# Beryl2000/SE-UNet-AirSeg

Hardware: AMD Instinct MI355X
Metric: voxels/sec SE-UNet fwd+bwd, 128^3 patch (higher is better)
Workload: dtype bf16

## Files before the change

### se-unet-airseg_amd/SE_UNet.py

```python
from __future__ import annotations

import ctypes as C
import os
from typing import List, Optional, Tuple

import torch
import torch.nn as nn

from . import _lib

config = {}

_DEBUG_FILL: Optional[int] = None


def _fresh(shape, dtype, device):
    t = torch.empty(shape, dtype=dtype, device=device)
    if _DEBUG_FILL is not None:
        t.view(torch.uint8).fill_(_DEBUG_FILL)
    return t


def _default_dtype() -> str:
    return os.environ.get("SEUNET_DTYPE", "bf16")
# ... 86 lines not shown
    while lib.seunet_net_conv_info(C.byref(desc), len(out), C.byref(info)) == 0:
        k = lambda code: _lib.KERNEL_NAMES[code]
        x_name = info.x_name.decode() or None
        out.append({
            "name": info.name.decode(), "taps": info.taps, "dilation": info.dilation, "level": info.level,
            "dims": (info.dims.n, info.dims.d, info.dims.h, info.dims.w),
            "src_c": [info.src_c[i] for i in range(info.nsrc)],
            "src_is_input": [bool(info.src_is_input[i]) for i in range(info.nsrc)],
            "cin": info.cin, "cout": info.cout, "need_dgrad": bool(info.need_dgrad),
            "fwd": k(info.fwd), "dgrad": k(info.dgrad) if info.need_dgrad else None, "wgrad": k(info.wgrad),
            "x_name": x_name, "x_materialised": bool(info.x_materialised),
            "x_fwd": k(info.x_fwd) if x_name and info.x_materialised else None,
            "x_wgrad": k(info.x_wgrad) if x_name and info.x_materialised else None,
            "src_dist": info.src_dist,
        })
    return out


def _is_decoder(name: str) -> bool:
    return name.startswith("dc") and not name.startswith("dc0_")


def alloc_flat_grads(params, dead, device, names=None):
    idx = list(range(len(params)))
    if names is not None:
        idx = [i for i in idx if not _is_decoder(names[i])] + [i for i in idx if _is_decoder(names[i])]
    sizes = {i: (0 if dead[i] else params[i].numel()) for i in idx}
    flat = _fresh(sum(sizes.values()), torch.float32, device)
    grads, off, split = [None] * len(params), 0, None
    for i in idx:
        if names is not None and split is None and _is_decoder(names[i]):
            split = off
        if not dead[i]:
            grads[i] = flat[off:off + sizes[i]].view(params[i].shape)
        off += sizes[i]
    return flat, grads, (off if split is None else split)


class _SEUNetFunction(torch.autograd.Function):
    @staticmethod
    def forward(ctx, x, drop1, drop2, meta, *params):
        lib = _lib.load()
        b, _, d, h, w = x.shape
        desc = make_desc(b, meta["in_channel"], meta["n_classes"], d, h, w, meta["width_mult"],
                         meta["dtype"], meta["conv_impl"], meta["negative_slope"])
        with torch.cuda.device(x.device):
            ws_bytes = lib.seunet_net_workspace_bytes(C.byref(desc))
            if ws_bytes == 0:
                raise RuntimeError("libseunet_hip net_workspace_bytes: " + _lib.last_error())
            ws = _fresh(ws_bytes, torch.uint8, x.device)
            pred0 = _fresh((b, meta["n_classes"], d, h, w), torch.float32, x.device)
            pred1 = _fresh((b, meta["n_classes"], d, h, w), torch.float32, x.device)
            plist = [p.detach().contiguous() for p in params]
            for p in plist:
                if p.device != x.device:
                    raise RuntimeError(f"SE_UNet parameters are on {p.device} but the input is on {x.device}")
            parr = _lib.ptr_array(plist)
            _lib.check(lib.seunet_net_forward(C.byref(desc), parr, x.data_ptr(), _lib.ptr(drop1), _lib.ptr(drop2),
                                              pred0.data_ptr(), pred1.data_ptr(), ws.data_ptr(), ws_bytes,
                                              _lib.stream_ptr()), "net_forward")
        ctx.desc, ctx.ws, ctx.ws_bytes = desc, ws, ws_bytes
        ctx.plist, ctx.drop = plist, (drop1, drop2)
        ctx.dead = meta["dead"]
        ctx.loss_scale = float(meta.get("loss_scale", 1.0))
        ctx.overflow, ctx.pending = meta.get("overflow"), meta.get("pending")
        ctx.names, ctx.grad_sync = meta.get("names"), meta.get("grad_sync")
        ctx.input_grad = bool(meta.get("input_grad", False))
        return pred0, pred1

    @staticmethod
    def backward(ctx, g0, g1):
        if ctx.ws is None:
            raise RuntimeError("SE_UNet (HIP path): the backward pass of this forward call has already run; it consumes "
                               "the saved workspace, so a second backward (retain_graph=True, or two losses "
                               "back-propagated separately) is not supported -- sum the losses and call backward once")
        lib = _lib.load()
        dev = ctx.ws.device
        shape = (ctx.desc.batch, ctx.desc.n_classes, ctx.desc.d, ctx.desc.h, ctx.desc.w)
        with torch.cuda.device(dev):
            g0 = torch.zeros(shape, dtype=torch.float32, device=dev) if g0 is None else g0.contiguous().float()
            g1 = torch.zeros(shape, dtype=torch.float32, device=dev) if g1 is None else g1.contiguous().float()
            if ctx.loss_scale != 1.0:
                g0, g1 = g0 * ctx.loss_scale, g1 * ctx.loss_scale
            flat, grads, split = alloc_flat_grads(ctx.plist, ctx.dead, dev, ctx.names)
            garr = _lib.ptr_array(grads)
            parr = _lib.ptr_array(ctx.plist)
            sync = ctx.grad_sync
            ev = sync.decoder_event() if sync is not None else None
            grad_x = None
            if ctx.input_grad and ctx.needs_input_grad[0]:
                d = ctx.desc
                grad_x = _fresh((d.batch, d.in_channel, d.d, d.h, d.w), torch.float32, dev)
                sbytes = lib.seunet_net_input_grad_bytes(C.byref(d))
                if sbytes == 0:
                    raise RuntimeError("libseunet_hip net_input_grad_bytes: " + _lib.last_error())
                scratch = _fresh(sbytes, torch.uint8, dev)
                _lib.check(lib.seunet_net_backward_input(C.byref(d), parr, g0.data_ptr(), g1.data_ptr(), _lib.ptr(ctx.drop[0]),
                                                         _lib.ptr(ctx.drop[1]), garr, grad_x.data_ptr(), scratch.data_ptr(), sbytes,
                                                         ctx.ws.data_ptr(), ctx.ws_bytes, _lib.stream_ptr(),
                                                         None if ev is None else ev.cuda_event), "net_backward_input")
            else:
                _lib.check(lib.seunet_net_backward_ev(C.byref(ctx.desc), parr, g0.data_ptr(), g1.data_ptr(),
                                                      _lib.ptr(ctx.drop[0]), _lib.ptr(ctx.drop[1]), garr,
                                                      ctx.ws.data_ptr(), ctx.ws_bytes, _lib.stream_ptr(),
                                                      None if ev is None else ev.cuda_event), "net_backward")
            if sync is not None:
                sync.exchange(flat, split, ev)
            if ctx.loss_scale != 1.0:
                ok = torch.isfinite(flat).all()
                if grad_x is not None:
                    ok = ok & torch.isfinite(grad_x).all()
                    grad_x.copy_(torch.where(ok, grad_x * (1.0 / ctx.loss_scale), torch.zeros((), dtype=grad_x.dtype, device=dev)))
                flat.copy_(torch.where(ok, flat * (1.0 / ctx.loss_scale), torch.zeros((), dtype=flat.dtype, device=dev)))
                if ctx.overflow is not None:
                    ctx.overflow.add_((~ok).to(ctx.overflow.dtype))
                if ctx.pending is not None:
                    ctx.pending.bitwise_or_((~ok).to(ctx.pending.dtype))
        ctx.ws = None
        return (grad_x, None, None, None) + tuple(grads)


class SE_UNet(nn.Module):

    def __init__(self, in_channel=1, n_classes=1, width_mult=1, negative_slope=0.01,
                 act_dtype: Optional[str] = None, conv_impl: Optional[int] = None, input_grad: bool = False):
        super().__init__()
        self.input_grad = bool(input_grad)
        self.in_channel, self.n_classes = in_channel, n_classes
        self.width_mult, self.negative_slope = width_mult, negative_slope
        self.act_dtype = act_dtype or _default_dtype()
        self.conv_impl = _default_conv_impl() if conv_impl is None else conv_impl
        self.loss_scale = 65536.0 if _lib.dtype_code(self.act_dtype) == _lib.F16 else 1.0
        self.overflow_steps = None
        self.overflow_pending = None
        self.batchnorm, self.bias, self.out_channel2, self.sigmoid_output = False, True, 2, 0
        m = width_mult
        self.ec1 = SSEConv(in_channel, 8 * m)
        self.ec2 = SSEConv(8 * m, 16 * m)
        self.ec3 = SSEConv(16 * m, 32 * m, dilation=2)
        self.ec33 = CATConv(56 * m, 32 * m)
        self.x33 = CATConv(in_channel, 32 * m)
        self.ec4 = SSEConv2(32 * m, 32 * m, down_sample=2)
        self.ec5 = SSEConv2(32 * m, 32 * m, dilation=2, down_sample=2)
        self.ec6 = SSEConv2(32 * m, 64 * m, dilation=2, down_sample=2)
        self.ec63 = CATConv(128 * m, 64 * m)
        self.x63 = CATConv(in_channel, 64 * m)
        self.ec7 = SSEConv2(64 * m, 64 * m, down_sample=4)
        self.ec8 = SSEConv2(64 * m, 64 * m, dilation=2, down_sample=4)
        self.ec9 = SSEConv2(64 * m, 64 * m, dilation=2, down_sample=4)
        self.ec93 = CATConv(192 * m, 64 * m)
        self.x93 = CATConv(in_channel, 64 * m)
        self.ec10 = SSEConv2(64 * m, 64 * m, down_sample=8)
        self.ec11 = SSEConv2(64 * m, 64 * m, down_sample=8)
        self.ec12 = SSEConv2(64 * m, 64 * m, down_sample=8)
        self.ec123 = CATConv(192 * m, 64 * m)
        self.dc1 = SSEConv2(128 * m, 64 * m, down_sample=4)
        self.dc2 = SSEConv2(64 * m, 64 * m, down_sample=4)
        self.dc22 = CATConv(128 * m, 64 * m)
        self.dc3 = SSEConv2(128 * m, 64 * m, down_sample=2)
        self.dc4 = SSEConv2(64 * m, 32 * m, down_sample=2)
        self.dc42 = CATConv(96 * m, 32 * m)
        self.dc5 = SSEConv(64 * m, 32 * m, down_sample=1)
        self.dc6 = SSEConv(32 * m, 16 * m, down_sample=1)
        self.dc62 = CATConv(48 * m, 16 * m)
        self.dc0_0 = nn.Conv3d(24, n_classes, 1, bias=True)
        self.dc0_1 = nn.Conv3d(12, n_classes, 1, bias=True)
        self.dropout1 = DropLayer(channel_num=24, thr=0.3)
# ... 222 lines not shown
```

### se-unet-airseg_amd/csrc/cat.hip

```cpp
#include "epilogue.h"
#include <type_traits>

namespace seunet {

template <bool XR>
__device__ __forceinline__ void second_branch(const float (&in8)[8], const float (&wa)[8], const float (&wb)[8], float (&x2)[8]) {
#pragma unroll
  for (int j = 0; j < 8; ++j) x2[j] = XR ? wa[j] * in8[0] + wb[j] * in8[1] : in8[j];
}

template <typename T, int LPV, bool TWO, bool XR>
__global__ void __launch_bounds__(EPI_THREADS)
cat_fwd_kernel(const T* __restrict__ raw, const float* __restrict__ mean, const float* __restrict__ rstd,
               const T* __restrict__ raw2, const float* __restrict__ mean2, const float* __restrict__ rstd2, int C, float slope,
               T* __restrict__ out, long long V, const float* __restrict__ w2x, int xic) {
  SEUNET_EPI_THREAD(LPV);
  float mu[8], rs[8], mu2[8], rs2[8], wa[8], wb[8];
#pragma unroll
  for (int j = 0; j < 8; ++j) {
    mu[j] = mean[n * C + c0 + j]; rs[j] = rstd[n * C + c0 + j];
    mu2[j] = TWO ? mean2[n * C + c0 + j] : 0.f;
    rs2[j] = TWO ? rstd2[n * C + c0 + j] : 0.f;
    wa[j] = XR ? w2x[(c0 + j) * xic] : 0.f;
    wb[j] = (XR && xic > 1) ? w2x[(c0 + j) * xic + 1] : 0.f;
  }
  const long long stride = (long long)P * VPB;
  long long v = (long long)blockIdx.x * VPB + vb;
  Pack8<T> nx, nx2;
  zero8p(nx); zero8p(nx2);
  if (v < V) {
    const long long o = ((long long)n * V + v) * C + c0;
    load8p(raw + o, nx);
    if (TWO) load8p(XR ? raw2 + ((long long)n * V + v) * 8 : raw2 + o, nx2);
  }
  for (; v < V; v += stride) {
    const long long o = ((long long)n * V + v) * C + c0;
    float x[8], in2[8], x2[8], y[8];
    unpack8(nx, x);
    if (TWO) { unpack8(nx2, in2); second_branch<XR>(in2, wa, wb, x2); }
    if (v + stride < V) {
      load8p(raw + o + stride * C, nx);
      if (TWO) load8p(XR ? raw2 + ((long long)n * V + v + stride) * 8 : raw2 + o + stride * C, nx2);
    }
#pragma unroll
    for (int j = 0; j < 8; ++j) y[j] = norm_lrelu(x[j], mu[j], rs[j], slope);
    if (TWO) {
#pragma unroll
      for (int j = 0; j < 8; ++j) y[j] += norm_lrelu(x2[j], mu2[j], rs2[j], slope);
    }
    store8(out + o, y);
  }
}

template <typename T, int LPV>
__global__ void __launch_bounds__(EPI_THREADS)
cat_fwd_pool_kernel(const T* __restrict__ raw, const float* __restrict__ mean, const float* __restrict__ rstd,
                    const T* __restrict__ xin, const float* __restrict__ mean2, const float* __restrict__ rstd2, int C, float slope,
                    T* __restrict__ out, T* __restrict__ pooled, int D, int H, int W, const float* __restrict__ w2x, int xic,
                    unsigned* __restrict__ argmax) {
  SEUNET_EPI_THREAD(LPV);
  float mu[8], rs[8], mu2[8], rs2[8], wa[8], wb[8];
#pragma unroll
  for (int j = 0; j < 8; ++j) {
    mu[j] = mean[n * C + c0 + j]; rs[j] = rstd[n * C + c0 + j];
    mu2[j] = mean2[n * C + c0 + j]; rs2[j] = rstd2[n * C + c0 + j];
    wa[j] = w2x[(c0 + j) * xic];
    wb[j] = xic > 1 ? w2x[(c0 + j) * xic + 1] : 0.f;
  }
  const int Do = D / 2, Ho = H / 2, Wo = W / 2;
  const long long V = (long long)D * H * W, Vo = (long long)Do * Ho * Wo;
  const long long stride = (long long)P * VPB;
  for (long long cv = (long long)blockIdx.x * VPB + vb; cv < Vo; cv += stride) {
    const int xo = (int)(cv % Wo);
    const int yo = (int)((cv / Wo) % Ho);
    const int zo = (int)(cv / ((long long)Wo * Ho));
    const long long v0 = ((long long)(2 * zo) * H + 2 * yo) * W + 2 * xo;
    Pack8<T> px[8], pi[8];
#pragma unroll
    for (int k = 0; k < 8; ++k) {
      const long long v = v0 + ((long long)(k >> 2) * H + ((k >> 1) & 1)) * W + (k & 1);
      load8p(raw + ((long long)n * V + v) * C + c0, px[k]);
      load8p(xin + ((long long)n * V + v) * 8, pi[k]);
    }
// ... 153 lines not shown
      }
    }
    if (APPLY) store8(dxhat_out + o, d);
  }
  if (APPLY) return;
  const int wave = threadIdx.x >> 6, lane = threadIdx.x & 63;
  if (XW) {
    __shared__ double redx[4][16][16];
#pragma unroll
    for (int j = 0; j < 8; ++j)
#pragma unroll
      for (int i = 0; i < 2; ++i) {
        const double r = stride_sum_d<LPV>((double)xw[j][i]);
        if (lane < LPV) redx[wave][lane][j * 2 + i] = r;
      }
    __syncthreads();
    double* rec = xw_partial + ((long long)n * P + blockIdx.x) * (C * 2);
    for (int e = threadIdx.x; e < LPV * 16; e += EPI_THREADS) {
      const int gq = e / 16, k = e % 16;
      rec[(gq * 8 + (k >> 1)) * 2 + (k & 1)] = ((redx[0][gq][k] + redx[1][gq][k]) + redx[2][gq][k]) + redx[3][gq][k];
    }
  }
  __shared__ double red[4][16][32];
#pragma unroll
  for (int q = 0; q < 4; ++q)
#pragma unroll
    for (int j = 0; j < 8; ++j) {
      const double r = stride_sum_d<LPV>((double)s[q][j]);
      if (lane < LPV) red[wave][lane][q * 8 + j] = r;
    }
  __syncthreads();
  const long long rec = (long long)n * P + blockIdx.x;
  for (int i = threadIdx.x; i < LPV * 32; i += EPI_THREADS) {
    const int gq = i / 32, k = i % 32, q = k >> 3;
    const double tot = ((red[0][gq][k] + red[1][gq][k]) + red[2][gq][k]) + red[3][gq][k];
    const int c = gq * 8 + (k & 7);
    if (q < 2) stat_partial[(rec * C + c) * 2 + q] = tot;
    else if (TWO) stat_partial2[(rec * C + c) * 2 + (q - 2)] = tot;
  }
}

template <typename T>
__global__ void __launch_bounds__(EPI_THREADS)
input_moments_kernel(const T* __restrict__ xin, double* __restrict__ partial, long long V) {
  const int n = blockIdx.y, P = gridDim.x;
  double s[5] = {0.0, 0.0, 0.0, 0.0, 0.0};
  for (long long v = (long long)blockIdx.x * EPI_THREADS + threadIdx.x; v < V; v += (long long)P * EPI_THREADS) {
    float x[8];
    load8(xin + ((long long)n * V + v) * 8, x);
    const double a = (double)x[0], b = (double)x[1];
    s[0] += a; s[1] += b; s[2] += a * a; s[3] += a * b; s[4] += b * b;
  }
  __shared__ double red[4][5];
  block_sum(s, red);
  if (const int k = threadIdx.x; k < 5) partial[((long long)n * P + blockIdx.x) * 5 + k] = wave4_sum(red, k);
}

__global__ void __launch_bounds__(256)
xbranch_stats_kernel(const double* __restrict__ partial, int slots, const float* __restrict__ w2, int C, int ic,
                     double inv_count, float eps, float* __restrict__ mean2, float* __restrict__ rstd2,
                     double* __restrict__ moments_out) {
  const int n = blockIdx.x;
  __shared__ double red[4][5], tot[5];
  double s[5] = {0.0, 0.0, 0.0, 0.0, 0.0};
  for (int b = threadIdx.x; b < slots; b += 256)
#pragma unroll
    for (int k = 0; k < 5; ++k) s[k] += partial[((long long)n * slots + b) * 5 + k];
  block_sum(s, red);
  if (threadIdx.x < 5) tot[threadIdx.x] = wave4_sum(red, threadIdx.x) * inv_count;
  __syncthreads();
  if (moments_out != nullptr && threadIdx.x < 5) moments_out[n * 5 + threadIdx.x] = tot[threadIdx.x];
  const double m0 = tot[0], m1 = tot[1];
  const double c00 = tot[2] - m0 * m0, c01 = tot[3] - m0 * m1, c11 = tot[4] - m1 * m1;
  for (int c = threadIdx.x; c < C; c += 256) {
    const double a = (double)w2[c * ic], b = ic > 1 ? (double)w2[c * ic + 1] : 0.0;
    const double mu = a * m0 + b * m1;
    double var = a * a * c00 + 2.0 * a * b * c01 + b * b * c11;
    if (var < 0.0) var = 0.0;
    mean2[n * C + c] = (float)mu;
    rstd2[n * C + c] = (float)(1.0 / sqrt(var + (double)eps));
  }
}

__global__ void __launch_bounds__(256)
xw_finalize_kernel(const double* __restrict__ xw_partial, const double* __restrict__ stat_partial2, int slots, int C, int N,
                   const double* __restrict__ moments, const float* __restrict__ w2, int ic, double eps, float* __restrict__ dw) {
  const int wave = threadIdx.x >> 6, lane = threadIdx.x & 63;
  const int c = blockIdx.x;
  __shared__ double red[4][3];
  const double wa = (double)w2[c * ic], wb = ic > 1 ? (double)w2[c * ic + 1] : 0.0;
  double g0 = 0.0, g1 = 0.0;
  for (int n = 0; n < N; ++n) {
    double s[3] = {0.0, 0.0, 0.0};
    for (int r = threadIdx.x; r < slots; r += 256) {
      const long long rec = (long long)n * slots + r;
      s[0] += xw_partial[(rec * C + c) * 2 + 0];
      s[1] += xw_partial[(rec * C + c) * 2 + 1];
      s[2] += stat_partial2[(rec * C + c) * 2 + 0];
    }
#pragma unroll
    for (int k = 0; k < 3; ++k) {
      double r = s[k];
#pragma unroll
      for (int off = 32; off >= 1; off >>= 1) r += shfl_xor_settled(r, off);
      if (lane == 0) red[wave][k] = r;
    }
    __syncthreads();
    if (threadIdx.x == 0) {
      const double S0 = wave4_sum(red, 0), S1 = wave4_sum(red, 1), Sd = wave4_sum(red, 2);
      const double* m = moments + n * 5;
      const double c00 = m[2] - m[0] * m[0], c01 = m[3] - m[0] * m[1], c11 = m[4] - m[1] * m[1];
      const double A0 = S0 - m[0] * Sd, A1 = S1 - m[1] * Sd;
      double var = wa * wa * c00 + 2.0 * wa * wb * c01 + wb * wb * c11;
      if (var < 0.0) var = 0.0;
      const double rs2 = 1.0 / (var + eps), rs = sqrt(rs2);
      const double proj = wa * A0 + wb * A1;
      g0 += rs * (A0 - rs2 * proj * (wa * c00 + wb * c01));
      g1 += rs * (A1 - rs2 * proj * (wa * c01 + wb * c11));
    }
    __syncthreads();
  }
  if (threadIdx.x == 0) {
    dw[c * ic] = (float)g0;
    if (ic > 1) dw[c * ic + 1] = (float)g1;
  }
}

template <typename T>
__global__ void __launch_bounds__(256)
xbranch_values_kernel(const T* __restrict__ x_in, const float* __restrict__ w2x, int C, int xic, float* __restrict__ out, long long V,
                      long long total) {
  for (long long i = blockIdx.x * (long long)blockDim.x + threadIdx.x; i < total; i += (long long)gridDim.x * blockDim.x) {
    const int cg = (int)(i % (C / 8));
    const long long nv = i / (C / 8);
    const long long n = nv / V, v = nv % V;
    float wa[8], wb[8], in2[8], x2[8];
#pragma unroll
    for (int j = 0; j < 8; ++j) {
      wa[j] = w2x[(cg * 8 + j) * xic];
      wb[j] = xic > 1 ? w2x[(cg * 8 + j) * xic + 1] : 0.f;
    }
    Pack8<T> px;
    load8p(x_in + nv * 8, px);
    unpack8(px, in2);
    second_branch<true>(in2, wa, wb, x2);
#pragma unroll
    for (int j = 0; j < 8; ++j) out[(n * C + cg * 8 + j) * V + v] = x2[j];
  }
}

static int cat_branch(const char* who, const CatBlock& b, Branch2& x, bool& two, bool& xr) {
  if (int e = check_c(b.C)) return e;
  x = b.b.kind == Branch2::None ? Branch2{} : b.b;
  two = x.kind != Branch2::None;
  xr = x.kind == Branch2::Recomputed;
  SEUNET_CHECK(!xr || (x.in_channel >= 1 && x.in_channel <= 2), "%s: in_channel %d (1 or 2)", who, x.in_channel);
  return 0;
}

int launch_cat_fwd(int dtype, const CatBlock& b, void* out, const PoolOut& pool, Dims d, hipStream_t s) {
  Branch2 x;
  bool two, xr;
  if (int e = cat_branch("cat_epilogue_fwd", b, x, two, xr)) return e;
  SEUNET_CHECK(!pool.pooled || (xr && d.D % 2 == 0 && d.H % 2 == 0 && d.W % 2 == 0),
               "cat_epilogue_fwd: the fused max-pool needs a recomputed second branch and even extents");
  dim3 grid(epi_partials(d) * 4, d.N);
#define SEUNET_CAT_FWD(...) <<<grid, EPI_THREADS, 0, s>>>((const T*)b.a.raw, b.a.mean, b.a.rstd, (const T*)x.src, x.mean2, x.rstd2, b.C, b.slope, (T*)out, __VA_ARGS__)
  SEUNET_LPV_SWITCH(b.C / 8, {
    SEUNET_DTYPE_SWITCH(dtype, {
      if (pool.pooled) cat_fwd_pool_kernel<T, LPV> SEUNET_CAT_FWD((T*)pool.pooled, d.D, d.H, d.W, x.w2, x.in_channel, pool.argmax);
      else if (xr) cat_fwd_kernel<T, LPV, true, true> SEUNET_CAT_FWD(d.vox(), x.w2, x.in_channel);
      else if (two) cat_fwd_kernel<T, LPV, true, false> SEUNET_CAT_FWD(d.vox(), nullptr, 0);
      else cat_fwd_kernel<T, LPV, false, false> SEUNET_CAT_FWD(d.vox(), nullptr, 0);
    });
  });
#undef SEUNET_CAT_FWD
  SEUNET_LAUNCH_CHECK();
  return 0;
}

static int cat_bwd_pool(const char* who, bool xr, const PoolGrad& pool, Dims d, PoolRef& pr) {
  pr = PoolRef{};
  if (pool.argmax == nullptr) return 0;
  SEUNET_CHECK(xr && pool.g_pool != nullptr && d.D % 2 == 0 && d.H % 2 == 0 && d.W % 2 == 0 && d.vox() < (1ll << 31),
               "%s: pooled gradient needs a recomputed second branch and even extents below 2^31 voxels", who);
  pr.argmax = pool.argmax; pr.g_pool = pool.g_pool;
  pr.W = (unsigned)d.W; pr.H = (unsigned)d.H; pr.Wo = (unsigned)d.W / 2; pr.Ho = (unsigned)d.H / 2;
  pr.mW = (unsigned)((1ull << 32) / (unsigned)d.W); pr.mH = (unsigned)((1ull << 32) / (unsigned)d.H);
  pr.Vo = d.vox() / 8;
  return 0;
}

#define SEUNET_CAT_BWD(TWO, APPLY, XW, XR, XG)                                                                                   \
  cat_bwd_kernel<T, LPV, TWO, APPLY, XW, XR, XG><<<grid, EPI_THREADS, 0, s>>>(                                                    \
      (const T*)g_out, (const T*)b.a.raw, b.a.mean, b.a.rstd, (const T*)x.src, x.mean2, x.rstd2, b.C, b.slope, a.m1, a.m2, a.m1b, \
      a.m2b, (T*)a.dx, (T*)a.dx2, o.stat_partial, o.stat_partial2, d.vox(), o.xw_partial, x.w2, x.in_channel, pr, a.gx_out,     \
      a.gx_acc)

int launch_cat_bwd_sums(int dtype, const CatBlock& b, const void* g_out, const PoolGrad& pool, const CatSums& out, Dims d,
                        hipStream_t s) {
  Branch2 x;
  bool two, xr;
  PoolRef pr;
  if (int e = cat_branch("cat_epilogue_bwd_sums", b, x, two, xr)) return e;
  if (int e = cat_bwd_pool("cat_epilogue_bwd_sums", xr, pool, d, pr)) return e;
  SEUNET_CHECK(out.stat_partial && (!two || out.stat_partial2), "cat_epilogue_bwd_sums needs the partial buffers");
  SEUNET_CHECK(!out.xw_partial || xr, "cat_epilogue_bwd_sums: the weight-gradient sums belong to a recomputed second branch");
  const CatSums o{out.stat_partial, two ? out.stat_partial2 : nullptr, out.xw_partial};
  const CatApply a{};
  dim3 grid(epi_partials(d), d.N);
  SEUNET_LPV_SWITCH(b.C / 8, {
    SEUNET_DTYPE_SWITCH(dtype, {
      if (xr && o.xw_partial) SEUNET_CAT_BWD(true, false, true, true, false);
      else if (xr) SEUNET_CAT_BWD(true, false, false, true, false);
      else if (two) SEUNET_CAT_BWD(true, false, false, false, false);
      else SEUNET_CAT_BWD(false, false, false, false, false);
    });
  });
  SEUNET_LAUNCH_CHECK();
  return 0;
}

int launch_cat_bwd_apply(int dtype, const CatBlock& b, const void* g_out, const PoolGrad& pool, const CatApply& io, Dims d,
                         hipStream_t s) {
  Branch2 x;
  bool two, xr;
  PoolRef pr;
  if (int e = cat_branch("cat_epilogue_bwd_apply", b, x, two, xr)) return e;
  if (int e = cat_bwd_pool("cat_epilogue_bwd_apply", xr, pool, d, pr)) return e;
  SEUNET_CHECK(io.m1 && io.m2 && io.dx && (!two || (io.m1b && io.m2b)) && (!two || xr || io.dx2),
               "cat_epilogue_bwd_apply: missing argument");
  SEUNET_CHECK(!io.gx_out || xr, "cat_epilogue_bwd_apply: the input-gradient term belongs to a recomputed second branch");
  const CatApply a{io.m1, io.m2, two ? io.m1b : nullptr, two ? io.m2b : nullptr, io.dx, two && !xr ? io.dx2 : nullptr,
                   io.gx_out, io.gx_out ? io.gx_acc : 0};
  const CatSums o{};
  dim3 grid(epi_partials(d) * 4, d.N);
  SEUNET_LPV_SWITCH(b.C / 8, {
    SEUNET_DTYPE_SWITCH(dtype, {
      if (xr && a.gx_out) SEUNET_CAT_BWD(true, true, false, true, true);
      else if (xr) SEUNET_CAT_BWD(true, true, false, true, false);
      else if (two) SEUNET_CAT_BWD(true, true, false, false, false);
      else SEUNET_CAT_BWD(false, true, false, false, false);
    });
  });
  SEUNET_LAUNCH_CHECK();
  return 0;
}
#undef SEUNET_CAT_BWD

int xbranch_moment_slots(Dims d) { return epi_partials(d); }

int launch_xbranch_moments(int dtype, const void* x_in, double* partial, Dims d, hipStream_t s) {
  dim3 grid(xbranch_moment_slots(d), d.N);
  SEUNET_DTYPE_SWITCH(dtype, input_moments_kernel<T><<<grid, EPI_THREADS, 0, s>>>((const T*)x_in, partial, d.vox()));
  SEUNET_LAUNCH_CHECK();
  return 0;
}

int launch_xbranch_stats(const double* partial, int slots, const float* w2, int C, int in_channel, int N, long long count,
                         float eps, float* mean2, float* rstd2, double* moments_out, hipStream_t s) {
  SEUNET_CHECK(in_channel >= 1 && in_channel <= 2, "xbranch_stats: in_channel %d (1 or 2)", in_channel);
  xbranch_stats_kernel<<<N, 256, 0, s>>>(partial, slots, w2, C, in_channel, 1.0 / (double)count, eps, mean2, rstd2, moments_out);
  SEUNET_LAUNCH_CHECK();
  return 0;
}

int launch_cat_xgrad_finalize(const double* xw_partial, const double* stat_partial2, int slots, const double* moments, const float* w2,
                              int C, int in_channel, int N, float eps, float* dw, hipStream_t s) {
  SEUNET_CHECK(in_channel >= 1 && in_channel <= 2, "cat_xgrad_finalize: in_channel %d (1 or 2)", in_channel);
  xw_finalize_kernel<<<C, 256, 0, s>>>(xw_partial, stat_partial2, slots, C, N, moments, w2, in_channel, (double)eps, dw);
  SEUNET_LAUNCH_CHECK();
  return 0;
}

int launch_xbranch_values(int dtype, const void* x_in, const float* w2, int C, int in_channel, float* out, Dims d, hipStream_t s) {
  SEUNET_CHECK(in_channel >= 1 && in_channel <= 2 && C % 8 == 0, "xbranch_values: bad argument");
  const long long total = (long long)d.N * d.vox() * (C / 8);
  const int grid = (int)((total + 255) / 256 > 8192 ? 8192 : (total + 255) / 256);
  SEUNET_DTYPE_SWITCH(dtype, xbranch_values_kernel<T><<<grid, 256, 0, s>>>((const T*)x_in, w2, C, in_channel, out, d.vox(), total));
  SEUNET_LAUNCH_CHECK();
  return 0;
}

}
```

### se-unet-airseg_amd/csrc/epilogue.h

```cpp
#pragma once
#include "seunet_common.h"

namespace seunet {

int epi_partials(Dims d);
int launch_channel_stats(int dtype, const void* t, int C, double* partial, Dims d, hipStream_t s);
int launch_stats_finalize(const double* partial, int slots, int C, int N, long long count,
                          float eps, int mode, float* out_a, float* out_b, hipStream_t s);
struct NormIn { const void* raw; const float* mean; const float* rstd; };
struct SseParams {
  const float* w_se;
  const float* w_se2;
  const float* w_side;
  const float* b_side;
  float slope;
};
struct GateBlock { NormIn a; int C; SseParams p; };
struct SseHead {
  float* side_out;
  float* level_map;
  int level_accumulate;
  const float* head_w;
  const float* drop;
  int drop_stride;
};
struct SseBwdIn {
  const void* g_e;
  const float* g_side;
  const float* g_level;
};
struct SseSums { double* stat_partial; float* pgrad_partial; };
struct SseApply { const float* m1; const float* m2; void* draw_out; };
int launch_sse_fwd(int dtype, const GateBlock& b, void* e_out, const SseHead& head, Dims d, hipStream_t s);
int launch_sse_bwd_sums(int dtype, const GateBlock& b, const SseBwdIn& g, const SseHead& head, const SseSums& out, Dims d,
                        hipStream_t s);
int launch_sse_bwd_apply(int dtype, const GateBlock& b, const SseBwdIn& g, const SseHead& head, const SseApply& io, Dims d,
                         hipStream_t s);
int launch_gate_bwd_finalize(const double* stat_partial, int slots, int C, int N, long long count, float* m1, float* m2,
                             const float* pgrad_partial, int records, float* dw_se, float* dw_se2, float* dw_side,
                             float* db_side, float* dhead_w, hipStream_t s);
int launch_pgrad_reduce(const float* pgrad_partial, int records, int C, float* dw_se,
                        float* dw_se2, float* dw_side, float* db_side, float* dhead_w,
                        hipStream_t s);
struct Branch2 {
  enum Kind { None, Stored, Recomputed } kind;
  const void* src;
  const float* mean2;
  const float* rstd2;
  const float* w2;
  int in_channel;
};
struct CatBlock { NormIn a; Branch2 b; int C; float slope; };
struct PoolOut { void* pooled; unsigned* argmax; };
struct PoolGrad { const unsigned* argmax; const void* g_pool; };
struct CatSums {
  double* stat_partial;
  double* stat_partial2;
  double* xw_partial;
};
struct CatApply {
  const float *m1, *m2, *m1b, *m2b;
  void* dx;
  void* dx2;
  float* gx_out;
  int gx_acc;
};
int launch_cat_fwd(int dtype, const CatBlock& b, void* out, const PoolOut& pool, Dims d, hipStream_t s);
int launch_cat_bwd_sums(int dtype, const CatBlock& b, const void* g_out, const PoolGrad& pool, const CatSums& out, Dims d,
                        hipStream_t s);
int launch_cat_bwd_apply(int dtype, const CatBlock& b, const void* g_out, const PoolGrad& pool, const CatApply& io, Dims d,
                         hipStream_t s);
int xbranch_moment_slots(Dims d);
int launch_xbranch_moments(int dtype, const void* x_in, double* partial, Dims d, hipStream_t s);
int launch_xbranch_stats(const double* partial, int slots, const float* w2, int C, int in_channel, int N, long long count,
                         float eps, float* mean2, float* rstd2, double* moments_out, hipStream_t s);
int launch_cat_xgrad_finalize(const double* xw_partial, const double* stat_partial2, int slots, const double* moments, const float* w2,
                              int C, int in_channel, int N, float eps, float* dw, hipStream_t s);
int launch_xbranch_values(int dtype, const void* x_in, const float* w2, int C, int in_channel, float* out_ncdhw, Dims d, hipStream_t s);

#ifdef __HIPCC__
static constexpr int EPI_THREADS = 256;

template <typename T> __device__ __forceinline__ float round_to(float v) {
  if constexpr (sizeof(T) == 4) return v;
  else return unpack_lo<T>(pack2<T>(v, 0.f));
}

template <typename T> __device__ __forceinline__ float gate_sigmoid(float z) {
  if constexpr (sizeof(T) == 4) return 1.f / (1.f + expf(-z));
  else return __builtin_amdgcn_rcpf(1.f + __builtin_amdgcn_exp2f(-1.44269504088896341f * z));
}

#define SEUNET_EPI_THREAD(LPV)                                \
  const int n = blockIdx.y, P = gridDim.x;                    \
  const int cg = threadIdx.x % LPV, vb = threadIdx.x / LPV;   \
  constexpr int VPB = EPI_THREADS / LPV;                      \
  const int c0 = cg * 8

__device__ __forceinline__ float lrelu(float xh, float slope) { return xh > 0.f ? xh : xh * slope; }
__device__ __forceinline__ float norm_lrelu(float x, float mu, float rs, float slope) { return lrelu((x - mu) * rs, slope); }
__device__ __forceinline__ float lrelu_slope(float xh, float slope) { return xh > 0.f ? 1.f : slope; }

template <typename E, int K> __device__ __forceinline__ E wave4_sum(const E (&red)[4][16][K], int g, int k) {
  return ((red[0][g][k] + red[1][g][k]) + red[2][g][k]) + red[3][g][k];
}
template <typename E, int K> __device__ __forceinline__ E wave4_sum(const E (&red)[4][K], int k) {
  return ((red[0][k] + red[1][k]) + red[2][k]) + red[3][k];
}
template <typename E> __device__ __forceinline__ E wave4_sum(const E (&w)[4]) { return ((w[0] + w[1]) + w[2]) + w[3]; }

template <int K> __device__ __forceinline__ void block_sum(const double (&s)[K], double (&red)[4][K]) {
  const int wave = threadIdx.x >> 6, lane = threadIdx.x & 63;
#pragma unroll
  for (int k = 0; k < K; ++k) {
    double r = s[k];
#pragma unroll
    for (int off = 32; off >= 1; off >>= 1) r += shfl_xor_settled(r, off);
    if (lane == 0) red[wave][k] = r;
  }
  __syncthreads();
}

__device__ __forceinline__ void stats_finalize_body(int idx, const double* __restrict__ partial, int slots, int C, double inv_count,
                                                    float eps, int mode, float* __restrict__ out_a, float* __restrict__ out_b) {
  const int n = idx / C, c = idx % C;
  double s1 = 0.0, s2 = 0.0;
  for (int p = threadIdx.x; p < slots; p += 256) {
    const double* q = partial + (((long long)n * slots + p) * C + c) * 2;
    s1 += q[0];
    s2 += q[1];
  }
#pragma unroll
  for (int off = 32; off >= 1; off >>= 1) {
    s1 += shfl_xor_settled(s1, off);
    s2 += shfl_xor_settled(s2, off);
  }
  __shared__ double w1[4], w2[4];
  if ((threadIdx.x & 63) == 0) { w1[threadIdx.x >> 6] = s1; w2[threadIdx.x >> 6] = s2; }
  __syncthreads();
  if (threadIdx.x == 0) {
    s1 = wave4_sum(w1);
    s2 = wave4_sum(w2);
    if (mode == 0) {
      const double mean = s1 * inv_count;
      double var = s2 * inv_count - mean * mean;
      if (var < 0.0) var = 0.0;
      out_a[idx] = (float)mean;
      out_b[idx] = (float)(1.0 / sqrt(var + (double)eps));
    } else {
      out_a[idx] = (float)(s1 * inv_count);
      out_b[idx] = (float)(s2 * inv_count);
    }
  }
}

#define SEUNET_LPV_SWITCH(LPVVAL, ...)                                                  \
  switch (LPVVAL) {                                                                       \
    case 1: { constexpr int LPV = 1; __VA_ARGS__; } break;                                       \
    case 2: { constexpr int LPV = 2; __VA_ARGS__; } break;                                       \
    case 4: { constexpr int LPV = 4; __VA_ARGS__; } break;                                       \
// ... 13 lines not shown
```

### se-unet-airseg_amd/csrc/gate.hip

```cpp
#include "epilogue.h"

namespace seunet {

template <typename T, int LPV, bool G2>
__global__ void __launch_bounds__(EPI_THREADS)
sse_fwd_kernel(const T* __restrict__ raw, const float* __restrict__ mean, const float* __restrict__ rstd, int C, SseParams p,
               T* __restrict__ e_out, SseHead head, long long V) {
  SEUNET_EPI_THREAD(LPV);
  float mu[8], rs[8], wse[8], wse2[8], w20[8], w21[8];
#pragma unroll
  for (int j = 0; j < 8; ++j) {
    mu[j] = mean[n * C + c0 + j];
    rs[j] = rstd[n * C + c0 + j];
    wse[j] = p.w_se[c0 + j];
    wse2[j] = G2 ? p.w_se2[c0 + j] : 0.f;
    w20[j] = p.w_side[c0 + j];
    w21[j] = p.w_side[C + c0 + j];
  }
  const float b20 = p.b_side[0], b21 = p.b_side[1], slope = p.slope;
  const bool want_side = head.side_out != nullptr || head.level_map != nullptr;
  float hw0 = 0.f, hw1 = 0.f;
  if (head.level_map) {
    hw0 = head.head_w[0] * (head.drop ? head.drop[n * head.drop_stride + 0] : 1.f);
    hw1 = head.head_w[1] * (head.drop ? head.drop[n * head.drop_stride + 1] : 1.f);
  }
  const long long stride = (long long)P * VPB;
  long long v = (long long)blockIdx.x * VPB + vb;
  Pack8<T> nx;
  zero8p(nx);
  if (v < V) load8p(raw + ((long long)n * V + v) * C + c0, nx);
  for (; v < V; v += stride) {
    const long long vi = (long long)n * V + v;
    float x[8], a[8], e[8];
    unpack8(nx, x);
    if (v + stride < V) load8p(raw + (vi + stride) * C + c0, nx);
    float d1 = 0.f;
#pragma unroll
    for (int j = 0; j < 8; ++j) {
      a[j] = norm_lrelu(x[j], mu[j], rs[j], slope);
      d1 += wse[j] * a[j];
    }
    const float g1 = gate_sigmoid<T>(group_sum<LPV>(d1));
    float d2 = 0.f;
#pragma unroll
    for (int j = 0; j < 8; ++j) {
      e[j] = a[j] * g1;
      d2 += wse2[j] * e[j];
    }
    if (G2) {
      const float g2 = gate_sigmoid<T>(group_sum<LPV>(d2));
#pragma unroll
      for (int j = 0; j < 8; ++j) e[j] *= g2;
    }
    store8(e_out + vi * C + c0, e);
    if (want_side) {
      float s0 = 0.f, s1 = 0.f;
#pragma unroll
      for (int j = 0; j < 8; ++j) { s0 += w20[j] * e[j]; s1 += w21[j] * e[j]; }
      s0 = group_sum<LPV>(s0) + b20;
      s1 = group_sum<LPV>(s1) + b21;
      if (cg == 0) {
        if (head.side_out) { head.side_out[vi * 2] = s0; head.side_out[vi * 2 + 1] = s1; }
        if (head.level_map) {
          const float t = hw0 * s0 + hw1 * s1;
          head.level_map[vi] = head.level_accumulate ? head.level_map[vi] + t : t;
        }
      }
    }
  }
}

template <typename T, int LPV, bool G2, bool APPLY, bool LEVEL>
__global__ void __launch_bounds__(EPI_THREADS, (APPLY || G2) ? 1 : 3)
sse_bwd_kernel(const T* __restrict__ raw, const float* __restrict__ mean, const float* __restrict__ rstd, int C, SseParams p,
               SseBwdIn g, SseHead head, const float* __restrict__ m1p, const float* __restrict__ m2p, T* dxhat_out,
               double* __restrict__ stat_partial, float* __restrict__ pgrad_partial, long long V) {
  SEUNET_EPI_THREAD(LPV);
  float mu[8], rs[8], wse[8], wse2[8], w20[8], w21[8];
#pragma unroll
  for (int j = 0; j < 8; ++j) {
    mu[j] = mean[n * C + c0 + j];
    rs[j] = rstd[n * C + c0 + j];
    wse[j] = p.w_se[c0 + j];
// ... 137 lines not shown
  if (LEVEL) {
    float h0 = cg == 0 ? b20 * sgl : 0.f, h1 = cg == 0 ? b21 * sgl : 0.f;
#pragma unroll
    for (int j = 0; j < 8; ++j) {
      const float G = aw20[j];
      h0 += w20[j] * G;
      h1 += w21[j] * G;
      aw20[j] = hw0 * G;
      aw21[j] = hw1 * G;
    }
    adh0 = dr0 * h0;
    adh1 = dr1 * h1;
    adb0 = cg == 0 ? hw0 * sgl : 0.f;
    adb1 = cg == 0 ? hw1 * sgl : 0.f;
  }
  double sdx[8], sdxx[8];
#pragma unroll
  for (int j = 0; j < 8; ++j) {
    sdx[j] = (F64ACC ? acc64[j][threadIdx.x] : 0.0) + (double)fdx[j];
    sdxx[j] = (F64ACC ? acc64[8 + j][threadIdx.x] : 0.0) + (double)fdxx[j];
  }

  __shared__ double redd[4][16][16];
  __shared__ float red[4][16][32];
  __shared__ float reds[4][4];
  const int wave = threadIdx.x >> 6, lane = threadIdx.x & 63;
#pragma unroll
  for (int j = 0; j < 8; ++j) {
    const double r0 = stride_sum_d<LPV>(sdx[j]), r1 = stride_sum_d<LPV>(sdxx[j]);
    const float r2 = stride_sum<LPV>(awse[j]), r3 = stride_sum<LPV>(awse2[j]);
    const float r4 = stride_sum<LPV>(aw20[j]), r5 = stride_sum<LPV>(aw21[j]);
    if (lane < LPV) {
      redd[wave][lane][j] = r0;     redd[wave][lane][8 + j] = r1;
      red[wave][lane][j] = r2;      red[wave][lane][8 + j] = r3;
      red[wave][lane][16 + j] = r4; red[wave][lane][24 + j] = r5;
    }
  }
  {
    const float q0 = stride_sum<1>(adb0), q1 = stride_sum<1>(adb1);
    const float q2 = stride_sum<1>(adh0), q3 = stride_sum<1>(adh1);
    if (lane == 0) { reds[wave][0] = q0; reds[wave][1] = q1; reds[wave][2] = q2; reds[wave][3] = q3; }
  }
  __syncthreads();
  const long long rec = (long long)n * P + blockIdx.x;
  float* pg = pgrad_partial + rec * (4 * C + 4);
  for (int i = threadIdx.x; i < LPV * 16; i += EPI_THREADS) {
    const int gq = i / 16, k = i % 16;
    const double tot = wave4_sum(redd, gq, k);
    stat_partial[(rec * C + gq * 8 + (k & 7)) * 2 + (k >> 3)] = tot;
  }
  for (int i = threadIdx.x; i < LPV * 32; i += EPI_THREADS) {
    const int gq = i / 32, k = i % 32;
    const float tot = wave4_sum(red, gq, k);
    pg[(k >> 3) * C + gq * 8 + (k & 7)] = tot;
  }
  if (const int k = threadIdx.x; k < 4) pg[4 * C + k] = wave4_sum(reds, k);
}

__device__ __forceinline__ void pgrad_reduce_body(int blk, const float* __restrict__ pg, int records, int C, float* dw_se,
                                                  float* dw_se2, float* dw_side, float* db_side, float* dhead_w) {
  const int wave = threadIdx.x >> 6, lane = threadIdx.x & 63;
  const int k = blk * 4 + wave, K = 4 * C + 4;
  if (k >= K) return;
  double s = 0.0;
  for (int r = lane; r < records; r += 64) s += (double)pg[(long long)r * K + k];
#pragma unroll
  for (int off = 32; off >= 1; off >>= 1) s += shfl_xor_settled(s, off);
  if (lane != 0) return;
  const float v = (float)s;
  if (k < C) { if (dw_se) dw_se[k] = v; }
  else if (k < 2 * C) { if (dw_se2) dw_se2[k - C] = v; }
  else if (k < 4 * C) { if (dw_side) dw_side[k - 2 * C] = v; }
  else if (k < 4 * C + 2) { if (db_side) db_side[k - 4 * C] = v; }
  else { if (dhead_w) dhead_w[k - 4 * C - 2] = v; }
}
__global__ void __launch_bounds__(256)
pgrad_reduce_kernel(const float* __restrict__ pg, int records, int C, float* dw_se, float* dw_se2,
                    float* dw_side, float* db_side, float* dhead_w) {
  pgrad_reduce_body(blockIdx.x, pg, records, C, dw_se, dw_se2, dw_side, db_side, dhead_w);
}
__global__ void __launch_bounds__(256)
gate_bwd_finalize_kernel(const double* __restrict__ partial, int slots, int C, int N, double inv_count, float* __restrict__ m1,
                         float* __restrict__ m2, const float* __restrict__ pg, int records, float* dw_se, float* dw_se2,
                         float* dw_side, float* db_side, float* dhead_w) {
  if ((int)blockIdx.x < N * C) stats_finalize_body(blockIdx.x, partial, slots, C, inv_count, 0.f, 1, m1, m2);
  else pgrad_reduce_body((int)blockIdx.x - N * C, pg, records, C, dw_se, dw_se2, dw_side, db_side, dhead_w);
}

int launch_sse_fwd(int dtype, const GateBlock& b, void* e_out, const SseHead& head, Dims d, hipStream_t s) {
  if (int e = check_c(b.C)) return e;
  dim3 grid(epi_partials(d) * 4, d.N);
  const bool g2 = b.p.w_se2 != nullptr;
  SEUNET_LPV_SWITCH(b.C / 8, {
    SEUNET_DTYPE_SWITCH(dtype, {
      if (g2) sse_fwd_kernel<T, LPV, true><<<grid, EPI_THREADS, 0, s>>>((const T*)b.a.raw, b.a.mean, b.a.rstd, b.C, b.p, (T*)e_out, head, d.vox());
      else sse_fwd_kernel<T, LPV, false><<<grid, EPI_THREADS, 0, s>>>((const T*)b.a.raw, b.a.mean, b.a.rstd, b.C, b.p, (T*)e_out, head, d.vox());
    });
  });
  SEUNET_LAUNCH_CHECK();
  return 0;
}

template <typename T, bool APPLY>
static int sse_bwd_t(const GateBlock& b, const SseBwdIn& g, const SseHead& head, const SseSums& o, const SseApply& a, Dims d,
                     hipStream_t s) {
  dim3 grid(epi_partials(d) * (APPLY ? 4 : 1), d.N);
  const bool g2 = b.p.w_se2 != nullptr;
  const bool level = g.g_level != nullptr;
#define SEUNET_SSE_BWD(G2V, LV) sse_bwd_kernel<T, LPV, G2V, APPLY, LV><<<grid, EPI_THREADS, 0, s>>>((const T*)b.a.raw, b.a.mean, b.a.rstd, b.C, b.p, g, head, a.m1, a.m2, (T*)a.draw_out, o.stat_partial, o.pgrad_partial, d.vox())
  SEUNET_LPV_SWITCH(b.C / 8, {
    if (g2) { if (level) SEUNET_SSE_BWD(true, true); else SEUNET_SSE_BWD(true, false); }
    else { if (level) SEUNET_SSE_BWD(false, true); else SEUNET_SSE_BWD(false, false); }
  });
#undef SEUNET_SSE_BWD
  SEUNET_LAUNCH_CHECK();
  return 0;
}

int launch_sse_bwd_sums(int dtype, const GateBlock& b, const SseBwdIn& g, const SseHead& head, const SseSums& out, Dims d,
                        hipStream_t s) {
  if (int e = check_c(b.C)) return e;
  SEUNET_CHECK(out.stat_partial && out.pgrad_partial, "gate_epilogue_bwd_sums needs the partial buffers");
  SEUNET_DTYPE_SWITCH(dtype, return (sse_bwd_t<T, false>(b, g, head, out, SseApply{}, d, s)));
  return 1;
}

int launch_sse_bwd_apply(int dtype, const GateBlock& b, const SseBwdIn& g, const SseHead& head, const SseApply& io, Dims d,
                         hipStream_t s) {
  if (int e = check_c(b.C)) return e;
  SEUNET_CHECK(io.m1 && io.m2 && io.draw_out, "gate_epilogue_bwd_apply needs m1, m2 and the output tensor");
  SEUNET_DTYPE_SWITCH(dtype, return (sse_bwd_t<T, true>(b, g, head, SseSums{}, io, d, s)));
  return 1;
}

int launch_gate_bwd_finalize(const double* stat_partial, int slots, int C, int N, long long count, float* m1, float* m2,
                             const float* pgrad_partial, int records, float* dw_se, float* dw_se2, float* dw_side,
                             float* db_side, float* dhead_w, hipStream_t s) {
  gate_bwd_finalize_kernel<<<N * C + cdiv(4 * C + 4, 4), 256, 0, s>>>(stat_partial, slots, C, N, 1.0 / (double)count, m1, m2,
                                                                     pgrad_partial, records, dw_se, dw_se2, dw_side, db_side, dhead_w);
  SEUNET_LAUNCH_CHECK();
  return 0;
}

int launch_pgrad_reduce(const float* pgrad_partial, int records, int C, float* dw_se, float* dw_se2, float* dw_side, float* db_side,
                        float* dhead_w, hipStream_t s) {
  pgrad_reduce_kernel<<<cdiv(4 * C + 4, 4), 256, 0, s>>>(pgrad_partial, records, C, dw_se, dw_se2, dw_side, db_side, dhead_w);
  SEUNET_LAUNCH_CHECK();
  return 0;
}

}
```

### se-unet-airseg_amd/csrc/heads.hip

```cpp
#include "seunet_common.h"
#include "trilinear.h"

namespace seunet {

__global__ void side_upsample_kernel(const float* __restrict__ side, int C, int scale,
                                     float* __restrict__ out, int c_total, int c_off, int D, int H, int W,
                                     long long total) {
  const int Do = D * scale, Ho = H * scale, Wo = W * scale;
  const float rz = ac_scale(D, Do), ry = ac_scale(H, Ho), rx = ac_scale(W, Wo);
  const long long Vo = (long long)Do * Ho * Wo;
  for (long long i = blockIdx.x * (long long)blockDim.x + threadIdx.x; i < total;
       i += (long long)gridDim.x * blockDim.x) {
    long long r = i;
    const int xo = (int)(r % Wo); r /= Wo;
    const int yo = (int)(r % Ho); r /= Ho;
    const int zo = (int)(r % Do);
    const long long n = r / Do;
    int z0, z1, y0, y1, x0, x1; float lz, ly, lx;
    ac_src(zo, rz, D, z0, z1, lz);
    ac_src(yo, ry, H, y0, y1, ly);
    ac_src(xo, rx, W, x0, x1, lx);
    for (int c = 0; c < C; ++c) {
      float acc = 0.f;
#pragma unroll
// ... 197 lines not shown
  ka = (ca + 3) & ~3; kb = (cb + 3) & ~3;
  const int la = e0 < ebase[2] ? 1 : (e0 < ebase[3] ? 2 : 3), lb = e1 < ebase[2] ? 1 : (e1 < ebase[3] ? 2 : 3);
  float* const outa = e0 < nent ? (la == 1 ? t1a : (la == 2 ? t1b : t1c)) : nullptr;
  float* const outb = e1 < nent ? (lb == 1 ? t1a : (lb == 2 ? t1b : t1c)) : nullptr;
  const int cola = e0 - ebase[la], colb = e1 - ebase[lb], wla = W >> la, wlb = W >> lb;
  double sum = 0.0;
#pragma unroll
  for (int j = 0; j < RPW; ++j) {
    const int rr = wv + 4 * j;
    const long long row = row0 + rr;
    if (row >= rows) break;
    float* rb = hsm + wv * RW;
    if (pf) {
#pragma unroll
      for (int k = 0; k < 4; ++k) {
        const int x = lane + 64 * k;
        if (x < W) { rb[x] = pre[j][k]; sum += (double)pre[j][k]; }
      }
    } else {
      for (int x = lane; x < W; x += 64) { const float v = g[row * W + x]; rb[x] = v; sum += (double)v; }
    }
    __builtin_amdgcn_wave_barrier();
    if (fast) {
      float a0 = 0.f, a1 = 0.f;
#pragma unroll
      for (int k = 0; k < HB_KA; ++k)
        if (k < ka) a0 += wa[k] * rb[fa + k];
#pragma unroll
      for (int k = 0; k < HB_K; ++k)
        if (k < kb) a1 += wb[k] * rb[fb + k];
      if (outa) outa[row * wla + cola] = a0;
      if (outb) outb[row * wlb + colb] = a1;
      __builtin_amdgcn_wave_barrier();
      continue;
    }
    for (int e = lane; e < nent; e += 64) {
      const int l = e < ebase[2] ? 1 : (e < ebase[3] ? 2 : 3);
      float* out = outs[l - 1];
      if (out == nullptr) continue;
      const float* t = tab + e * (HB_K + 2);
      const int first = __float_as_int(t[0]), cnt = __float_as_int(t[1]);
      float acc = 0.f;
      for (int k = 0; k < cnt; k += 4) {
        float w[4], v[4];
#pragma unroll
        for (int j = 0; j < 4; ++j) {
          const bool in = k + j < cnt;
          w[j] = in ? t[2 + k + j] : 0.f;
          v[j] = in ? rb[first + k + j] : 0.f;
        }
#pragma unroll
        for (int j = 0; j < 4; ++j)
          if (w[j] != 0.f) acc += w[j] * v[j];
      }
      out[row * (W >> l) + (e - ebase[l])] = acc;
    }
    __builtin_amdgcn_wave_barrier();
  }
  if (bias_part != nullptr) {
#pragma unroll
    for (int off = 32; off >= 1; off >>= 1) sum += shfl_xor_settled(sum, off);
    __shared__ double wsum[4];
    if (lane == 0) wsum[wv] = sum;
    __syncthreads();
    if (threadIdx.x == 0) bias_part[blockIdx.x] = ((wsum[0] + wsum[1]) + wsum[2]) + wsum[3];
  }
}

__global__ void __launch_bounds__(1024) sum_stage2_wide_kernel(const double* __restrict__ partial, int n, float* __restrict__ out) {
  double s = 0.0;
  for (int i = threadIdx.x; i < n; i += 1024) s += partial[i];
#pragma unroll
  for (int off = 32; off >= 1; off >>= 1) s += shfl_xor_settled(s, off);
  __shared__ double w[16];
  if ((threadIdx.x & 63) == 0) w[threadIdx.x >> 6] = s;
  __syncthreads();
  if (threadIdx.x == 0) {
    double t = 0.0;
    for (int k = 0; k < 16; ++k) t += w[k];
    out[0] = (float)t;
  }
}

int launch_side_upsample(const float* side, int C, int scale, float* out, int c_total, int c_off, Dims dl,
                         hipStream_t s) {
  const long long total = (long long)dl.N * dl.vox() * scale * scale * scale;
  side_upsample_kernel<<<grid_for(total), 256, 0, s>>>(side, C, scale, out, c_total, c_off, dl.D, dl.H, dl.W, total);
  SEUNET_LAUNCH_CHECK();
  return 0;
}

int launch_head_fwd(const float* const* level_maps, int nlevels, const float* bias, float* pred, Dims d0,
                    hipStream_t s) {
  SEUNET_CHECK(nlevels >= 1 && nlevels <= 4, "head: nlevels=%d out of range", nlevels);
  HeadLevels lv;
  for (int l = 0; l < 4; ++l) lv.map[l] = l < nlevels ? level_maps[l] : nullptr;
  for (int l = 1; l < nlevels; ++l)
    SEUNET_CHECK((d0.D >> l) >= 1 && (d0.H >> l) >= 1 && (d0.W >> l) >= 1, "head: volume too small for level %d", l);
  SEUNET_CHECK(d0.W % 4 == 0, "head: W=%d must be a multiple of 4", d0.W);
  if (d0.W % 8 == 0 && d0.W <= 2048 && (long long)d0.D * d0.H * d0.W < (1ll << 31)) {
    const size_t lds = (size_t)4 * HF_RPW * ((d0.W >> 1) + (d0.W >> 2) + (d0.W >> 3)) * sizeof(float);
    const int ybl = (d0.H + 4 * HF_RPW - 1) / (4 * HF_RPW);
    head_fwd_rows_kernel<<<d0.N * d0.D * ybl, 256, lds, s>>>(lv, bias, pred, d0.D, d0.H, d0.W);
  } else {
    const long long total4 = (long long)d0.N * d0.vox() / 4;
    head_fwd_kernel<<<grid_for(total4), 256, 0, s>>>(lv, bias, pred, d0.D, d0.H, d0.W, total4);
  }
  SEUNET_LAUNCH_CHECK();
  return 0;
}

struct AxisJob { const float* in; float* out; int I, O; long long inner, total; };
struct AxisJobs { AxisJob j[3]; };
__global__ void __launch_bounds__(256) up_transpose_axis_multi_kernel(AxisJobs jobs) {
  const AxisJob jb = jobs.j[blockIdx.y];
  if (jb.total == 0) return;
  const float rs = ac_scale(jb.I, jb.O);
  const unsigned inner = (unsigned)jb.inner, I = (unsigned)jb.I, total = (unsigned)jb.total;
  for (unsigned idx = blockIdx.x * blockDim.x + threadIdx.x; idx < total; idx += gridDim.x * blockDim.x) {
    const unsigned q = idx / inner;
    const unsigned in_i = idx - q * inner;
    const unsigned outer = q / I;
    const int i = (int)(q - outer * I);
    int lo, hi;
    ac_range(i, rs, jb.O, lo, hi);
    float acc = 0.f;
    for (int o = lo; o <= hi; o += 4) {
      float w[4], v[4];
#pragma unroll
      for (int k = 0; k < 4; ++k) {
        w[k] = o + k <= hi ? ac_weight(o + k, i, rs, jb.I) : 0.f;
        v[k] = w[k] != 0.f ? jb.in[(outer * (unsigned)jb.O + (unsigned)(o + k)) * inner + in_i] : 0.f;
      }
#pragma unroll
      for (int k = 0; k < 4; ++k)
        if (w[k] != 0.f) acc += w[k] * v[k];
    }
    jb.out[idx] = acc;
  }
}

struct HeadBwdLayout { long long t1[4], t2[4], part, total; };
static HeadBwdLayout head_bwd_layout(Dims d0, int nlevels) {
  HeadBwdLayout m{};
  const long long rows = (long long)d0.N * d0.D * d0.H, V = rows * d0.W;
  long long off = 0, off2 = V - V / 8;
  for (int l = 1; l < nlevels; ++l) {
    m.t1[l] = off;
    off += rows * (d0.W >> l);
    m.t2[l] = off2;
    off2 += (long long)d0.N * d0.D * (d0.H >> l) * (d0.W >> l);
  }
  m.part = (V + V / 2 + 64 + 1) & ~1ll;
  m.total = V + V / 2 + 64 + 2 * ((rows + HB_ROWS - 1) / HB_ROWS + 64);
  return m;
}
size_t head_bwd_tmp_floats(Dims d0) { return (size_t)head_bwd_layout(d0, 4).total; }
int launch_head_bwd(const float* g_pred, float* const* g_levels, int nlevels, float* tmp, float* g_bias,
                    Dims d0, hipStream_t s) {
  SEUNET_CHECK(nlevels >= 1 && nlevels <= 4, "head: nlevels=%d out of range", nlevels);
  const long long rows = (long long)d0.N * d0.D * d0.H;
  const long long V = rows * d0.W;
  const HeadBwdLayout m = head_bwd_layout(d0, nlevels);
  float* t1[4] = {nullptr, nullptr, nullptr, nullptr};
  float* t2[4] = {nullptr, nullptr, nullptr, nullptr};
  for (int l = 1; l < nlevels; ++l) {
    if (g_levels[l]) t1[l] = tmp + m.t1[l];
    t2[l] = tmp + m.t2[l];
  }
  double* part = reinterpret_cast<double*>(tmp + m.part);
  const int nblk = (int)((rows + HB_ROWS - 1) / HB_ROWS);
  SEUNET_CHECK(d0.W <= 1024, "head_bwd: W=%d too large", d0.W);
  SEUNET_CHECK(V / 2 < (1ll << 31), "head_bwd: %lld voxels per call exceed the 32-bit index range of the axis passes", V);
  const size_t lds = ((size_t)4 * (d0.W + HB_PAD) + (size_t)(d0.W - (d0.W >> 3)) * (HB_K + 2)) * sizeof(float);
  head_bwd_x_multi_kernel<<<nblk, 256, lds, s>>>(g_pred, t1[1], t1[2], t1[3], nlevels, d0.W, rows, g_bias ? part : nullptr);
  AxisJobs jy{}, jz{};
  long long max_y = 0, max_z = 0;
  int njobs = 0;
  for (int l = 1; l < nlevels; ++l) {
    if (!g_levels[l]) continue;
    const int Dl = d0.D >> l, Hl = d0.H >> l, Wl = d0.W >> l;
    const long long ty = (long long)d0.N * d0.D * Hl * Wl, tz = (long long)d0.N * Dl * Hl * Wl;
    jy.j[njobs] = AxisJob{t1[l], t2[l], Hl, d0.H, (long long)Wl, ty};
    jz.j[njobs] = AxisJob{t2[l], g_levels[l], Dl, d0.D, (long long)Hl * Wl, tz};
    max_y = ty > max_y ? ty : max_y;
    max_z = tz > max_z ? tz : max_z;
    ++njobs;
  }
  if (njobs) {
    up_transpose_axis_multi_kernel<<<dim3((unsigned)grid_for(max_y), (unsigned)njobs), 256, 0, s>>>(jy);
    up_transpose_axis_multi_kernel<<<dim3((unsigned)grid_for(max_z), (unsigned)njobs), 256, 0, s>>>(jz);
  }
  if (g_bias) sum_stage2_wide_kernel<<<1, 1024, 0, s>>>(part, nblk, g_bias);
  SEUNET_LAUNCH_CHECK();
  return 0;
}

}
```

### se-unet-airseg_amd/csrc/layout.hip

```cpp
#include "seunet_common.h"

namespace seunet {

template <typename T>
__global__ void pack_cl_kernel(const float* __restrict__ in, int C, T* __restrict__ out, int Cpad,
                               long long V, long long total) {
  const int G = Cpad / 8;
  for (long long i = blockIdx.x * (long long)blockDim.x + threadIdx.x; i < total;
       i += (long long)gridDim.x * blockDim.x) {
    const long long v = i % V;
    const int g = (int)((i / V) % G);
    const long long n = i / (V * G);
    float x[8];
#pragma unroll
    for (int j = 0; j < 8; ++j) {
      const int c = g * 8 + j;
      x[j] = c < C ? in[(n * C + c) * V + v] : 0.f;
    }
    store8(out + (n * V + v) * Cpad + g * 8, x);
  }
}

template <typename T>
__global__ void unpack_cl_kernel(const T* __restrict__ in, int C, float* __restrict__ out, long long V,
                                 long long total) {
  const int G = C / 8;
  for (long long i = blockIdx.x * (long long)blockDim.x + threadIdx.x; i < total;
       i += (long long)gridDim.x * blockDim.x) {
    const long long v = i % V;
    const int g = (int)((i / V) % G);
    const long long n = i / (V * G);
    float x[8];
    load8(in + (n * V + v) * C + g * 8, x);
#pragma unroll
    for (int j = 0; j < 8; ++j) out[(n * C + g * 8 + j) * V + v] = x[j];
  }
}

template <typename T>
__global__ void maxpool_fwd_kernel(const T* __restrict__ in, int C, T* __restrict__ out, int D, int H,
                                   int W, long long total) {
  const int G = C / 8, Do = D / 2, Ho = H / 2, Wo = W / 2;
  for (long long i = blockIdx.x * (long long)blockDim.x + threadIdx.x; i < total;
       i += (long long)gridDim.x * blockDim.x) {
    const int g = (int)(i % G);
    long long r = i / G;
    const int xo = (int)(r % Wo); r /= Wo;
    const int yo = (int)(r % Ho); r /= Ho;
    const int zo = (int)(r % Do);
    const long long n = r / Do;
    float m[8];
#pragma unroll
    for (int j = 0; j < 8; ++j) m[j] = -INFINITY;
#pragma unroll
    for (int k = 0; k < 8; ++k) {
      const int z = 2 * zo + (k >> 2), y = 2 * yo + ((k >> 1) & 1), x = 2 * xo + (k & 1);
      float v[8];
      load8(in + ((((n * D + z) * H + y) * W + x) * (long long)C) + g * 8, v);
#pragma unroll
      for (int j = 0; j < 8; ++j) m[j] = v[j] > m[j] ? v[j] : m[j];
    }
    store8(out + ((((n * Do + zo) * Ho + yo) * Wo + xo) * (long long)C) + g * 8, m);
  }
}

template <typename T>
__global__ void maxpool_bwd_kernel(const T* __restrict__ in, const T* __restrict__ g_out, int C,
                                   T* g_in, int accumulate, int D, int H, int W, long long total) {
  const int G = C / 8, Do = D / 2, Ho = H / 2, Wo = W / 2;
  for (long long i = blockIdx.x * (long long)blockDim.x + threadIdx.x; i < total;
       i += (long long)gridDim.x * blockDim.x) {
    const int g = (int)(i % G);
    long long r = i / G;
    const int xo = (int)(r % Wo); r /= Wo;
    const int yo = (int)(r % Ho); r /= Ho;
    const int zo = (int)(r % Do);
    const long long n = r / Do;
    float m[8], gy[8];
    int am[8];
#pragma unroll
    for (int j = 0; j < 8; ++j) { m[j] = -INFINITY; am[j] = 0; }
#pragma unroll
    for (int k = 0; k < 8; ++k) {
      const int z = 2 * zo + (k >> 2), y = 2 * yo + ((k >> 1) & 1), x = 2 * xo + (k & 1);
      float v[8];
      load8(in + ((((n * D + z) * H + y) * W + x) * (long long)C) + g * 8, v);
#pragma unroll
      for (int j = 0; j < 8; ++j)
        if (v[j] > m[j]) { m[j] = v[j]; am[j] = k; }
    }
    load8(g_out + ((((n * Do + zo) * Ho + yo) * Wo + xo) * (long long)C) + g * 8, gy);
#pragma unroll
    for (int k = 0; k < 8; ++k) {
      const int z = 2 * zo + (k >> 2), y = 2 * yo + ((k >> 1) & 1), x = 2 * xo + (k & 1);
      T* p = g_in + ((((n * D + z) * H + y) * W + x) * (long long)C) + g * 8;
      float v[8];
      if (accumulate) load8(p, v);
#pragma unroll
      for (int j = 0; j < 8; ++j) v[j] = (accumulate ? v[j] : 0.f) + (am[j] == k ? gy[j] : 0.f);
      store8(p, v);
    }
  }
}

int launch_pack_cl(int dtype, const float* in, int C, void* out, int Cpad, Dims d, hipStream_t s) {
  SEUNET_CHECK(Cpad % 8 == 0 && Cpad >= C, "pack_cl: padded channel count %d invalid for C=%d", Cpad, C);
  const long long V = d.vox(), total = (long long)d.N * V * (Cpad / 8);
  SEUNET_DTYPE_SWITCH(dtype, pack_cl_kernel<T><<<grid_for(total), 256, 0, s>>>(in, C, (T*)out, Cpad, V, total));
  SEUNET_LAUNCH_CHECK();
  return 0;
}
int launch_pack_input(int dtype, const float* x, int in_channel, void* out, Dims d, hipStream_t s) {
  SEUNET_CHECK(in_channel >= 1 && in_channel <= 8, "in_channel %d unsupported (1..8)", in_channel);
  return launch_pack_cl(dtype, x, in_channel, out, 8, d, s);
}
int launch_unpack_cl(int dtype, const void* in, int C, float* out, Dims d, hipStream_t s) {
  SEUNET_CHECK(C % 8 == 0, "unpack_cl: C=%d must be a multiple of 8", C);
  const long long V = d.vox(), total = (long long)d.N * V * (C / 8);
  SEUNET_DTYPE_SWITCH(dtype, unpack_cl_kernel<T><<<grid_for(total), 256, 0, s>>>((const T*)in, C, out, V, total));
  SEUNET_LAUNCH_CHECK();
  return 0;
}

int launch_maxpool_fwd(int dtype, const void* in, int C, void* out, Dims d, hipStream_t s) {
  SEUNET_CHECK(C % 8 == 0 && d.D % 2 == 0 && d.H % 2 == 0 && d.W % 2 == 0, "maxpool: bad shape");
  const long long total = (long long)d.N * (d.D / 2) * (d.H / 2) * (d.W / 2) * (C / 8);
  SEUNET_DTYPE_SWITCH(dtype, maxpool_fwd_kernel<T><<<grid_for(total), 256, 0, s>>>((const T*)in, C, (T*)out, d.D, d.H, d.W, total));
  SEUNET_LAUNCH_CHECK();
  return 0;
}
int launch_maxpool_bwd(int dtype, const void* in, const void* g_out, int C, void* g_in, int accumulate,
                       Dims d, hipStream_t s) {
  SEUNET_CHECK(C % 8 == 0 && d.D % 2 == 0 && d.H % 2 == 0 && d.W % 2 == 0, "maxpool: bad shape");
  const long long total = (long long)d.N * (d.D / 2) * (d.H / 2) * (d.W / 2) * (C / 8);
  SEUNET_DTYPE_SWITCH(dtype, maxpool_bwd_kernel<T><<<grid_for(total), 256, 0, s>>>((const T*)in, (const T*)g_out, C, (T*)g_in, accumulate, d.D, d.H, d.W, total));
  SEUNET_LAUNCH_CHECK();
  return 0;
}

struct ZeroList { float* ptr[48]; int count[48]; int n; };
__global__ void multi_zero_kernel(ZeroList z) {
  float* p = z.ptr[blockIdx.x];
  for (int i = threadIdx.x; i < z.count[blockIdx.x]; i += blockDim.x) p[i] = 0.f;
}
int launch_multi_zero(float* const* ptrs, const int* counts, int n, hipStream_t s) {
  for (int base = 0; base < n; base += 48) {
    ZeroList z{};
    z.n = n - base < 48 ? n - base : 48;
    for (int i = 0; i < z.n; ++i) { z.ptr[i] = ptrs[base + i]; z.count[i] = counts[base + i]; }
    multi_zero_kernel<<<z.n, 256, 0, s>>>(z);
  }
  SEUNET_LAUNCH_CHECK();
  return 0;
}

}
```

### se-unet-airseg_amd/csrc/net.cpp

```cpp
#include "seunet_common.h"
#include "epilogue.h"
#include "wgrad.h"
#include "../../include/seunet_hip.h"

#include <algorithm>
#include <cstdio>
#include <cstring>
#include <string>
#include <vector>

namespace seunet {

ConvKernel wgrad_kernel(int dtype, int taps, int dil, const SrcList& x, int cin_logical, int cout, Dims d, long long src_dist) {
  if (taps == 1) {
    const int combos = cdiv(cin_logical, 32) * cdiv(cout, 32);
    const long long nv = (long long)d.N * d.vox();
    const bool pays = combos >= 16 || (combos >= 8 && nv >= 500000);
    return pays && wgrad_1x1_supported(dtype, x, cin_logical, cout) ? ConvKernel::Wgrad1x1 : ConvKernel::Tiled;
  }
  const bool fine = d.W >= 32 && (long long)d.D * d.H * d.W >= 48LL * 48 * 48;
  const bool pays = fine || dil == 2 || cin_logical >= 256;
  return pays && wgrad_march_supported(dtype, taps, dil, x, cin_logical, cout, d, src_dist) ? ConvKernel::March : ConvKernel::Tiled;
}

namespace {

enum TId {
  T_NONE,
  T_X0, T_X1, T_X2,
  T_E0, T_E1A, T_E1_1, T_E1, T_E2IN, T_E2, T_E3A, T_E3_1, T_E3, T_E4IN, T_E4, T_E5A, T_E5_1, T_E5,
  T_E6IN, T_E6, T_E7A, T_E7_1, T_E7, T_E8, T_D0A, T_D0_1, T_D0, T_D1U, T_D1A, T_D1_1, T_D1, T_D2U, T_D2A, T_D2_1,
  T_COUNT
};
enum OpKind { OP_GATED, OP_CAT, OP_POOL, OP_UP };
struct OpDesc {
  OpKind kind; const char* name;
  int src[3]; int dst;
  int cout;
  int dil; int gates;
  const char* xname; int xsrc;
};
constexpr OpDesc kOps[] = {
    {.kind = OP_GATED, .name = "ec1", .src = {T_X0}, .dst = T_E0, .cout = 8, .dil = 1, .gates = 1},
    {.kind = OP_GATED, .name = "ec2", .src = {T_E0}, .dst = T_E1A, .cout = 16, .dil = 1, .gates = 1},
    {.kind = OP_GATED, .name = "ec3", .src = {T_E1A}, .dst = T_E1_1, .cout = 32, .dil = 2, .gates = 1},
    {.kind = OP_CAT, .name = "ec33", .src = {T_E1_1, T_E0, T_E1A}, .dst = T_E1, .cout = 32, .xname = "x33", .xsrc = T_X0},
    {.kind = OP_POOL, .name = "pool0", .src = {T_E1}, .dst = T_E2IN},
    {.kind = OP_POOL, .name = "pool0x", .src = {T_X0}, .dst = T_X1},
    {.kind = OP_GATED, .name = "ec4", .src = {T_E2IN}, .dst = T_E2, .cout = 32, .dil = 1, .gates = 2},
    {.kind = OP_GATED, .name = "ec5", .src = {T_E2}, .dst = T_E3A, .cout = 32, .dil = 2, .gates = 2},
    {.kind = OP_GATED, .name = "ec6", .src = {T_E3A}, .dst = T_E3_1, .cout = 64, .dil = 2, .gates = 2},
    {.kind = OP_CAT, .name = "ec63", .src = {T_E3_1, T_E2, T_E3A}, .dst = T_E3, .cout = 64, .xname = "x63", .xsrc = T_X1},
    {.kind = OP_POOL, .name = "pool1", .src = {T_E3}, .dst = T_E4IN},
    {.kind = OP_POOL, .name = "pool1x", .src = {T_X1}, .dst = T_X2},
    {.kind = OP_GATED, .name = "ec7", .src = {T_E4IN}, .dst = T_E4, .cout = 64, .dil = 1, .gates = 2},
    {.kind = OP_GATED, .name = "ec8", .src = {T_E4}, .dst = T_E5A, .cout = 64, .dil = 2, .gates = 2},
    {.kind = OP_GATED, .name = "ec9", .src = {T_E5A}, .dst = T_E5_1, .cout = 64, .dil = 2, .gates = 2},
    {.kind = OP_CAT, .name = "ec93", .src = {T_E5_1, T_E4, T_E5A}, .dst = T_E5, .cout = 64, .xname = "x93", .xsrc = T_X2},
    {.kind = OP_POOL, .name = "pool2", .src = {T_E5}, .dst = T_E6IN},
    {.kind = OP_GATED, .name = "ec10", .src = {T_E6IN}, .dst = T_E6, .cout = 64, .dil = 1, .gates = 2},
    {.kind = OP_GATED, .name = "ec11", .src = {T_E6}, .dst = T_E7A, .cout = 64, .dil = 1, .gates = 2},
    {.kind = OP_GATED, .name = "ec12", .src = {T_E7A}, .dst = T_E7_1, .cout = 64, .dil = 1, .gates = 2},
    {.kind = OP_CAT, .name = "ec123", .src = {T_E7_1, T_E6, T_E7A}, .dst = T_E7, .cout = 64},
    {.kind = OP_UP, .name = "up0", .src = {T_E7}, .dst = T_E8},
    {.kind = OP_GATED, .name = "dc1", .src = {T_E8, T_E5}, .dst = T_D0A, .cout = 64, .dil = 1, .gates = 2},
    {.kind = OP_GATED, .name = "dc2", .src = {T_D0A}, .dst = T_D0_1, .cout = 64, .dil = 1, .gates = 2},
    {.kind = OP_CAT, .name = "dc22", .src = {T_D0_1, T_D0A}, .dst = T_D0, .cout = 64},
    {.kind = OP_UP, .name = "up1", .src = {T_D0}, .dst = T_D1U},
    {.kind = OP_GATED, .name = "dc3", .src = {T_D1U, T_E3}, .dst = T_D1A, .cout = 64, .dil = 1, .gates = 2},
    {.kind = OP_GATED, .name = "dc4", .src = {T_D1A}, .dst = T_D1_1, .cout = 32, .dil = 1, .gates = 2},
    {.kind = OP_CAT, .name = "dc42", .src = {T_D1_1, T_D1A}, .dst = T_D1, .cout = 32},
    {.kind = OP_UP, .name = "up2", .src = {T_D1}, .dst = T_D2U},
    {.kind = OP_GATED, .name = "dc5", .src = {T_D2U, T_E1}, .dst = T_D2A, .cout = 32, .dil = 1, .gates = 1},
    {.kind = OP_GATED, .name = "dc6", .src = {T_D2A}, .dst = T_D2_1, .cout = 16, .dil = 1, .gates = 1},
};
constexpr int kNumOps = sizeof(kOps) / sizeof(kOps[0]);
constexpr bool is_conv(const OpDesc& o) { return o.kind == OP_GATED || o.kind == OP_CAT; }

enum PField { P_CONV1_W, P_CONV1_B, P_CONV2_W, P_CONV2_B, P_SE, P_SE2, P_HEAD_W, P_HEAD_B };
constexpr const char* kFieldName[] = {"conv1.weight", "conv1.bias", "conv2.weight", "conv2.bias", "conv_se.weight", "conv_se2.weight",
                                      "weight", "bias"};
struct BlockParams { int at[6] = {-1, -1, -1, -1, -1, -1}, xw = -1; };
struct ParamDesc { const char* block; PField f; int cin, cout, k; };
constexpr int kNumParams = 117;

struct Graph {
  int level[T_COUNT] = {}, cbase[T_COUNT] = {};
  const char* tname[T_COUNT] = {};
  int nsrc[kNumOps] = {}, cin[kNumOps] = {};
  int head[kNumOps] = {}, slot[kNumOps] = {};
  int sides[2] = {};
  int first_up = -1, nconv = 0;
  BlockParams prm[kNumOps] = {};
  ParamDesc param[kNumParams] = {};
  int nparams = 0, dead = -1, head_w[2] = {}, head_b[2] = {};

  constexpr int add(const char* block, PField f, int ci, int co, int k) { param[nparams] = {block, f, ci, co, k}; return nparams++; }
  constexpr BlockParams add_block(const char* name, int gates, int ci, int co) {
    BlockParams b;
    const int fields = gates ? 4 + gates : 1;
    for (int f = 0; f < fields; ++f) b.at[f] = add(name, (PField)f, ci, co, gates ? 3 : 1);
    return b;
  }
};
constexpr Graph derive() {
  Graph g;
  g.tname[T_X0] = "x";
  for (int i = 0; i < kNumOps; ++i) {
// ... 386 lines not shown
    mark("epi_fwd:", c.o.name);
    if (int e = launch_sse_fwd(p.d.dtype, gate_block(c), at(p.feat[c.o.dst]), hd, c.dm, s)) return e;
    return hd.side_out ? side_to_level(c, hd.level_accumulate) : 0;
  }

  int cat_forward(const Op& c) {
    const OpRes& r = c.r;
    const CatBlock blk = cat_block(c);
    if (int e = conv_and_stats(c.o.name, r.fwd, 1, 1, srcs(c.i), r.cin, par(c.i, P_CONV1_W), nullptr, r.wp_f, r.raw, r.cout, r.mean,
                               r.rstd, c.dm)) return e;
    PoolOut pool_out{};
    if (blk.b.kind == Branch2::Recomputed) {
      mark("stats");
      if (int e = launch_xbranch_moments(p.d.dtype, blk.b.src, dat(p.xmom), c.dm, s)) return e;
      if (int e = launch_xbranch_stats(dat(p.xmom), xbranch_moment_slots(c.dm), blk.b.w2, r.cout, p.d.in_channel, c.dm.N, c.dm.vox(),
                                       p.d.eps, fat(r.mean2), fat(r.rstd2), dat(r.xtot), s)) return e;
      SEUNET_CHECK(r.fused >= 0, "net: internal: %s has no max-pool to write", c.o.name);
      pool_out = PoolOut{at(p.feat[kOps[r.fused].dst]), reinterpret_cast<unsigned*>(at(p.op[r.fused].pool_idx))};
    } else if (blk.b.kind == Branch2::Stored) {
      if (int e = conv_and_stats(c.o.xname, r.x_fwd, 1, 1, xbranch_src(c.o), p.d.in_channel, par(kG.prm[c.i].xw), nullptr, r.wp_x, r.raw2,
                                 r.cout, r.mean2, r.rstd2, c.dm)) return e;
    }
    mark("cat_fwd:", c.o.name);
    return launch_cat_fwd(p.d.dtype, blk, at(p.feat[c.o.dst]), pool_out, c.dm, s);
  }

  int pool_forward(const Op& c) {
    if (c.r.fused >= 0) return 0;
    const int t = c.o.src[0];
    mark("pool_fwd:", c.o.name);
    return launch_maxpool_fwd(p.d.dtype, at(p.feat[t]), p.C[t], at(p.feat[c.o.dst]), p.dims_of(t), s);
  }

  int up_forward(const Op& c) {
    const int t = c.o.src[0];
    mark("up_fwd:", c.o.name);
    return launch_upsample2_fwd(p.d.dtype, at(p.feat[t]), p.C[t], at(p.feat[c.o.dst]), p.dims_of(t), s);
  }

  int heads_forward(float* pred0, float* pred1) {
    float* const pred[2] = {pred0, pred1};
    const Dims d1{1, p.dims[0].D, p.dims[0].H, p.dims[0].W};
    mark("head_fwd");
    for (int h = 0; h < 2; ++h) {
      if (pred[h] == nullptr) continue;
      const int nl = 4 - h;
      if (p.d.n_classes > 1) {
        if (int e = per_sample_class(p.lvl[h], 0, nl, [&](float* const* lm, size_t nc) {
              return launch_head_fwd(lm, nl, par(kG.head_b[h]) + nc % p.d.n_classes, pred[h] + nc * d1.vox(), d1, s);
            })) return e;
      } else {
        const float* lm[4] = {fat(p.lvl[h][0]), fat(p.lvl[h][1]), fat(p.lvl[h][2]), fat(p.lvl[h][3])};
        if (int e = launch_head_fwd(lm, nl, par(kG.head_b[h]), pred[h], p.dims[0], s)) return e;
      }
    }
    mark("outside");
    return 0;
  }

  int forward(const float* x, const float* drop1, const float* drop2, float* pred0, float* pred1) {
    skip_enc_head = pred0 == nullptr;
    drops[0] = drop1; drops[1] = drop2;
    if (int e = pack_all_weights(false)) return e;
    mark("pack_input");
    if (int e = launch_pack_input(p.d.dtype, x, p.d.in_channel, at(p.feat[T_X0]), p.dims[0], s)) return e;
    for (int i = 0; i < kNumOps; ++i) {
      const Op c = op(i);
      const OpKind k = c.o.kind;
      if (int e = k == OP_GATED ? gated_forward(c) : k == OP_CAT ? cat_forward(c) : k == OP_POOL ? pool_forward(c) : up_forward(c))
        return e;
    }
    return heads_forward(pred0, pred1);
  }

  const float* g_pred[2] = {nullptr, nullptr};
  float* const* grads = nullptr;
  bool written[T_COUNT] = {};
  std::vector<float*> zero_ptrs;
  std::vector<int> zero_counts;
  hipEvent_t decoder_done = nullptr;

  float* gpar(int op, PField f) const { const int k = kG.prm[op].at[f]; return k < 0 ? nullptr : grads[k]; }

  int conv_backward(const Op& c) {
    const OpDesc& o = c.o;
    const OpRes& r = c.r;
    const SrcList x = srcs(c.i);
    if (float* gw = gpar(c.i, P_CONV1_W)) {
      mark("wgrad:", o.name);
      if (int e = run_wgrad(r.wgrad, p.d.dtype, r.taps, o.dil, x, r.cin, at(p.grad[o.dst]), r.cout, gw, at(p.wgrad_ws),
                            p.wgrad_ws_bytes, c.dm, s)) return e;
    }
    if (!r.need_dgrad) return 0;
    const SrcList gsrc{{at(p.grad[o.dst])}, {r.cout}, 1};
    DstList gd{};
    gd.n = x.n;
    for (int k = 0; k < x.n; ++k) {
      const int t = o.src[k];
      gd.C[k] = p.C[t];
      gd.ptr[k] = is_input(t) ? nullptr : at(p.grad[t]);
      gd.acc[k] = (!is_input(t) && written[t]) ? 1 : 0;
      if (!is_input(t)) written[t] = true;
    }
    mark("dgrad:", o.name);
    return run_conv(r.dgrad, r.taps, o.dil, gsrc, r.cout, par(c.i, P_CONV1_W), 1, at(r.wp_d), nullptr, gd, nullptr, c.dm);
  }

  int heads_backward() {
    const Dims d1{1, p.dims[0].D, p.dims[0].H, p.dims[0].W};
    mark("head_bwd");
    for (int h = 0; h < 2; ++h) {
      const int nl = 4 - h;
      float* gb = grads[kG.head_b[h]];
      if (p.d.n_classes > 1) {
        if (int e = per_sample_class(p.glvl[h], 1, nl, [&](float* const* gl, size_t nc) {
              return launch_head_bwd(g_pred[h] + nc * d1.vox(), gl, nl, fat(p.head_tmp), fat(p.cls_bias) + nc, d1, s);
            })) return e;
        if (gb)
          if (int e = launch_class_bias_grad(fat(p.cls_bias), p.d.batch, p.d.n_classes, gb, s)) return e;
      } else {
        float* gl[4] = {nullptr, fat(p.glvl[h][1]), fat(p.glvl[h][2]), nl == 4 ? fat(p.glvl[h][3]) : nullptr};
        if (int e = launch_head_bwd(g_pred[h], gl, nl, fat(p.head_tmp), gb, p.dims[0], s)) return e;
      }
    }
    return 0;
  }

  int gated_backward(const Op& c) {
    const OpDesc& o = c.o;
    const int h = kG.head[c.i], P_slots = epi_partials(c.dm);
    const GateBlock blk = gate_block(c);
    SseBwdIn g{written[o.dst] ? at(p.grad[o.dst]) : nullptr, nullptr, c.lv == 0 ? g_pred[h] : fat(p.glvl[h][c.lv])};
    SseHead hd = sse_head(c.i, false);
    float* g_head = head_slice(c.i, grads).gw;
    if (p.d.n_classes > 1) {
      if (int e = level_to_side_grad(c, g.g_level)) return e;
      g.g_level = nullptr;
      g.g_side = fat(p.gside);
      hd.side_out = nullptr;
      g_head = nullptr;
    }
    mark("epi_bwd:", o.name);
    if (int e = launch_sse_bwd_sums(p.d.dtype, blk, g, hd, SseSums{dat(p.stats), fat(p.pgrad)}, c.dm, s)) return e;
    mark("stats");
    if (int e = launch_gate_bwd_finalize(dat(p.stats), P_slots, c.r.cout, c.dm.N, c.dm.vox(), fat(p.m1), fat(p.m2), fat(p.pgrad),
                                         c.dm.N * P_slots, gpar(c.i, P_SE), gpar(c.i, P_SE2), gpar(c.i, P_CONV2_W),
                                         gpar(c.i, P_CONV2_B), g_head, s)) return e;
    mark("in_bwd:", o.name);
    if (int e = launch_sse_bwd_apply(p.d.dtype, blk, g, hd, SseApply{fat(p.m1), fat(p.m2), at(p.grad[o.dst])}, c.dm, s)) return e;
    written[o.dst] = true;
    if (float* gb = gpar(c.i, P_CONV1_B)) { zero_ptrs.push_back(gb); zero_counts.push_back(c.r.cout); }
    return conv_backward(c);
  }

  int cat_backward(const Op& c) {
    const OpDesc& o = c.o;
    const OpRes& r = c.r;
    const int P_slots = epi_partials(c.dm);
    SEUNET_CHECK(written[o.dst], "net: internal: gradient of %s output missing", o.name);
    const CatBlock blk = cat_block(c);
    const bool two = blk.b.kind != Branch2::None, recomputed = blk.b.kind == Branch2::Recomputed;
    float* gxw = two ? grads[kG.prm[c.i].xw] : nullptr;
    const void* g_out = at(p.grad[o.dst]);
    PoolGrad pool{};
    if (r.fused >= 0) pool = PoolGrad{reinterpret_cast<const unsigned*>(at(p.op[r.fused].pool_idx)), at(p.grad[kOps[r.fused].dst])};
    mark("cat_bwd:", o.name);
    const CatSums sums{dat(p.stats), dat(p.stats2), recomputed && gxw ? dat(p.xwp) : nullptr};
    if (int e = launch_cat_bwd_sums(p.d.dtype, blk, g_out, pool, sums, c.dm, s)) return e;
    mark("stats");
    if (recomputed && gxw)
      if (int e = launch_cat_xgrad_finalize(dat(p.xwp), dat(p.stats2), P_slots, dat(r.xtot), blk.b.w2, r.cout, p.d.in_channel, c.dm.N,
                                            p.d.eps, gxw, s)) return e;
    if (int e = launch_stats_finalize(dat(p.stats), P_slots, r.cout, c.dm.N, c.dm.vox(), 0.f, 1, fat(p.m1), fat(p.m2), s)) return e;
    if (two)
      if (int e = launch_stats_finalize(dat(p.stats2), P_slots, r.cout, c.dm.N, c.dm.vox(), 0.f, 1, fat(p.m1b), fat(p.m2b), s)) return e;
    mark("in_bwd:", o.name);
    CatApply ap{fat(p.m1), fat(p.m2), fat(p.m1b), fat(p.m2b), at(p.grad[o.dst]), two && !recomputed ? at(p.gx) : nullptr, nullptr, 0};
    if (recomputed && grad_x) { ap.gx_out = gxl(c.lv); ap.gx_acc = c.lv == 1 ? 1 : 0; }
    if (int e = launch_cat_bwd_apply(p.d.dtype, blk, g_out, pool, ap, c.dm, s)) return e;
    if (two && !recomputed) {
      if (grad_x) {
        mark("input_grad:", o.xname);
        if (int e = launch_xgrad_contract(p.d.dtype, at(p.gx), r.cout, par(kG.prm[c.i].xw), p.d.in_channel, gxl(c.lv), c.lv == 1 ? 1 : 0, c.dm, s)) return e;
      }
      if (gxw) {
        mark("wgrad:", o.xname);
        if (int e = run_wgrad(r.x_wgrad, p.d.dtype, 1, 1, xbranch_src(o), p.d.in_channel, at(p.gx), r.cout, gxw, at(p.wgrad_ws),
                              p.wgrad_ws_bytes, c.dm, s)) return e;
      }
    }
    return conv_backward(c);
  }

  int pool_backward(const Op& c) {
    const OpDesc& o = c.o;
    const int t = o.src[0];
    if (grad_x && o.dst == T_X2) {
      mark("input_grad:unpool1");
      if (int e = launch_xgrad_unpool(p.d.dtype, at(p.feat[T_X1]), p.d.in_channel, gxl(2), gxl(1), p.dims[1], s)) return e;
    }
    if (is_input(t)) return 0;
    SEUNET_CHECK(written[o.dst], "net: internal: gradient of %s output missing", o.name);
    mark("pool_bwd:", o.name);
    if (c.r.fused >= 0) {
      SEUNET_CHECK(written[t], "net: internal: gradient of %s input missing before its deferred pool gradient", o.name);
      return 0;
    }
    if (int e = launch_maxpool_bwd(p.d.dtype, at(p.feat[t]), at(p.grad[o.dst]), p.C[t], at(p.grad[t]), written[t] ? 1 : 0,
                                   p.dims_of(t), s)) return e;
    written[t] = true;
    return 0;
  }

  int up_backward(const Op& c) {
    const int t = c.o.src[0];
    SEUNET_CHECK(written[c.o.dst], "net: internal: gradient of %s output missing", c.o.name);
    mark("up_bwd:", c.o.name);
    if (int e = launch_upsample2_bwd(p.d.dtype, at(p.grad[c.o.dst]), p.C[t], at(p.grad[t]), written[t] ? 1 : 0, p.dims_of(t), s)) return e;
    written[t] = true;
    return 0;
  }

  int backward(const float* g_pred0, const float* g_pred1, const float* drop1, const float* drop2, float* const* grads_) {
    drops[0] = drop1; drops[1] = drop2;
    g_pred[0] = g_pred0; g_pred[1] = g_pred1;
    grads = grads_;
    if (int e = pack_all_weights(true)) return e;
    if (int e = heads_backward()) return e;
    for (int i = kNumOps - 1; i >= 0; --i) {
      if (decoder_done && i == kG.first_up) {
        SEUNET_HIP(hipEventRecord(decoder_done, s));
      }
      const Op c = op(i);
      const OpKind k = c.o.kind;
      if (int e = k == OP_GATED ? gated_backward(c) : k == OP_CAT ? cat_backward(c) : k == OP_POOL ? pool_backward(c) : up_backward(c))
        return e;
    }
    if (!zero_ptrs.empty()) {
      mark("stats");
      if (int e = launch_multi_zero(zero_ptrs.data(), zero_counts.data(), (int)zero_ptrs.size(), s)) return e;
    }
    if (grad_x) {
      mark("input_grad:ec1");
      if (int e = launch_input_grad(p.d.dtype, at(p.grad[T_E0]), p.C[T_E0], par(0, P_CONV1_W), at(p.feat[T_X0]), p.d.in_channel,
                                    gxl(0), gxl(1), grad_x, p.dims[0], s)) return e;
    }
    mark("outside");
    return 0;
  }
};

}
}

using namespace seunet;

extern "C" {

int seunet_net_param_count(const seunet_net_desc* desc) {
  return desc ? kNumParams : -1;
}

int seunet_net_param_info(const seunet_net_desc* desc, int index, char* name, int name_cap, int* shape5, int* ndim) {
  SEUNET_CHECK(desc && name && shape5 && ndim, "param_info: null argument");
  SEUNET_CHECK(index >= 0 && index < kNumParams, "param_info: index %d out of range", index);
  const seunet_net_desc& d = *desc;
  const ParamDesc& q = kG.param[index];
  snprintf(name, (size_t)name_cap, "%s.%s", q.block, kFieldName[q.f]);
  const int ci = q.cin ? q.cin * d.width_mult : d.in_channel, co = q.cout * d.width_mult;
  const int shapes[][5] = {{co, ci, q.k, q.k, q.k}, {co}, {2, co, 1, 1, 1}, {2}, {1, co, 1, 1, 1}, {1, co, 1, 1, 1},
                           {d.n_classes, q.cin, 1, 1, 1}, {d.n_classes}};
  for (int k = 0; k < 5; ++k) shape5[k] = shapes[q.f][k];
  *ndim = shapes[q.f][1] ? 5 : 1;
  return 0;
}

size_t seunet_net_workspace_bytes(const seunet_net_desc* desc) {
  Plan p;
  return desc && p.init(*desc) == 0 ? p.total : 0;
}

int seunet_debug_net_layout(const seunet_net_desc* desc, int index, char* name, int cap, size_t* offset, size_t* bytes) {
  SEUNET_CHECK(desc && name && offset && bytes, "debug_net_layout: null argument");
  Plan p;
  if (int e = p.init(*desc)) return e;
  if (index < 0 || index >= (int)p.log.size()) return 1;
  const Take& t = p.log[index];
  snprintf(name, (size_t)cap, "%s%s%s", t.what, t.of[0] ? ":" : "", t.of);
  *offset = t.off;
  *bytes = t.bytes;
  return 0;
}

int seunet_net_forward(const seunet_net_desc* desc, const float* const* params, const float* x, const float* drop1,
                       const float* drop2, float* pred0, float* pred1, void* workspace, size_t workspace_bytes,
                       seunet_stream_t s) {
  SEUNET_CHECK(x && pred1, "net_forward: null tensor");
  Exec ex;
  if (int e = ex.setup(desc, params, workspace, workspace_bytes, (hipStream_t)s)) return e;
  return ex.forward(x, drop1, drop2, pred0, pred1);
}

struct NetGraph {
  hipGraph_t graph = nullptr;
  hipGraphExec_t exec = nullptr;
};

int seunet_net_forward_capture(const seunet_net_desc* desc, const float* const* params, const float* x, const float* drop1,
                               const float* drop2, float* pred0, float* pred1, void* workspace, size_t workspace_bytes,
                               seunet_stream_t s, void** graph_out) {
  SEUNET_CHECK(x && pred1 && graph_out, "net_forward_capture: null argument");
  SEUNET_CHECK(s != nullptr, "net_forward_capture: stream capture needs a stream other than the null stream");
  SEUNET_CHECK(!prof_on(), "net_forward_capture: switch the launch-group timer off before capturing");
  *graph_out = nullptr;
  Exec ex;
  if (int e = ex.setup(desc, params, workspace, workspace_bytes, (hipStream_t)s)) return e;
  SEUNET_CHECK(device_zero_page() != nullptr, "net_forward_capture: zero page allocation failed");
  SEUNET_HIP(hipStreamBeginCapture((hipStream_t)s, hipStreamCaptureModeThreadLocal));
  const int rc = ex.forward(x, drop1, drop2, pred0, pred1);
  NetGraph* g = new NetGraph;
  const hipError_t e_end = hipStreamEndCapture((hipStream_t)s, &g->graph);
  if (rc != 0 || e_end != hipSuccess) {
    if (g->graph) (void)hipGraphDestroy(g->graph);
    delete g;
    if (rc != 0) return rc;
    return fail("net_forward_capture: hipStreamEndCapture failed: %s", hipGetErrorString(e_end));
  }
  const hipError_t e_inst = hipGraphInstantiate(&g->exec, g->graph, nullptr, nullptr, 0);
  if (e_inst != hipSuccess) {
    (void)hipGraphDestroy(g->graph);
    delete g;
    return fail("net_forward_capture: hipGraphInstantiate failed: %s", hipGetErrorString(e_inst));
  }
  *graph_out = g;
  return 0;
}

int seunet_graph_launch(void* graph, seunet_stream_t s) {
  SEUNET_CHECK(graph != nullptr, "graph_launch: null graph");
  SEUNET_HIP(hipGraphLaunch(static_cast<NetGraph*>(graph)->exec, (hipStream_t)s));
  return 0;
}

int seunet_graph_destroy(void* graph) {
  if (!graph) return 0;
  NetGraph* g = static_cast<NetGraph*>(graph);
  if (g->exec) (void)hipGraphExecDestroy(g->exec);
  if (g->graph) (void)hipGraphDestroy(g->graph);
  delete g;
  return 0;
}

int seunet_net_read_tensor(const seunet_net_desc* desc, const float* const* params, const void* workspace, size_t workspace_bytes,
                           const char* name, int which, float* out, int* channels, seunet_stream_t s) {
  SEUNET_CHECK(desc && workspace && name && out, "net_read_tensor: null argument");
  Plan p;
  int i;
  bool xbranch;
  if (int e = plan_and_find(*desc, -1, name, &p, &i, &xbranch)) return e;
  SEUNET_CHECK(workspace_bytes >= p.total, "net_read_tensor: workspace too small");
  SEUNET_CHECK(i >= 0, "net_read_tensor: no block named %s", name);
  const unsigned char* ws = reinterpret_cast<const unsigned char*>(workspace);
  const OpDesc& o = kOps[i];
  const OpRes& r = p.op[i];
  const Dims& dm = p.dims_of(o.dst);
  const size_t raw = xbranch ? r.raw2 : r.raw, mean = xbranch ? r.mean2 : r.mean, rstd = xbranch ? r.rstd2 : r.rstd;
  SEUNET_CHECK(!xbranch || (which >= 0 && which <= 2), "net_read_tensor: which=%d is not stored for an x-branch", which);
  if (channels) *channels = which == 3 ? p.C[o.dst] : r.cout;
  if (xbranch && which == 0 && p.fuse_x) {
    SEUNET_CHECK(params != nullptr, "net_read_tensor: the recomputed x-branch %s needs the parameter list", name);
    const float* w = params[kG.prm[i].xw];
    SEUNET_CHECK(w, "net_read_tensor: no weight for %s", name);
    return launch_xbranch_values(p.d.dtype, ws + p.feat[o.xsrc], w, r.cout, p.d.in_channel, out, dm, (hipStream_t)s);
  }
// ... 85 lines not shown
```

### se-unet-airseg_amd/csrc/seunet_common.h

```cpp
#pragma once
#include <hip/hip_runtime.h>
#include <stdint.h>
#include <string>

#define SEUNET_F32 0
#define SEUNET_BF16 1
#define SEUNET_F16 2

typedef __bf16 bf16_t;
typedef _Float16 f16_t;

namespace seunet {

void set_error(const std::string& msg);
const char* get_error();
int fail(const char* fmt, ...);
bool prof_on();
void prof_mark(const char* tag, hipStream_t s);

#define SEUNET_CHECK(cond, ...)                       \
  do {                                                \
    if (!(cond)) return ::seunet::fail(__VA_ARGS__);  \
  } while (0)

// ... 173 lines not shown
  asm volatile("v_mov_b32 %0, %0\n\tv_mov_b32 %1, %1" : "+v"(lo), "+v"(hi));
  return ((unsigned long long)hi << 32) | lo;
}
__device__ __forceinline__ double dpp_settle(double v) {
  return __builtin_bit_cast(double, dpp_settle(__builtin_bit_cast(unsigned long long, v)));
}
template <typename V> __device__ __forceinline__ V shfl_xor_settled(V v, int off) { return dpp_settle(__shfl_xor(v, off, 64)); }
template <int CTRL> __device__ __forceinline__ int dpp_fetch_bits(int v) {
  return __builtin_amdgcn_update_dpp(0, v, CTRL, 0xF, 0xF, true);
}
template <int CTRL> __device__ __forceinline__ float dpp_fetch(float v) {
  return __builtin_bit_cast(float, dpp_fetch_bits<CTRL>(__builtin_bit_cast(int, v)));
}
template <int LPV> __device__ __forceinline__ float group_sum(float v) {
  static_assert(LPV == 1 || LPV == 2 || LPV == 4 || LPV == 8 || LPV == 16, "group_sum: LPV must be 1..16");
  if (LPV >= 2) v += dpp_fetch<0xB1>(v);
  if (LPV >= 4) v += dpp_fetch<0x4E>(v);
  if (LPV >= 8) v += dpp_fetch<0x141>(v);
  if (LPV >= 16) v += dpp_fetch<0x140>(v);
  return LPV >= 2 ? dpp_settle(v) : v;
}
template <int LPV> __device__ __forceinline__ float stride_sum(float v) {
#pragma unroll
  for (int off = 32; off >= LPV; off >>= 1) v += shfl_xor_settled(v, off);
  return v;
}
template <int LPV> __device__ __forceinline__ double stride_sum_d(double v) {
#pragma unroll
  for (int off = 32; off >= LPV; off >>= 1) v += shfl_xor_settled(v, off);
  return v;
}
#endif

int launch_pack_input(int dtype, const float* x_ncdhw, int in_channel, void* out_cl8, Dims d, hipStream_t s);
int launch_unpack_cl(int dtype, const void* in_cl, int C, float* out_ncdhw, Dims d, hipStream_t s);
int launch_pack_cl(int dtype, const float* in_ncdhw, int C, void* out_cl, int Cpad, Dims d, hipStream_t s);

size_t conv_wpack_bytes(int dtype, int taps, int cin, int cout);
int launch_conv_pack_weights(int dtype, const float* w_torch, int taps, int cin_w, int cout_w,
                             int transpose_flip, void* wpack, hipStream_t s);
int conv_stats_tiles(Dims d, int taps, int dil);
struct ConvPackJob { const float* w; void* wpack; int taps, cin_w, cout_w, tflip; };
int launch_conv_pack_weights_multi(int dtype, const ConvPackJob* jobs, int n, hipStream_t s);
int launch_conv_igemm(int dtype, int taps, int dil, const SrcList& src, int cin_logical,
                      const void* wpack, const float* bias, const DstList& dst,
                      double* stats_partial, Dims d, hipStream_t s);
int launch_conv_naive(int dtype, int taps, int dil, const SrcList& src, int cin_logical,
                      const float* w_torch, int transpose_flip, const float* bias,
                      const DstList& dst, Dims d, hipStream_t s);

bool conv_stream_supported(int dtype, int taps, int dil, int src_c, int dst_c);
size_t conv_stream_wpack_bytes(int src_c);
int conv_stream_slots(Dims d, int dil);
int launch_conv_stream_pack(int dtype, const float* w, int cin_w, int cout_w, int tflip, int src_c, int dst_c, void* wpack, hipStream_t s);
struct StreamPackJob { const float* w; void* wpack; int cin_w, cout_w, tflip, src_c, dst_c; };
int launch_conv_stream_pack_multi(int dtype, const StreamPackJob* jobs, int n, hipStream_t s);
int launch_conv_stream(int dtype, int dil, const void* src, int src_c, const void* wpack, const float* bias, void* dst, int dst_c,
                       int dst_accumulate, double* stats, Dims d, hipStream_t s);

bool conv_march_supported(int dtype, int taps, int dil, const SrcList& src, const DstList& dst);
size_t conv_march_wpack_bytes(int cin_e, int cout_e);
int conv_march_slots(Dims d, int dil, int cin_e, int cout_e);
int launch_conv_march_pack(int dtype, const float* w, int cin_w, int cout_w, int tflip, int cin_e, int cout_e, void* wpack, hipStream_t s);
struct MarchPackJob { const float* w; void* wpack; int cin_w, cout_w, tflip, cin_e, cout_e; };
int launch_conv_march_pack_multi(int dtype, const MarchPackJob* jobs, int n, hipStream_t s);
int launch_conv_march(int dtype, int dil, const SrcList& src, const void* wpack, const float* bias, const DstList& dst, double* stats,
                      Dims d, hipStream_t s);

enum class ConvKernel { Naive, Tiled, Stream, March, Wgrad1x1 };


int launch_xgrad_contract(int dtype, const void* d2, int C, const float* w2, int in_channel, float* gx, int accumulate, Dims d,
                          hipStream_t s);
int launch_xgrad_unpool(int dtype, const void* x_fine, int in_channel, const float* gx_coarse, float* gx_fine, Dims fine, hipStream_t s);
int launch_input_grad(int dtype, const void* draw, int ce, const float* w_ec1, const void* x0, int in_channel, const float* gx0,
                      const float* gx1, float* grad_x, Dims d, hipStream_t s);
int launch_maxpool_fwd(int dtype, const void* in, int C, void* out, Dims din, hipStream_t s);
int launch_maxpool_bwd(int dtype, const void* in, const void* g_out, int C, void* g_in,
                       int accumulate, Dims din, hipStream_t s);
int launch_upsample2_fwd(int dtype, const void* in, int C, void* out, Dims din, hipStream_t s);
int launch_upsample2_bwd(int dtype, const void* g_out, int C, void* g_in, int accumulate,
                         Dims din, hipStream_t s);
int upsample2_form(int dtype, int C, Dims din, bool backward);
int launch_multi_zero(float* const* ptrs, const int* counts, int n, hipStream_t s);
int class_max();
int class_grad_records(Dims d);
int launch_side_to_level(const float* side, const float* head_w, int wstride, const float* drop, int drop_stride, int K, float* level,
                         int accumulate, Dims d, hipStream_t s);
int launch_level_to_side_grad(const float* glev, long long cstride, long long nstride, const float* side, const float* head_w, int wstride,
                              const float* drop, int drop_stride, int K, float* g_side, double* partial, float* dhead, Dims d,
                              hipStream_t s);
int launch_class_bias_grad(const float* per_sample, int N, int K, float* out, hipStream_t s);
int launch_crop_batch(const void* img, int img_dtype, const unsigned char* label, const void* weight, int w_dtype,
                      const unsigned char* skel, int D, int H, int W, int cube, int ncrop, const int* starts, const int* aug,
                      double weight_exponent, int f64_math, float* data_out, float* label_out, float* weight_out, float* skel_out,
                      hipStream_t s);
int launch_hu_two_channel(const void* img, int img_dtype, long long nvox, int f64_math, float* out, hipStream_t s);
int launch_window_gather(const float* vol, int C, int X, int Y, int Z, int cube, int nwin, const int* starts, float* out, hipStream_t s);
int launch_window_accumulate(const float* logits, int apply_sigmoid, int nwin, const int* starts, int cube, double* acc, int X, int Y,
                             int Z, hipStream_t s);
int launch_window_finalize(const double* acc, int X, int Y, int Z, int cube, int nx, const int* xs, int ny, const int* ys, int nz,
                           const int* zs, int dup0, double* out, hipStream_t s);
int launch_adamw(float* const* params, const float* const* grads, float* const* exp_avg, float* const* exp_avg_sq,
                 const long long* counts, int n, double lr, double beta1, double beta2, double eps, double weight_decay,
                 int step, int maximize, hipStream_t s);
int launch_adamw_gated(float* const* params, const float* const* grads, float* const* exp_avg, float* const* exp_avg_sq,
                       const long long* counts, const int* steps, float* const* skipped, int n, double lr, double beta1,
                       double beta2, double eps, double weight_decay, int maximize, const int* flag, float* table, hipStream_t s);
int configure_kernel_lds(unsigned long long& mask, const void* fn, int bytes);
const void* device_zero_page();
int launch_side_upsample(const float* side, int C, int scale, float* out_ncdhw, int c_total,
                         int c_off, Dims dlow, hipStream_t s);
int launch_head_fwd(const float* const* level_maps, int nlevels, const float* bias, float* pred,
                    Dims d0, hipStream_t s);
int launch_head_bwd(const float* g_pred, float* const* g_levels, int nlevels, float* tmp,
                    float* g_bias, Dims d0, hipStream_t s);
size_t head_bwd_tmp_floats(Dims d0);

#define SEUNET_LOSS_NSUMS 7
int loss_partials();
int launch_loss_sums(const float* pred, int apply_sigmoid, const float* target,
                     const float* weight, const float* skel, long long n, float* partial,
                     double* sums, hipStream_t s, int terms = 7);
int launch_loss_value(const double* sums0, double c_dice0, double c_gul0, double c_atr0, const double* sums1, double c_dice1,
                      double c_gul1, double c_atr1, float* value, hipStream_t s);
int launch_loss_grad(const float* pred, int apply_sigmoid, const float* target,
                     const float* weight, const float* skel, long long n, const double* sums,
                     float c_dice, float c_gul, float c_atr, float g_scale,
                     const float* g_scale_dev, float* g_pred, hipStream_t s);
int loss_sample_partials(int batch);
int launch_loss_sums_per_sample(const float* pred, int apply_sigmoid, const float* target, const float* weight, const float* skel,
                                int batch, long long n, float* partial, double* sums, int terms, hipStream_t s);
int launch_loss_sample_values(const double* sums, int batch, double c_dice, double c_gul, double c_atr, float* values, hipStream_t s);
#define SEUNET_POOL_MAX_CAPACITY 65535
#define SEUNET_POOL_MAX_BATCH 1024
#define SEUNET_POOL_MAX_GATHER 32
int launch_pool_select(const float* new_keys, int batch, float* keys, long long* seq, long long* state, int capacity, int* slots_out,
                       hipStream_t s);
int launch_pool_scatter(const int* slots_dev, int batch, int capacity, long long voxels, const float* data, const float* label,
                        const float* weight, const float* skel, float* pool_data, unsigned char* pool_label, float* pool_weight,
                        unsigned char* pool_skel, hipStream_t s);
int launch_pool_gather(const int* slots_host, int n, int capacity, long long voxels, const float* pool_data,
                       const unsigned char* pool_label, const float* pool_weight, const unsigned char* pool_skel, float* data_out,
                       float* label_out, float* weight_out, float* skel_out, hipStream_t s);
}
```

### se-unet-airseg_amd/csrc/wgrad.h

```cpp
#pragma once
#include "seunet_common.h"

namespace seunet {

bool wgrad_stream_supported(int dtype, int taps, int dil, int x_c, int dy_c);
size_t wgrad_stream_workspace_bytes(int x_c, int dy_c, int dil, Dims d);
int launch_wgrad_stream(int dtype, int dil, const void* x, int x_c, int cin_w, const void* dy, int dy_c, int cout_w, float* dw,
                        void* workspace, size_t ws_bytes, Dims d, hipStream_t s);

static constexpr int WG_TILED_SLABS = 512;
size_t wgrad_workspace_bytes(int taps, int cin, int cout);
int launch_wgrad(int dtype, int taps, int dil, const SrcList& x, int cin_logical, const void* dy,
                 int cout, float* dw_torch, void* workspace, size_t ws_bytes, Dims d, hipStream_t s);
bool wgrad_march_supported(int dtype, int taps, int dil, const SrcList& x, int cin_logical, int cout, Dims d, long long src_dist);
int launch_wgrad_march(int dtype, int taps, int dil, const SrcList& x, int cin_logical, const void* dy, int cout,
                       float* dw, void* workspace, size_t ws_bytes, Dims d, hipStream_t s);
size_t wgrad_march_workspace_bytes(int taps, int cin, int cout);
bool wgrad_1x1_supported(int dtype, const SrcList& x, int cin_logical, int cout);
int launch_wgrad_1x1(int dtype, const SrcList& x, int cin_logical, const void* dy, int cout, float* dw, void* workspace,
                     size_t ws_bytes, Dims d, hipStream_t s);
size_t wgrad_1x1_workspace_bytes(int cin, int cout);
int launch_wgrad_naive(int dtype, int taps, int dil, const SrcList& x, int cin_logical,
                       const void* dy, int cout, float* dw_torch, Dims d, hipStream_t s);
ConvKernel wgrad_kernel(int dtype, int taps, int dil, const SrcList& x, int cin_logical, int cout, Dims d, long long src_dist);
int run_wgrad(ConvKernel k, int dtype, int taps, int dil, const SrcList& x, int cin_logical, const void* dy, int cout, float* dw,
              void* workspace, size_t ws_bytes, Dims d, hipStream_t s);

static constexpr size_t WG_SLAB_PREFIX = 256;
struct WgSlabs {
  size_t prefix, nslab, per;
  size_t bytes() const { return prefix + nslab * per * sizeof(float); }
  float* base(void* workspace, size_t ws_bytes) const {
    return ws_bytes >= bytes() ? reinterpret_cast<float*>(reinterpret_cast<unsigned char*>(workspace) + prefix) : nullptr;
  }
};

#ifdef __HIPCC__
template <typename Map>
__global__ void __launch_bounds__(256)
wgrad_reduce_kernel(const float* __restrict__ slab, int nslab, int per, Map map, float* __restrict__ dw) {
  const int el = threadIdx.x & 15, part = threadIdx.x >> 4;
  const int e = blockIdx.x * 16 + el;
  const int combo = blockIdx.y;
  double s0 = 0.0, s1 = 0.0;
  if (e < per) {
    const float* p = slab + (size_t)combo * nslab * per + e;
    int k = part;
    for (; k + 16 < nslab; k += 32) {
      s0 += (double)p[(size_t)k * per];
      s1 += (double)p[(size_t)(k + 16) * per];
    }
    if (k < nslab) s0 += (double)p[(size_t)k * per];
  }
  __shared__ double red[16][17];
  red[part][el] = s0 + s1;
  __syncthreads();
  if (part == 0 && e < per) {
    const long long i = map(combo, e);
    if (i >= 0) {
      double t = red[0][el];
#pragma unroll
      for (int q = 1; q < 16; ++q) t += red[q][el];
      dw[i] = (float)t;
    }
  }
}

template <typename Map>
static int launch_wgrad_reduce(const float* slab, int nslab, int per, int combos, Map map, float* dw, hipStream_t s) {
  wgrad_reduce_kernel<Map><<<dim3(cdiv(per, 16), combos), 256, 0, s>>>(slab, nslab, per, map, dw);
  SEUNET_LAUNCH_CHECK();
  return 0;
}
#endif

}
```

### se-unet-airseg_amd/csrc/wgrad.hip

```cpp
#include "seunet_common.h"
#include "mfma.h"
#include "wgrad.h"
#include <climits>
#include <cstdlib>

namespace seunet {

extern unsigned long long* g_conv_debug;

struct WgArgs {
  const void* src0; const void* src1; const void* src2;
  int srcC0, srcC1, srcC2;
  int cum1, cum2;
  int cin;
  const void* dy; int cout;
  float* slab;
  const void* zero;
  int N, D, H, W;
  int tx, ty, tz;
  int co_tiles;
  unsigned long long* debug;
};

template <typename T> struct WgTile;
// ... 211 lines not shown
      load_a(std::integral_constant<int, 1>{});
      static_for<NSTEP>([&](auto st_c) __attribute__((always_inline)) {
        constexpr int ST = decltype(st_c)::value, ti = ST % NT, ri = ST / NT;
        load_a(std::integral_constant<int, ST + 2>{});
        if constexpr (ti == 0) load_b(std::integral_constant<int, ri + 1>{});
        __builtin_amdgcn_sched_barrier(0);
#pragma unroll
        for (int ab = 0; ab < 2; ++ab) {
          const bf16x8 afr = frag_join(abuf[ST % 3][ab][0], abuf[ST % 3][ab][1]);
#pragma unroll
          for (int bb = 0; bb < 2; ++bb) {
            const bf16x8 bfr = frag_join(bbuf[ri % 2][bb][0], bbuf[ri % 2][bb][1]);
            const int q = 4 * (2 * ab + bb);
            f32x4 c = {acc[ti][q], acc[ti][q + 1], acc[ti][q + 2], acc[ti][q + 3]};
            c = mfma_16x16x32<T>(afr, bfr, c);
            acc[ti][q] = c[0]; acc[ti][q + 1] = c[1]; acc[ti][q + 2] = c[2]; acc[ti][q + 3] = c[3];
          }
        }
        __builtin_amdgcn_sched_barrier(0);
      });
    } else {
      for (int row = 0; row < TZ * TY; ++row) {
        if (TAPS == 1 && (row % NW) != wave) continue;
        const int lz = row / TY, ly = row % TY;
        const int xrow = (lz * HY + ly) * HX;
        const int yrow = row * TX;
        const int pl = col >> 2, sub = (col & 3) * 4;
#pragma unroll 4
        for (int kk = 0; kk < 16; ++kk) {
          const int xo = 2 * kk + h;
          const float bfr = *reinterpret_cast<const float*>(ys + pl * YPL + (yrow + xo) * 16 + sub);
#pragma unroll
          for (int ti = 0; ti < NT; ++ti) {
            const float afr = *reinterpret_cast<const float*>(xs + pl * XPL + (xrow + tapoff[ti] + xo) * 16 + sub);
            acc[ti] = __builtin_amdgcn_mfma_f32_32x32x2f32(afr, bfr, acc[ti], 0, 0, 0);
          }
        }
      }
    }
    WSTAMP(4);
  }
  if (TAPS == 27) {
    float* out = a.slab + ((size_t)combo * gridDim.x + blockIdx.x) * (27 * 1024);
#pragma unroll
    for (int ti = 0; ti < NT; ++ti) {
      const int tap = wave + NW * ti;
      if (tap < 27) {
#pragma unroll
        for (int r = 0; r < 16; ++r) {
          const int row = sizeof(T) == 4 ? (r & 3) + 8 * (r >> 2) + 4 * h : 16 * (r >> 3) + 4 * (lane >> 4) + (r & 3);
          const int cc = sizeof(T) == 4 ? col : 16 * ((r >> 2) & 1) + (lane & 15);
          out[(tap * 32 + row) * 32 + cc] = acc[ti][r];
        }
      }
    }
  } else {
    __syncthreads();
    float* part = reinterpret_cast<float*>(smem);
#pragma unroll
    for (int r = 0; r < 16; ++r) {
      const int row = sizeof(T) == 4 ? (r & 3) + 8 * (r >> 2) + 4 * h : 16 * (r >> 3) + 4 * (lane >> 4) + (r & 3);
      const int cc = sizeof(T) == 4 ? col : 16 * ((r >> 2) & 1) + (lane & 15);
      part[wave * 1024 + row * 32 + cc] = acc[0][r];
    }
    __syncthreads();
    float* out = a.slab + ((size_t)combo * gridDim.x + blockIdx.x) * 1024;
    for (int e = tid; e < 1024; e += NW * 64) {
      float t = part[e];
#pragma unroll
      for (int w = 1; w < NW; ++w) t += part[w * 1024 + e];
      out[e] = t;
    }
  }
#ifdef SEUNET_STAMP
  WSTAMP(5);
  if (a.debug != nullptr && lane == 0) {
    const size_t w = ((size_t)blockIdx.y * gridDim.x + blockIdx.x) * NW + wave;
    for (int i = 0; i < 6; ++i) a.debug[w * 12 + i] = ph[i];
    for (int i = 6; i < 12; ++i) a.debug[w * 12 + i] = 0;
  }
#endif
}

struct WgMap {
  int taps, cin_w, cout_w, co_tiles;
  __device__ long long operator()(int combo, int e) const {
    const int tap = e >> 10, ci = (combo / co_tiles) * 32 + ((e >> 5) & 31), co = (combo % co_tiles) * 32 + (e & 31);
    return ci < cin_w && co < cout_w ? (long long)(((size_t)co * cin_w + ci) * taps + tap) : -1;
  }
};

static inline int wgrad_groups(int combos, int total_tiles) {
  int g = WG_TILED_SLABS / combos;
  if (g < 16) g = 16;
  if (g > WG_TILED_SLABS) g = WG_TILED_SLABS;
  if (g > total_tiles) g = total_tiles;
  if (g < 1) g = 1;
  return g;
}
static WgSlabs wgrad_tiled_slabs(int taps, int combos, int groups) {
  return {WG_SLAB_PREFIX, (size_t)combos * groups, (size_t)taps * 1024};
}

size_t wgrad_workspace_bytes(int taps, int cin, int cout) {
  const int combos = cdiv(cin, 32) * cdiv(cout, 32);
  const size_t tiled = wgrad_tiled_slabs(taps, combos, wgrad_groups(combos, INT_MAX)).bytes();
  const size_t other = taps == 1 ? wgrad_1x1_workspace_bytes(cin, cout) : wgrad_march_workspace_bytes(taps, cin, cout);
  return tiled > other ? tiled : other;
}

int run_wgrad(ConvKernel k, int dtype, int taps, int dil, const SrcList& x, int cin_logical, const void* dy, int cout, float* dw,
              void* workspace, size_t ws_bytes, Dims d, hipStream_t s) {
  switch (k) {
    case ConvKernel::Naive: return launch_wgrad_naive(dtype, taps, dil, x, cin_logical, dy, cout, dw, d, s);
    case ConvKernel::Tiled: return launch_wgrad(dtype, taps, dil, x, cin_logical, dy, cout, dw, workspace, ws_bytes, d, s);
    case ConvKernel::Stream:
      return launch_wgrad_stream(dtype, dil, x.ptr[0], x.C[0], cin_logical, dy, cout, cout, dw, workspace, ws_bytes, d, s);
    case ConvKernel::March: return launch_wgrad_march(dtype, taps, dil, x, cin_logical, dy, cout, dw, workspace, ws_bytes, d, s);
    case ConvKernel::Wgrad1x1: return launch_wgrad_1x1(dtype, x, cin_logical, dy, cout, dw, workspace, ws_bytes, d, s);
  }
  return fail("wgrad: unknown kernel %d", (int)k);
}

template <typename T, int TAPS, int DIL, int NW>
static int wgrad_launch_one(const WgArgs& a, dim3 grid, hipStream_t s) {
  constexpr int HALO = (TAPS == 27) ? 1 : 0;
  constexpr int TZ = WgTile<T>::TZ, TY = WgTile<T>::TY;
  constexpr int PPV = 32 / (16 / (int)sizeof(T));
  constexpr int NVH = (TZ + 2 * HALO) * (TY + 2 * HALO) * (32 + 2 * HALO), NVT = TZ * TY * 32;
  constexpr int LDS = PPV * ((((NVH + 63) / 64) * 64 + 4) + (((NVT + 63) / 64) * 64 + 4)) * 16 + NW * 64 * 32;
  static unsigned long long configured = 0;
  if (int e = configure_kernel_lds(configured, reinterpret_cast<const void*>(&wgrad_kernel<T, TAPS, DIL, NW>), LDS)) return e;
  wgrad_kernel<T, TAPS, DIL, NW><<<grid, NW * 64, LDS, s>>>(a);
  SEUNET_LAUNCH_CHECK();
  return 0;
}

static void wg_sources(WgArgs& a, const SrcList& x, int cin_logical) {
  a.src0 = x.ptr[0]; a.srcC0 = x.C[0];
  a.src1 = x.n > 1 ? x.ptr[1] : nullptr; a.srcC1 = x.n > 1 ? x.C[1] : 0;
  a.src2 = x.n > 2 ? x.ptr[2] : nullptr; a.srcC2 = x.n > 2 ? x.C[2] : 0;
  a.cin = cin_logical;
  a.cum1 = x.n > 1 ? x.C[0] : x.total();
  a.cum2 = x.n > 2 ? x.C[0] + x.C[1] : x.total();
}

int launch_wgrad(int dtype, int taps, int dil, const SrcList& x, int cin_logical, const void* dy, int cout,
                 float* dw, void* workspace, size_t ws_bytes, Dims d, hipStream_t s) {
  SEUNET_CHECK(taps == 27 || taps == 1, "wgrad: taps=%d unsupported", taps);
  SEUNET_CHECK(taps == 1 || dil == 1 || dil == 2, "wgrad: dilation %d unsupported", dil);
  SEUNET_CHECK(x.n >= 1 && x.n <= 3, "wgrad: 1..3 sources");
  SEUNET_CHECK(cout % 8 == 0 && cin_logical >= 1 && cin_logical <= x.total(), "wgrad: bad channel counts");
  WgArgs a{};
  wg_sources(a, x, cin_logical);
  a.dy = dy; a.cout = cout;
  a.zero = device_zero_page();
  SEUNET_CHECK(a.zero != nullptr, "wgrad: cannot allocate the device zero page");
  a.N = d.N; a.D = d.D; a.H = d.H; a.W = d.W;
  const int tz = dtype_size(dtype) == 2 ? WgTile<bf16_t>::TZ : WgTile<float>::TZ;
  const int ty = dtype_size(dtype) == 2 ? WgTile<bf16_t>::TY : WgTile<float>::TY;
  const int st = taps == 27 ? dil : 1;
  a.tx = cdiv(cdiv(d.W, st), 32); a.ty = cdiv(cdiv(d.H, st), ty); a.tz = cdiv(cdiv(d.D, st), tz);
  a.co_tiles = cdiv(cout, 32);
  a.debug = g_conv_debug;
  const int combos = cdiv(cin_logical, 32) * a.co_tiles;
  const int G = wgrad_groups(combos, a.tx * a.ty * a.tz * st * st * st * d.N);
  a.slab = wgrad_tiled_slabs(taps, combos, G).base(workspace, ws_bytes);
  SEUNET_CHECK(a.slab != nullptr, "wgrad: workspace too small");
  dim3 grid(G, combos);
  int e;
  SEUNET_DTYPE_SWITCH(dtype, {
    if (taps == 1) e = wgrad_launch_one<T, 1, 1, 4>(a, grid, s);
    else if (dil == 1) e = wgrad_launch_one<T, 27, 1, 4>(a, grid, s);
    else e = wgrad_launch_one<T, 27, 2, 4>(a, grid, s);
  });
  if (e) return e;
  return launch_wgrad_reduce(a.slab, G, taps * 1024, combos, WgMap{taps, cin_logical, cout, a.co_tiles}, dw, s);
}

template <typename T>
__global__ void wgrad_naive_kernel(WgArgs a, int taps, int dil, float* __restrict__ dw, long long total) {
  const long long V = (long long)a.D * a.H * a.W;
  const int t3 = taps == 27 ? 3 : 1, c = taps == 27 ? 1 : 0;
  for (long long i = blockIdx.x * (long long)blockDim.x + threadIdx.x; i < total;
       i += (long long)gridDim.x * blockDim.x) {
    const int tap = (int)(i % taps);
    const int ci = (int)((i / taps) % a.cin);
    const int co = (int)(i / ((long long)taps * a.cin));
    const int dz = (tap / (t3 * t3) - c) * dil, dy = ((tap / t3) % t3 - c) * dil, dx = (tap % t3 - c) * dil;
    const void* sp = a.src0; int sC = a.srcC0, cc = ci;
    if (ci >= a.cum2) { sp = a.src2; sC = a.srcC2; cc = ci - a.cum2; }
    else if (ci >= a.cum1) { sp = a.src1; sC = a.srcC1; cc = ci - a.cum1; }
    double s = 0.0;
    for (int n = 0; n < a.N; ++n)
      for (int z = 0; z < a.D; ++z) {
        const int zz = z + dz;
        if ((unsigned)zz >= (unsigned)a.D) continue;
        for (int y = 0; y < a.H; ++y) {
          const int yy = y + dy;
          if ((unsigned)yy >= (unsigned)a.H) continue;
          for (int x = 0; x < a.W; ++x) {
            const int xx = x + dx;
            if ((unsigned)xx >= (unsigned)a.W) continue;
            const float xv = to_f32(reinterpret_cast<const T*>(sp)[(n * V + ((long long)zz * a.H + yy) * a.W + xx) * sC + cc]);
            const float gv = to_f32(reinterpret_cast<const T*>(a.dy)[(n * V + ((long long)z * a.H + y) * a.W + x) * a.cout + co]);
            s += (double)xv * (double)gv;
          }
        }
      }
    dw[i] = (float)s;
  }
}

int launch_wgrad_naive(int dtype, int taps, int dil, const SrcList& x, int cin_logical, const void* dy, int cout,
                       float* dw, Dims d, hipStream_t s) {
  WgArgs a{};
  wg_sources(a, x, cin_logical);
  a.dy = dy; a.cout = cout;
  a.N = d.N; a.D = d.D; a.H = d.H; a.W = d.W;
  const long long total = (long long)cout * cin_logical * taps;
  const int grid = (int)((total + 63) / 64);
  SEUNET_DTYPE_SWITCH(dtype, wgrad_naive_kernel<T><<<grid, 64, 0, s>>>(a, taps, dil, dw, total));
  SEUNET_LAUNCH_CHECK();
  return 0;
}

}
```

### se-unet-airseg_amd/csrc/wgrad_1x1.hip

```cpp
#include "seunet_common.h"
#include "lds_dma.h"
#include "mfma.h"
#include "wgrad.h"
#include <cstdlib>

namespace seunet {

struct W1Args {
  const void* src[3]; int srcC[3]; int nsrc;
  const void* dy; int cout;
  float* slab; const void* zero;
  long long nvox;
  int nchunk;
  int nst;
};

static constexpr int W1_NW = 4;

template <typename T, int CIBW, int NCOB, int CH>
__global__ void __launch_bounds__(256)
wgrad_1x1_kernel(W1Args a) {
  constexpr int KS = CH / 32;
  extern __shared__ __attribute__((aligned(16))) unsigned char smem[];
  const unsigned lds_base = (unsigned)(size_t)(__attribute__((address_space(3))) unsigned char*)smem;
// ... 43 lines not shown
#pragma unroll
  for (int it = 0; it < MAXI; ++it) {
    const int id = wave + W1_NW * it;
    const int byte = id * 1024 + lane * 16;
    int sel, C, rel;
    if (byte >= yoff0) { sel = 3; C = a.cout; rel = byte - yoff0; }
    else if (a.nsrc > 2 && byte >= roff[2]) { sel = 2; C = a.srcC[2]; rel = byte - roff[2]; }
    else if (a.nsrc > 1 && byte >= roff[1]) { sel = 1; C = a.srcC[1]; rel = byte - roff[1]; }
    else { sel = 0; C = a.srcC[0]; rel = byte; }
    const int sh = 31 - __clz(C * 2);
    const int v = rel >> sh, slot = (rel & (C * 2 - 1)) >> 4;
    const int piece = slot ^ tr16_swz(C / 8, v);
    plan[it] = (it < items && id < ni) ? ((unsigned)sel | ((unsigned)((v << sh) + piece * 16) << 4) | ((unsigned)v << 20)) : 0xFFFFFFFFu;
  }
  const unsigned char* zero_page = reinterpret_cast<const unsigned char*>(a.zero) + lane * 16;
  const unsigned char* tb[4] = {reinterpret_cast<const unsigned char*>(a.src[0]), reinterpret_cast<const unsigned char*>(a.nsrc > 1 ? a.src[1] : a.src[0]),
                                reinterpret_cast<const unsigned char*>(a.nsrc > 2 ? a.src[2] : a.src[0]), reinterpret_cast<const unsigned char*>(a.dy)};
  const long long tstride[4] = {(long long)CH * a.srcC[0] * 2, (long long)CH * a.srcC[1] * 2, (long long)CH * a.srcC[2] * 2, (long long)CH * a.cout * 2};
  auto issue = [&](int chunk, int st) __attribute__((always_inline)) {
    const bool cok = chunk < a.nchunk;
    const long long left = a.nvox - (long long)chunk * CH;
    const unsigned char* cb[4];
#pragma unroll
    for (int t = 0; t < 4; ++t) cb[t] = tb[t] + (long long)(cok ? chunk : 0) * tstride[t];
#pragma unroll
    for (int it = 0; it < MAXI; ++it) {
      if (it < LW) {
        const unsigned w = plan[it];
        const int sel = w & 3, v = (w >> 20) & 0xFF;
        const unsigned char* base = sel == 0 ? cb[0] : (sel == 1 ? cb[1] : (sel == 2 ? cb[2] : cb[3]));
        const bool ok = cok && w != 0xFFFFFFFFu && v < left;
        const unsigned char* gp = ok ? base + ((w >> 4) & 0xFFFF) : zero_page;
        const int id = wave + W1_NW * it;
        dma16(gp, (it < items && id < ni) ? lds_base + (unsigned)(st * stage + id * 1024) : lds_base + (unsigned)dump);
      }
    }
  };

  f32x4 acc[CIBW][NCOB];
#pragma unroll
  for (int c = 0; c < CIBW; ++c)
#pragma unroll
    for (int k = 0; k < NCOB; ++k) acc[c][k] = f32x4{0.f, 0.f, 0.f, 0.f};

  const int nst = a.nst, PF = nst - 1;
  int chunk = blockIdx.x, st = 0, stp = 0;
  for (int k = 0; k < PF; ++k) { issue(chunk + k * (int)gridDim.x, stp); stp = stp + 1 == nst ? 0 : stp + 1; }
  for (; chunk < a.nchunk; chunk += gridDim.x) {
    issue(chunk + PF * (int)gridDim.x, stp);
    stp = stp + 1 == nst ? 0 : stp + 1;
    switch (PF * LW) {
      case 8: wait_loads<8>(); break;
      case 16: wait_loads<16>(); break;
      case 24: wait_loads<24>(); break;
      case 32: wait_loads<32>(); break;
      case 48: wait_loads<48>(); break;
      default: wait_loads<0>(); break;
    }
    __builtin_amdgcn_s_barrier();
    const unsigned sb = lds_base + (unsigned)(st * stage);
#pragma unroll
    for (int ks = 0; ks < KS; ++ks) {
      bf16x8 xf[CIBW], yf[NCOB];
#pragma unroll
      for (int c = 0; c < CIBW; ++c) xf[c] = frag_tr16(sb + xoff[c][ks][0], sb + xoff[c][ks][1]);
#pragma unroll
      for (int k = 0; k < NCOB; ++k) yf[k] = frag_tr16(sb + yoff[k][ks][0], sb + yoff[k][ks][1]);
#pragma unroll
      for (int c = 0; c < CIBW; ++c)
#pragma unroll
        for (int k = 0; k < NCOB; ++k) acc[c][k] = mfma_16x16x32<T>(yf[k], xf[c], acc[c][k]);
    }
    __builtin_amdgcn_s_barrier();
    st = st + 1 == nst ? 0 : st + 1;
  }
  wait_loads<0>();

  float* out = a.slab + ((size_t)blockIdx.x * W1_NW + wave) * (CIBW * NCOB * 256) + lane * 4;
#pragma unroll
  for (int c = 0; c < CIBW; ++c)
#pragma unroll
    for (int k = 0; k < NCOB; ++k) *reinterpret_cast<f32x4*>(out + (c * NCOB + k) * 256) = acc[c][k];
}

struct W1Map {
  int cibw, ncob, cin;
  __device__ long long operator()(int, int e) const {
    const int comp = e & 3, lane = (e >> 2) & 63, pair = e >> 8;
    const int kk = pair % ncob, c = (pair / ncob) % cibw, wave = pair / (ncob * cibw);
    const int co = kk * 16 + 4 * (lane >> 4) + comp;
    const int ci = (wave * cibw + c) * 16 + (lane & 15);
    return ci < cin ? (long long)((size_t)co * cin + ci) : -1;
  }
};

struct W1Cfg { int cibw, ncob, ch, nst; };
static bool wgrad_1x1_cfg(int dtype, const SrcList& x, int cin_logical, int cout, W1Cfg& c) {
  if (dtype_size(dtype) != 2 || x.n < 1 || x.n > 3 || cin_logical != x.total()) return false;
  for (int i = 0; i < x.n; ++i) if (x.C[i] != 32 && x.C[i] != 64) return false;
  if (cout != 32 && cout != 64 && cout != 128) return false;
  const int ncib = cin_logical / 16;
  c.cibw = (ncib + W1_NW - 1) / W1_NW;
  c.ncob = cout / 16;
  if (ncib != W1_NW * c.cibw || c.cibw * c.ncob > 24) return false;
  if (!((c.cibw == 1 && c.ncob == 2) || (c.cibw == 2 && c.ncob == 4) || (c.cibw == 3 && c.ncob == 8))) return false;
  c.ch = 128; c.nst = 0;
  for (int ch = 128; ch >= 64 && c.nst < 3; ch /= 2) {
    const int stage = (cin_logical + cout) * 2 * ch;
    const int items = (stage / 1024 + W1_NW - 1) / W1_NW, lw = items <= 8 ? 8 : (items <= 16 ? 16 : 24);
    if (items > 24) continue;
    int nst = (159 * 1024) / stage;
    if (nst > 4) nst = 4;
    while (nst > 2 && (nst - 1) * lw > 48) --nst;
    if (nst >= 2 && nst > c.nst) { c.nst = nst; c.ch = ch; }
  }
  return c.nst >= 2;
}
bool wgrad_1x1_supported(int dtype, const SrcList& x, int cin_logical, int cout) {
  W1Cfg c;
  return wgrad_1x1_cfg(dtype, x, cin_logical, cout, c);
}

static constexpr int W1_MAX_WG = 256;
static size_t w1_slab_floats(int cin, int cout) { return (size_t)W1_NW * cdiv(cin, 64) * cdiv(cout, 16) * 256; }
static WgSlabs w1_slabs(int groups, int cin, int cout) { return {WG_SLAB_PREFIX, (size_t)groups, w1_slab_floats(cin, cout)}; }
struct W1Cut { long long nvox; int nchunk, groups; };
static W1Cut w1_cut(const W1Cfg& c, Dims d) {
  W1Cut m;
  m.nvox = (long long)d.N * d.vox();
  m.nchunk = (int)((m.nvox + c.ch - 1) / c.ch);
  m.groups = m.nchunk < W1_MAX_WG ? m.nchunk : W1_MAX_WG;
  return m;
}
size_t wgrad_1x1_workspace_bytes(int cin, int cout) { return w1_slabs(W1_MAX_WG, cin, cout).bytes(); }

template <typename T, int CIBW, int NCOB, int CH>
static int wgrad_1x1_launch(const W1Args& a, int grid, int lds, hipStream_t s) {
  static unsigned long long configured = 0;
  if (int e = configure_kernel_lds(configured, reinterpret_cast<const void*>(&wgrad_1x1_kernel<T, CIBW, NCOB, CH>), lds)) return e;
  wgrad_1x1_kernel<T, CIBW, NCOB, CH><<<grid, 256, lds, s>>>(a);
  SEUNET_LAUNCH_CHECK();
  return 0;
}

int launch_wgrad_1x1(int dtype, const SrcList& x, int cin_logical, const void* dy, int cout, float* dw, void* workspace,
                     size_t ws_bytes, Dims d, hipStream_t s) {
  W1Cfg c;
  SEUNET_CHECK(wgrad_1x1_cfg(dtype, x, cin_logical, cout, c),
               "wgrad_1x1: 16-bit tensors, 1..3 sources of 32 or 64 channels (64, 128 or 192 together), 32 / 64 / 128 output channels only");
  const W1Cut cut = w1_cut(c, d);
  const WgSlabs slabs = w1_slabs(cut.groups, cin_logical, cout);
  W1Args a{};
  a.slab = slabs.base(workspace, ws_bytes);
  SEUNET_CHECK(a.slab != nullptr, "wgrad_1x1: workspace too small");
  for (int i = 0; i < 3; ++i) { a.src[i] = i < x.n ? x.ptr[i] : nullptr; a.srcC[i] = i < x.n ? x.C[i] : 0; }
  a.nsrc = x.n;
  a.dy = dy; a.cout = cout;
  a.zero = device_zero_page();
  SEUNET_CHECK(a.zero != nullptr, "wgrad_1x1: cannot allocate the device zero page");
  a.nvox = cut.nvox;
  a.nchunk = cut.nchunk;
  const int grid = cut.groups;
  const int lds = (cin_logical + cout) * 2 * c.ch * c.nst + 1024;
  a.nst = c.nst;
  int e = -1;
  SEUNET_DTYPE_SWITCH(dtype, if constexpr (sizeof(T) == 2) {
    if (c.cibw == 1 && c.ch == 128) e = wgrad_1x1_launch<T, 1, 2, 128>(a, grid, lds, s);
    else if (c.cibw == 1) e = wgrad_1x1_launch<T, 1, 2, 64>(a, grid, lds, s);
    else if (c.cibw == 2 && c.ch == 128) e = wgrad_1x1_launch<T, 2, 4, 128>(a, grid, lds, s);
    else if (c.cibw == 2) e = wgrad_1x1_launch<T, 2, 4, 64>(a, grid, lds, s);
    else if (c.ch == 128) e = wgrad_1x1_launch<T, 3, 8, 128>(a, grid, lds, s);
    else e = wgrad_1x1_launch<T, 3, 8, 64>(a, grid, lds, s);
  });
  if (e) return e;
  return launch_wgrad_reduce(a.slab, grid, (int)slabs.per, 1, W1Map{c.cibw, c.ncob, cin_logical}, dw, s);
}

}
```

### se-unet-airseg_amd/csrc/wgrad_march.hip

```cpp
#include "seunet_common.h"
#include "lds_dma.h"
#include "mfma.h"
#include "wgrad.h"
#include <cstdlib>

namespace seunet {

struct WmArgs {
  const void* src0; const void* src1;
  int srcC, nsrc;
  const void* dy; int cout;
  float* slab;
  int N, D, H, W;
  int nyb, nxb, nseg, zsteps;
  int nco;
  int items;
};

static constexpr int WM_TX = 32, WM_RY = 4, WM_HXP = 36, WM_NW = 4, WM_XRING = 3, WM_YRING = 5;

template <int NCB, int NOB, int DIL> struct WmGeo {
  static constexpr int XC = 16 * NCB, YC = 16 * NOB;
  static constexpr int NPX = XC / 8, NPY = YC / 8, VBX = XC * 2, VBY = YC * 2;
  static constexpr int PW = NCB * NOB / WM_NW;
// ... 169 lines not shown
#pragma unroll
          for (int r = 0; r < 2; ++r) ya[tz][k][r] = pb + yoff[k][r];
      }
    };
    bf16x8 xf[2][3];
    bf16x8 yw[RY][3][PW];
    auto load_frag = [&](auto i_c, auto f_c) __attribute__((always_inline)) {
      constexpr int i = decltype(i_c)::value, f = decltype(f_c)::value;
      constexpr int hy = wm_row<DIL, HY>(i);
      if constexpr (f < 3) xf[i & 1][f] = frag_tr16(xa[f][0] + hy * ROWBX, xa[f][1] + hy * ROWBX);
      else {
        constexpr int tz = (f - 3) / PW, k = (f - 3) % PW;
        yw[hy][tz][k] = frag_tr16(ya[tz][k][0] + hy * ROWBY, ya[tz][k][1] + hy * ROWBY);
      }
    };
    auto mfma_one = [&](auto i_c, auto m_c) __attribute__((always_inline)) {
      constexpr int i = decltype(i_c)::value, m = decltype(m_c)::value;
      constexpr int hy = wm_row<DIL, HY>(i);
      constexpr int ty = wm_tap_y<DIL>(hy, m / (9 * PW));
      constexpr int rem = m % (9 * PW), tz = rem / (3 * PW), dx = (rem / PW) % 3, k = rem % PW;
      constexpr int r = hy - DIL * ty;
      static_assert(r >= 0 && r < RY, "row pairing");
      mfma_16x16x32_pinned<T>(acc[k][(tz * 3 + ty) * 3 + dx], yw[r][tz][k], xf[i & 1][dx]);
    };
    auto row = [&](auto i_c, auto nx_c, auto&& extra) __attribute__((always_inline)) {
      constexpr int i = decltype(i_c)::value, nx = decltype(nx_c)::value;
      constexpr int NF = wm_row_frags<DIL, HY, PW>(nx), NM = wm_row_mfmas<DIL, HY, PW>(i);
      extra();
      static_for<NF>([&](auto g_c) __attribute__((always_inline)) {
        constexpr int g = decltype(g_c)::value;
        load_frag(nx_c, g_c);
        static_for<(g + 1) * NM / NF - g * NM / NF>([&](auto j_c) __attribute__((always_inline)) {
          mfma_one(i_c, std::integral_constant<int, g * NM / NF + decltype(j_c)::value>{});
        });
        __builtin_amdgcn_sched_barrier(0);
      });
    };

    wait_loads<0>();
    __syncthreads();
    if (nsteps == 0) continue;
    {
      const PlaneRef p0 = plane_of(0, 0, 0), p1 = plane_of(1, 1, 1);
      static_for<LOADS_PER_STEP>([&](auto it_c) __attribute__((always_inline)) { issue_item(p0, it_c); });
      static_for<LOADS_PER_STEP>([&](auto it_c) __attribute__((always_inline)) { issue_item(p1, it_c); });
    }
    wait_loads<LOADS_PER_STEP>();
    __builtin_amdgcn_s_barrier();
    int xs = 0, ys = 0;
    set_addr(0, 0, 0);
    static_for<wm_row_frags<DIL, HY, PW>(0)>([&](auto f_c) __attribute__((always_inline)) { load_frag(std::integral_constant<int, 0>{}, f_c); });
    for (int s = 0; s < nsteps; ++s) {
      const int xs2 = xs + 2 >= WM_XRING ? xs + 2 - WM_XRING : xs + 2;
      const int ys2 = ys + 2 >= WM_YRING ? ys + 2 - WM_YRING : ys + 2;
      const PlaneRef pr = plane_of(s + 2, xs2, ys2);
      static_for<HY - 1>([&](auto i_c) __attribute__((always_inline)) {
        constexpr int i = decltype(i_c)::value;
        row(i_c, std::integral_constant<int, i + 1>{}, [&]() __attribute__((always_inline)) {
          static_for<LOADS_PER_STEP>([&](auto it_c) __attribute__((always_inline)) {
            constexpr int it = decltype(it_c)::value;
            if constexpr ((it * (HY - 1)) / LOADS_PER_STEP == i) issue_item(pr, it_c);
          });
        });
      });
      asm volatile("s_waitcnt lgkmcnt(0)" ::: "memory");
      wait_loads<LOADS_PER_STEP>();
      __builtin_amdgcn_s_barrier();
      xs = xs + 1 == WM_XRING ? 0 : xs + 1;
      ys = ys + 1 == WM_YRING ? 0 : ys + 1;
      set_addr(s + 1, xs, ys);
      row(std::integral_constant<int, HY - 1>{}, std::integral_constant<int, 0>{}, []() {});
    }
  }
  asm volatile("s_nop 15\n\ts_nop 15" ::: "memory");
  wait_loads<0>();

  float* out = a.slab + ((size_t)(blockIdx.y * gridDim.x + blockIdx.x) * (WM_NW * PW) + wave * PW) * (27 * 256) + lane * 4;
#pragma unroll
  for (int k = 0; k < PW; ++k)
#pragma unroll
    for (int t = 0; t < 27; ++t) *reinterpret_cast<f32x4*>(out + (k * 27 + t) * 256) = acc[k][t];
}

struct WmMap {
  int ncb, pw, xc, yc, nco, cin_w;
  __device__ long long operator()(int combo, int e) const {
    const int comp = e & 3, lane = (e >> 2) & 63, tap = (e >> 8) % 27, pair = e / (27 * 256);
    const int wave = pair / pw, kk = pair % pw;
    const int cib = wave % ncb, cob = (wave / ncb) * pw + kk;
    const int co = (combo % nco) * yc + cob * 16 + 4 * (lane >> 4) + comp;
    const int ci = (combo / nco) * xc + cib * 16 + (lane & 15);
    return (long long)(((size_t)co * cin_w + ci) * 27 + tap);
  }
};

struct WmCfg { int ncb, nob; };
static WmCfg wm_blocks(int cin, int cout) {
  if (cin % 64 == 0) return {4, 2};
  if (cout % 64 == 0) return {2, 4};
  return {2, 2};
}

static constexpr int WM_MAX_WG = 256;
struct WmCut {
  int xc, yc, pw, nco, combos, gmax;
  int nyb, nxb, nseg, zsteps, items, groups;
  size_t slab_floats() const { return (size_t)WM_NW * pw * 27 * 256; }
  WgSlabs slabs(int g) const { return {WG_SLAB_PREFIX, (size_t)combos * g, slab_floats()}; }
};
static WmCut wm_channels(const WmCfg& c, int cin, int cout) {
  WmCut m{};
  m.xc = 16 * c.ncb; m.yc = 16 * c.nob; m.pw = c.ncb * c.nob / WM_NW;
  m.nco = cout / m.yc;
  m.combos = (cin / m.xc) * m.nco;
  m.gmax = WM_MAX_WG / m.combos < 1 ? 1 : WM_MAX_WG / m.combos;
  return m;
}
static WmCut wm_cut(const WmCfg& c, int cin, int cout, Dims d, int dil) {
  WmCut m = wm_channels(c, cin, cout);
  m.nyb = cdiv(d.H, WM_RY); m.nxb = cdiv(d.W, WM_TX);
  const int nplanes = cdiv(d.D, dil);
  const int per_seg = d.N * dil * m.nyb * m.nxb;
  m.nseg = 1;
  while (per_seg * m.nseg < m.gmax && nplanes / (m.nseg * 2) >= 8) m.nseg *= 2;
  m.zsteps = cdiv(nplanes, m.nseg);
  m.items = per_seg * m.nseg;
  m.groups = m.items < m.gmax ? m.items : m.gmax;
  return m;
}
static_assert(WM_NW * 256 == 32 * 32 && 2 * WM_MAX_WG <= WG_TILED_SLABS,
              "a marching launch's WgSlabs fit those of the tiled kernel for the same channels");
size_t wgrad_march_workspace_bytes(int taps, int cin, int cout) {
  if (taps != 27 || cin < 32 || cout < 32 || cin % 32 || cout % 32) return 0;
  const WmCut m = wm_channels(wm_blocks(cin, cout), cin, cout);
  return m.slabs(m.gmax).bytes();
}
static bool wgrad_march_cfg(int dtype, int taps, int dil, const SrcList& x, int cin_logical, int cout, Dims d, long long src_dist, WmCfg& c) {
  if (dtype_size(dtype) != 2 || taps != 27 || (dil != 1 && dil != 2)) return false;
  if (x.n < 1 || x.n > 2 || (x.n == 2 && x.C[0] != x.C[1])) return false;
  if (cin_logical != x.total() || cin_logical % 32 || cout % 32 || x.C[0] % 8) return false;
  {
    const long long esz = 2, xs = (long long)d.D * d.H * d.W * x.C[0] * esz, ys = (long long)d.D * d.H * d.W * cout * esz;
    const long long dist = x.n == 2 ? (src_dist < 0 ? -src_dist : src_dist) : 0;
    if (dist + xs >= 0xFFFFFFFFll || ys >= 0xFFFFFFFFll) return false;
  }
  c = wm_blocks(cin_logical, cout);
  return true;
}

bool wgrad_march_supported(int dtype, int taps, int dil, const SrcList& x, int cin_logical, int cout, Dims d, long long src_dist) {
  WmCfg c;
  return wgrad_march_cfg(dtype, taps, dil, x, cin_logical, cout, d, src_dist, c);
}

template <typename T, int NCB, int NOB, int DIL>
static int wgrad_march_launch(const WmArgs& a, dim3 grid, hipStream_t s) {
  using Geo = WmGeo<NCB, NOB, DIL>;
  static unsigned long long configured = 0;
  if (int e = configure_kernel_lds(configured, reinterpret_cast<const void*>(&wgrad_march_kernel<T, NCB, NOB, DIL>), Geo::LDS)) return e;
  wgrad_march_kernel<T, NCB, NOB, DIL><<<grid, 256, Geo::LDS, s>>>(a);
  SEUNET_LAUNCH_CHECK();
  return 0;
}

int launch_wgrad_march(int dtype, int taps, int dil, const SrcList& x, int cin_logical, const void* dy, int cout,
                       float* dw, void* workspace, size_t ws_bytes, Dims d, hipStream_t s) {
  WmCfg c;
  SEUNET_CHECK(wgrad_march_cfg(dtype, taps, dil, x, cin_logical, cout, d, x.gap(), c),
               "wgrad_march: 16-bit 3x3x3 layers with 32k input and 32k output channels (one tensor or two equal halves) only");
  const WmCut cut = wm_cut(c, cin_logical, cout, d, dil);
  WmArgs a{};
  a.slab = cut.slabs(cut.groups).base(workspace, ws_bytes);
  SEUNET_CHECK(a.slab != nullptr, "wgrad_march: workspace too small");
  a.src0 = x.ptr[0]; a.src1 = x.n > 1 ? x.ptr[1] : nullptr; a.srcC = x.C[0]; a.nsrc = x.n;
  a.dy = dy; a.cout = cout;
  a.N = d.N; a.D = d.D; a.H = d.H; a.W = d.W;
  a.nyb = cut.nyb; a.nxb = cut.nxb; a.nseg = cut.nseg; a.zsteps = cut.zsteps;
  a.nco = cut.nco; a.items = cut.items;
  const dim3 grid(cut.groups, cut.combos);
  int e = -1;
  SEUNET_DTYPE_SWITCH(dtype, if constexpr (sizeof(T) == 2) {
    if (c.ncb == 4 && dil == 1) e = wgrad_march_launch<T, 4, 2, 1>(a, grid, s);
    else if (c.ncb == 4) e = wgrad_march_launch<T, 4, 2, 2>(a, grid, s);
    else if (c.nob == 4 && dil == 1) e = wgrad_march_launch<T, 2, 4, 1>(a, grid, s);
    else if (c.nob == 4) e = wgrad_march_launch<T, 2, 4, 2>(a, grid, s);
    else if (dil == 1) e = wgrad_march_launch<T, 2, 2, 1>(a, grid, s);
    else e = wgrad_march_launch<T, 2, 2, 2>(a, grid, s);
  });
  if (e) return e;
  return launch_wgrad_reduce(a.slab, cut.groups, (int)cut.slab_floats(), cut.combos,
                             WmMap{c.ncb, cut.pw, cut.xc, cut.yc, cut.nco, cin_logical}, dw, s);
}

}
```

### se-unet-airseg_amd/csrc/wgrad_stream.hip

```cpp
#include "seunet_common.h"
#include "lds_dma.h"
#include "mfma.h"
#include "wgrad.h"

namespace seunet {

struct WsArgs {
  const void* x; const void* dy; float* slab;
  int N, D, H, W;
  int nyb, nxb, nzseg, zsteps;
};

static constexpr int WS_TY = 8, WS_TX = 32, WS_NW = 8, WS_PF = 2;

template <int CIN, int COUT, int DIL> struct WsGeo {
  static constexpr bool XF = CIN == 8;
  static constexpr int NP = CIN / 8;
  static constexpr int HX = WS_TX + 2 * DIL + (XF ? DIL : 0), HY = WS_TY + 2 * DIL;
  static constexpr int NVP = HX * HY, G = (NVP + 63) / 64;
  static constexpr int PS = G * 1024, XPLANE = NP * PS;
  static constexpr int YPLANE = WS_TY * WS_TX * COUT * 2, NDY = YPLANE / 1024;
  static constexpr int RX = WS_PF + 2, RY = WS_PF + 4;
  static constexpr int XITEMS = (NP * G + WS_NW - 1) / WS_NW, YITEMS = (NDY + WS_NW - 1) / WS_NW;
  static constexpr int LOADS_PER_STEP = XITEMS + YITEMS;
// ... 118 lines not shown
#pragma unroll
      for (int dzi = 0; dzi < 3; ++dzi) {
        int ysl = ys0 + (2 - dzi);
        ysl = ysl >= RY ? ysl - RY : ysl;
        const unsigned char* yp = smem + Geo::YOFF + ysl * YPLANE + yfrag0 + (w * WS_TX) * COUT * 2;
#pragma unroll
        for (int ob = 0; ob < OB; ++ob) bf[dzi][ob] = read_y(yp + ob * 32);
      }
      dma_group(s + WS_PF, xs_pf, s + 2 + WS_PF, ys_pf, r);
#pragma unroll
      for (int u = 0; u < AUG; ++u) {
        const int au = grp * AUG + u;
        if (au >= AU) continue;
        int dyi, dxo, cb;
        if constexpr (XF) { dyi = au >> 1; dxo = 2 * (au & 1); cb = 0; }
        else { dyi = au / (3 * CB); dxo = (au / CB) % 3; cb = au % CB; }
        const bf16x8 af = read_x(xp + ((w + DIL * dyi) * HX + DIL * dxo) * 16 + (XF ? 0 : cb * 2 * PS));
#pragma unroll
        for (int dzi = 0; dzi < 3; ++dzi)
#pragma unroll
          for (int ob = 0; ob < OB; ++ob)
            acc[u][dzi][ob] = mfma_16x16x32<T>(af, bf[dzi][ob], acc[u][dzi][ob]);
      }
    }
  };

  int ysl = 0;
  static_for<YITEMS>([&](auto i_c) __attribute__((always_inline)) { dma_y(0, 0, i_c); dma_y(1, 1, i_c); });
#pragma unroll
  for (int k = 0; k < WS_PF; ++k) dma_group(k, k, k + 2, k + 2, 2);
  wait_loads<(WS_PF - 1) * Geo::LOADS_PER_STEP>();
  __builtin_amdgcn_s_barrier();
  int xs = 0, xs_pf = WS_PF, ys_pf = 2 + WS_PF;
  for (int s = 0; s < nsteps; ++s) {
    if (s > 0) {
      wait_loads<(WS_PF - 1) * Geo::LOADS_PER_STEP>();
      __builtin_amdgcn_s_barrier();
    }
    compute(s, xs, ysl, xs_pf, ys_pf);
    xs = xs == RX - 1 ? 0 : xs + 1;
    xs_pf = xs_pf == RX - 1 ? 0 : xs_pf + 1;
    ysl = ysl == RY - 1 ? 0 : ysl + 1;
    ys_pf = ys_pf == RY - 1 ? 0 : ys_pf + 1;
  }
  wait_loads<0>();
  __syncthreads();

  float* slab = a.slab + (((size_t)blockIdx.z * gridDim.y + blockIdx.y) * gridDim.x + blockIdx.x) * (size_t)Geo::SLAB;
  f32x4* stage = reinterpret_cast<f32x4*>(smem);
  constexpr int TILES = AUG * 3 * OB, ROUND = 8;
#pragma unroll
  for (int t0 = 0; t0 < TILES; t0 += ROUND) {
#pragma unroll
    for (int k = 0; k < ROUND; ++k) {
      const int tl = t0 + k;
      if (tl < TILES) stage[(wave * ROUND + k) * 64 + lane] = acc[tl / (3 * OB)][(tl / OB) % 3][tl % OB];
    }
    __syncthreads();
#pragma unroll
    for (int j = 0; j < 2; ++j) {
      const int idx = tid + 512 * j;
      const int gg = idx >> 9, k = (idx >> 6) & 7, ln = idx & 63;
      const int tl = t0 + k, u = tl / (3 * OB), dzi = (tl / OB) % 3, ob = tl % OB;
      const int au = gg * AUG + u;
      if (tl < TILES && au < AU) {
        f32x4 sum = stage[((gg + 0) * ROUND + k) * 64 + ln];
#pragma unroll
        for (int p = 1; p < 4; ++p) sum += stage[((gg + 2 * p) * ROUND + k) * 64 + ln];
        const int co = ob * 16 + (ln & 15);
#pragma unroll
        for (int e = 0; e < 4; ++e) {
          const int cl = 4 * (ln >> 4) + e;
          int dyi, dxi, ci;
          if constexpr (XF) { dyi = au >> 1; dxi = 2 * (au & 1) + (cl >> 3); ci = cl & 7; }
          else { dyi = au / (3 * CB); dxi = (au / CB) % 3; ci = (au % CB) * 16 + cl; }
          if (dxi < 3 && ci < CIN && co < COUT) slab[(((dzi * 3 + dyi) * 3 + dxi) * CIN + ci) * COUT + co] = sum[e];
        }
      }
    }
    __syncthreads();
  }
}

struct WsMap {
  int cin, cout, cin_w, cout_w;
  __device__ long long operator()(int, int e) const {
    const int co = e % cout, ci = (e / cout) % cin, tap = e / (cout * cin);
    return ci < cin_w && co < cout_w ? (long long)(((size_t)co * cin_w + ci) * 27 + tap) : -1;
  }
};

static bool ws_shape_ok(int cin, int cout, int dil) {
  if (cin == 32 && cout == 16) return dil == 1;
  return (cin == 8 && (cout == 8 || cout == 16)) || (cin == 16 && cout == 32) || (cin == 16 && cout == 16);
}
bool wgrad_stream_supported(int dtype, int taps, int dil, int x_c, int dy_c) {
  return (dtype == SEUNET_BF16 || dtype == SEUNET_F16) && taps == 27 && (dil == 1 || dil == 2) && ws_shape_ok(x_c, dy_c, dil);
}
struct WsCut {
  int planes, zsteps, nzseg, nyb, nxb, dil, n;
  int slabs() const { return nyb * nxb * nzseg * dil * n; }
  dim3 grid() const { return dim3(nyb * nxb, nzseg * dil, n); }
};
static WsCut ws_cut(Dims d, int dil) {
  WsCut c;
  c.dil = dil; c.n = d.N;
  c.planes = cdiv(d.D, dil);
  c.nyb = cdiv(d.H, WS_TY); c.nxb = cdiv(d.W, WS_TX);
  const int base = c.nyb * c.nxb * d.N * dil;
  int segs = (256 + base - 1) / base;
  if (segs < 1) segs = 1;
  if (segs > cdiv(c.planes, 8)) segs = cdiv(c.planes, 8);
  if (segs < 1) segs = 1;
  c.zsteps = cdiv(c.planes, segs);
  c.nzseg = cdiv(c.planes, c.zsteps);
  return c;
}
static WgSlabs ws_slabs(const WsCut& c, int x_c, int dy_c) { return {0, (size_t)c.slabs(), (size_t)(27 * x_c * dy_c)}; }
size_t wgrad_stream_workspace_bytes(int x_c, int dy_c, int dil, Dims d) { return ws_slabs(ws_cut(d, dil), x_c, dy_c).bytes(); }

template <typename T, int CIN, int COUT, int DIL>
static int ws_launch_t(const WsArgs& a, dim3 grid, hipStream_t s) {
  using Geo = WsGeo<CIN, COUT, DIL>;
  static_assert(Geo::LDS <= 160 * 1024, "wgrad_stream: LDS budget");
  static unsigned long long configured = 0;
  if (int e = configure_kernel_lds(configured, reinterpret_cast<const void*>(&wgrad_stream_kernel<T, CIN, COUT, DIL>), Geo::LDS)) return e;
  wgrad_stream_kernel<T, CIN, COUT, DIL><<<grid, WS_NW * 64, Geo::LDS, s>>>(a);
  SEUNET_LAUNCH_CHECK();
  return 0;
}
template <int CIN, int COUT, int DIL>
static int ws_launch(int dtype, const WsArgs& a, dim3 grid, hipStream_t s) {
  return dtype == SEUNET_F16 ? ws_launch_t<f16_t, CIN, COUT, DIL>(a, grid, s) : ws_launch_t<bf16_t, CIN, COUT, DIL>(a, grid, s);
}

int launch_wgrad_stream(int dtype, int dil, const void* x, int x_c, int cin_w, const void* dy, int dy_c, int cout_w, float* dw,
                        void* workspace, size_t ws_bytes, Dims d, hipStream_t s) {
  SEUNET_CHECK(wgrad_stream_supported(dtype, 27, dil, x_c, dy_c), "wgrad_stream: unsupported shape (%d x %d channels, dilation %d)", x_c, dy_c, dil);
  SEUNET_CHECK(x && dy && dw && workspace && cin_w >= 1 && cin_w <= x_c && cout_w >= 1 && cout_w <= dy_c, "wgrad_stream: bad argument");
  const WsCut cut = ws_cut(d, dil);
  const WgSlabs slabs = ws_slabs(cut, x_c, dy_c);
  WsArgs a{};
  a.x = x; a.dy = dy; a.slab = slabs.base(workspace, ws_bytes);
  SEUNET_CHECK(a.slab != nullptr, "wgrad_stream: workspace too small");
  SEUNET_CHECK((long long)d.D * d.H * d.W * (x_c > dy_c ? x_c : dy_c) * 2 < 0xFFFFFFFFll,
               "wgrad_stream: one sample exceeds the 32-bit buffer offsets of this kernel");
  a.N = d.N; a.D = d.D; a.H = d.H; a.W = d.W;
  a.zsteps = cut.zsteps; a.nzseg = cut.nzseg; a.nyb = cut.nyb; a.nxb = cut.nxb;
  SEUNET_CHECK(d.N <= 65535, "wgrad_stream: batch too large");
  const dim3 grid = cut.grid();
  int e = 1;
  if (x_c == 8 && dy_c == 8) e = dil == 1 ? ws_launch<8, 8, 1>(dtype, a, grid, s) : ws_launch<8, 8, 2>(dtype, a, grid, s);
  else if (x_c == 8 && dy_c == 16) e = dil == 1 ? ws_launch<8, 16, 1>(dtype, a, grid, s) : ws_launch<8, 16, 2>(dtype, a, grid, s);
  else if (x_c == 16 && dy_c == 16) e = dil == 1 ? ws_launch<16, 16, 1>(dtype, a, grid, s) : ws_launch<16, 16, 2>(dtype, a, grid, s);
  else if (x_c == 16 && dy_c == 32) e = dil == 1 ? ws_launch<16, 32, 1>(dtype, a, grid, s) : ws_launch<16, 32, 2>(dtype, a, grid, s);
  else if (x_c == 32 && dy_c == 16) e = ws_launch<32, 16, 1>(dtype, a, grid, s);
  if (e) return e;
  return launch_wgrad_reduce(a.slab, cut.slabs(), (int)slabs.per, 1, WsMap{x_c, dy_c, cin_w, cout_w}, dw, s);
}

}
```

Baseline: 576.6 million.

## Defer wgrad slab reductions and piggyback them on later finalize/zero kernels

Weight-gradient slab reductions are no longer launched right after each wgrad kernel. They are recorded as a pending job and appended as extra blocks to the next gate/cat finalize, multi-zero or upsample kernel, or flushed before the next wgrad reuses the workspace. The cat backward finalize also merges its stats and x-branch finalizes into one launch, and the bias stage-2 sum rides on the upsample-transpose kernel. Together these cut the number of small kernel launches in backward. The cost is more complex control flow and an ordering dependency on the shared wgrad workspace. Parameter gradients not requested by autograd are also skipped.

After: 583.4 million, median of 6. 1.01x the previous value.

```diff
diff --git a/se-unet-airseg_amd/SE_UNet.py b/se-unet-airseg_amd/SE_UNet.py
--- a/se-unet-airseg_amd/SE_UNet.py
+++ b/se-unet-airseg_amd/SE_UNet.py
@@ -192,7 +192,8 @@
             g1 = torch.zeros(shape, dtype=torch.float32, device=dev) if g1 is None else g1.contiguous().float()
             if ctx.loss_scale != 1.0:
                 g0, g1 = g0 * ctx.loss_scale, g1 * ctx.loss_scale
-            flat, grads, split = alloc_flat_grads(ctx.plist, ctx.dead, dev, ctx.names)
+            skip = [dd or not ctx.needs_input_grad[4 + i] for i, dd in enumerate(ctx.dead)]
+            flat, grads, split = alloc_flat_grads(ctx.plist, skip, dev, ctx.names)
             garr = _lib.ptr_array(grads)
             parr = _lib.ptr_array(ctx.plist)
             sync = ctx.grad_sync
diff --git a/se-unet-airseg_amd/csrc/cat.hip b/se-unet-airseg_amd/csrc/cat.hip
--- a/se-unet-airseg_amd/csrc/cat.hip
+++ b/se-unet-airseg_amd/csrc/cat.hip
@@ -1,4 +1,5 @@
 #include "epilogue.h"
+#include "wgrad.h"
 #include <type_traits>
 
 namespace seunet {
@@ -318,11 +319,10 @@
   }
 }
 
-__global__ void __launch_bounds__(256)
-xw_finalize_kernel(const double* __restrict__ xw_partial, const double* __restrict__ stat_partial2, int slots, int C, int N,
-                   const double* __restrict__ moments, const float* __restrict__ w2, int ic, double eps, float* __restrict__ dw) {
+__device__ __forceinline__ void
+xw_finalize_body(int c, const double* __restrict__ xw_partial, const double* __restrict__ stat_partial2, int slots, int C, int N,
+                 const double* __restrict__ moments, const float* __restrict__ w2, int ic, double eps, float* __restrict__ dw) {
   const int wave = threadIdx.x >> 6, lane = threadIdx.x & 63;
-  const int c = blockIdx.x;
   __shared__ double red[4][3];
   const double wa = (double)w2[c * ic], wb = ic > 1 ? (double)w2[c * ic + 1] : 0.0;
   double g0 = 0.0, g1 = 0.0;
@@ -360,6 +360,23 @@
     dw[c * ic] = (float)g0;
     if (ic > 1) dw[c * ic + 1] = (float)g1;
   }
+}
+__global__ void __launch_bounds__(256)
+xw_finalize_kernel(const double* __restrict__ xw_partial, const double* __restrict__ stat_partial2, int slots, int C, int N,
+                   const double* __restrict__ moments, const float* __restrict__ w2, int ic, double eps, float* __restrict__ dw) {
+  xw_finalize_body(blockIdx.x, xw_partial, stat_partial2, slots, C, N, moments, w2, ic, eps, dw);
+}
+__global__ void __launch_bounds__(256)
+cat_bwd_finalize_kernel(const double* __restrict__ partial, const double* __restrict__ partial2, int slots, int C, int N,
+                        double inv_count, float* __restrict__ m1, float* __restrict__ m2, float* __restrict__ m1b,
+                        float* __restrict__ m2b, int nb2, int nxw, const double* __restrict__ xw_partial,
+                        const double* __restrict__ moments, const float* __restrict__ w2, int ic, double eps, float* __restrict__ dw,
+                        WgReduceJob rider) {
+  const int b = blockIdx.x, nb = N * C;
+  if (b < nb) stats_finalize_body(b, partial, slots, C, inv_count, 0.f, 1, m1, m2);
+  else if (b < nb + nb2) stats_finalize_body(b - nb, partial2, slots, C, inv_count, 0.f, 1, m1b, m2b);
+  else if (b < nb + nb2 + nxw) xw_finalize_body(b - nb - nb2, xw_partial, partial2, slots, C, N, moments, w2, ic, eps, dw);
+  else wgrad_reduce_body(rider, b - nb - nb2 - nxw);
 }
 
 template <typename T>
@@ -509,6 +526,21 @@
   return 0;
 }
 
+int launch_cat_bwd_finalize(const double* stat_partial, const double* stat_partial2, int slots, int C, int N, long long count,
+                            float* m1, float* m2, float* m1b, float* m2b, const CatXwFinalize& xw, hipStream_t s,
+                            const WgReduceJob* rider) {
+  SEUNET_CHECK(stat_partial && m1 && m2 && (!stat_partial2 || (m1b && m2b)), "cat_bwd_finalize: missing argument");
+  SEUNET_CHECK(!xw.dw || (stat_partial2 && xw.xw_partial && xw.moments && xw.w2 && xw.in_channel >= 1 && xw.in_channel <= 2),
+               "cat_bwd_finalize: the x-branch weight gradient needs the second branch's sums and in_channel 1 or 2");
+  const WgReduceJob job = rider ? *rider : WgReduceJob{};
+  const int nb2 = stat_partial2 ? N * C : 0, nxw = xw.dw ? C : 0;
+  cat_bwd_finalize_kernel<<<N * C + nb2 + nxw + job.blocks(), 256, 0, s>>>(
+      stat_partial, stat_partial2, slots, C, N, 1.0 / (double)count, m1, m2, m1b, m2b, nb2, nxw, xw.xw_partial, xw.moments, xw.w2,
+      xw.in_channel, (double)xw.eps, xw.dw, job);
+  SEUNET_LAUNCH_CHECK();
+  return 0;
+}
+
 int launch_xbranch_values(int dtype, const void* x_in, const float* w2, int C, int in_channel, float* out, Dims d, hipStream_t s) {
   SEUNET_CHECK(in_channel >= 1 && in_channel <= 2 && C % 8 == 0, "xbranch_values: bad argument");
   const long long total = (long long)d.N * d.vox() * (C / 8);
diff --git a/se-unet-airseg_amd/csrc/epilogue.h b/se-unet-airseg_amd/csrc/epilogue.h
--- a/se-unet-airseg_amd/csrc/epilogue.h
+++ b/se-unet-airseg_amd/csrc/epilogue.h
@@ -3,6 +3,7 @@
 
 namespace seunet {
 
+struct WgReduceJob;
 int epi_partials(Dims d);
 int launch_channel_stats(int dtype, const void* t, int C, double* partial, Dims d, hipStream_t s);
 int launch_stats_finalize(const double* partial, int slots, int C, int N, long long count,
@@ -38,7 +39,7 @@
                          hipStream_t s);
 int launch_gate_bwd_finalize(const double* stat_partial, int slots, int C, int N, long long count, float* m1, float* m2,
                              const float* pgrad_partial, int records, float* dw_se, float* dw_se2, float* dw_side,
-                             float* db_side, float* dhead_w, hipStream_t s);
+                             float* db_side, float* dhead_w, hipStream_t s, const WgReduceJob* rider = nullptr);
 int launch_pgrad_reduce(const float* pgrad_partial, int records, int C, float* dw_se,
                         float* dw_se2, float* dw_side, float* db_side, float* dhead_w,
                         hipStream_t s);
@@ -76,6 +77,10 @@
                          float eps, float* mean2, float* rstd2, double* moments_out, hipStream_t s);
 int launch_cat_xgrad_finalize(const double* xw_partial, const double* stat_partial2, int slots, const double* moments, const float* w2,
                               int C, int in_channel, int N, float eps, float* dw, hipStream_t s);
+struct CatXwFinalize { const double* xw_partial; const double* moments; const float* w2; int in_channel; float eps; float* dw; };
+int launch_cat_bwd_finalize(const double* stat_partial, const double* stat_partial2, int slots, int C, int N, long long count,
+                            float* m1, float* m2, float* m1b, float* m2b, const CatXwFinalize& xw, hipStream_t s,
+                            const WgReduceJob* rider = nullptr);
 int launch_xbranch_values(int dtype, const void* x_in, const float* w2, int C, int in_channel, float* out_ncdhw, Dims d, hipStream_t s);
 
 #ifdef __HIPCC__
diff --git a/se-unet-airseg_amd/csrc/gate.hip b/se-unet-airseg_amd/csrc/gate.hip
--- a/se-unet-airseg_amd/csrc/gate.hip
+++ b/se-unet-airseg_amd/csrc/gate.hip
@@ -1,4 +1,5 @@
 #include "epilogue.h"
+#include "wgrad.h"
 
 namespace seunet {
 
@@ -302,9 +303,11 @@
 __global__ void __launch_bounds__(256)
 gate_bwd_finalize_kernel(const double* __restrict__ partial, int slots, int C, int N, double inv_count, float* __restrict__ m1,
                          float* __restrict__ m2, const float* __restrict__ pg, int records, float* dw_se, float* dw_se2,
-                         float* dw_side, float* db_side, float* dhead_w) {
+                         float* dw_side, float* db_side, float* dhead_w, WgReduceJob rider) {
+  const int own = N * C + (4 * C + 4 + 3) / 4;
   if ((int)blockIdx.x < N * C) stats_finalize_body(blockIdx.x, partial, slots, C, inv_count, 0.f, 1, m1, m2);
-  else pgrad_reduce_body((int)blockIdx.x - N * C, pg, records, C, dw_se, dw_se2, dw_side, db_side, dhead_w);
+  else if ((int)blockIdx.x < own) pgrad_reduce_body((int)blockIdx.x - N * C, pg, records, C, dw_se, dw_se2, dw_side, db_side, dhead_w);
+  else wgrad_reduce_body(rider, (int)blockIdx.x - own);
 }
 
 int launch_sse_fwd(int dtype, const GateBlock& b, void* e_out, const SseHead& head, Dims d, hipStream_t s) {
@@ -355,9 +358,10 @@
 
 int launch_gate_bwd_finalize(const double* stat_partial, int slots, int C, int N, long long count, float* m1, float* m2,
                              const float* pgrad_partial, int records, float* dw_se, float* dw_se2, float* dw_side,
-                             float* db_side, float* dhead_w, hipStream_t s) {
-  gate_bwd_finalize_kernel<<<N * C + cdiv(4 * C + 4, 4), 256, 0, s>>>(stat_partial, slots, C, N, 1.0 / (double)count, m1, m2,
-                                                                     pgrad_partial, records, dw_se, dw_se2, dw_side, db_side, dhead_w);
+                             float* db_side, float* dhead_w, hipStream_t s, const WgReduceJob* rider) {
+  const WgReduceJob job = rider ? *rider : WgReduceJob{};
+  gate_bwd_finalize_kernel<<<N * C + cdiv(4 * C + 4, 4) + job.blocks(), 256, 0, s>>>(
+      stat_partial, slots, C, N, 1.0 / (double)count, m1, m2, pgrad_partial, records, dw_se, dw_se2, dw_side, db_side, dhead_w, job);
   SEUNET_LAUNCH_CHECK();
   return 0;
 }
diff --git a/se-unet-airseg_amd/csrc/heads.hip b/se-unet-airseg_amd/csrc/heads.hip
--- a/se-unet-airseg_amd/csrc/heads.hip
+++ b/se-unet-airseg_amd/csrc/heads.hip
@@ -303,6 +303,24 @@
   }
 }
 
+__device__ __forceinline__ void sum_stage2_wide_by_256(const double* __restrict__ partial, int n, float* __restrict__ out) {
+  __shared__ double w[16];
+#pragma unroll
+  for (int j = 0; j < 4; ++j) {
+    double s = 0.0;
+    for (int i = threadIdx.x + 256 * j; i < n; i += 1024) s += partial[i];
+#pragma unroll
+    for (int off = 32; off >= 1; off >>= 1) s += shfl_xor_settled(s, off);
+    if ((threadIdx.x & 63) == 0) w[(threadIdx.x >> 6) + 4 * j] = s;
+  }
+  __syncthreads();
+  if (threadIdx.x == 0) {
+    double t = 0.0;
+    for (int k = 0; k < 16; ++k) t += w[k];
+    out[0] = (float)t;
+  }
+}
+
 int launch_side_upsample(const float* side, int C, int scale, float* out, int c_total, int c_off, Dims dl,
                          hipStream_t s) {
   const long long total = (long long)dl.N * dl.vox() * scale * scale * scale;
@@ -332,8 +350,12 @@
 }
 
 struct AxisJob { const float* in; float* out; int I, O; long long inner, total; };
-struct AxisJobs { AxisJob j[3]; };
+struct AxisJobs { AxisJob j[3]; int njobs; const double* bias_part; int bias_n; float* g_bias; };
 __global__ void __launch_bounds__(256) up_transpose_axis_multi_kernel(AxisJobs jobs) {
+  if ((int)blockIdx.y >= jobs.njobs) {
+    if (blockIdx.x == 0) sum_stage2_wide_by_256(jobs.bias_part, jobs.bias_n, jobs.g_bias);
+    return;
+  }
   const AxisJob jb = jobs.j[blockIdx.y];
   if (jb.total == 0) return;
   const float rs = ac_scale(jb.I, jb.O);
@@ -408,11 +430,14 @@
     max_z = tz > max_z ? tz : max_z;
     ++njobs;
   }
+  jy.njobs = jz.njobs = njobs;
   if (njobs) {
-    up_transpose_axis_multi_kernel<<<dim3((unsigned)grid_for(max_y), (unsigned)njobs), 256, 0, s>>>(jy);
+    if (g_bias) { jy.bias_part = part; jy.bias_n = nblk; jy.g_bias = g_bias; }
+    up_transpose_axis_multi_kernel<<<dim3((unsigned)grid_for(max_y), (unsigned)njobs + (g_bias ? 1 : 0)), 256, 0, s>>>(jy);
     up_transpose_axis_multi_kernel<<<dim3((unsigned)grid_for(max_z), (unsigned)njobs), 256, 0, s>>>(jz);
-  }
-  if (g_bias) sum_stage2_wide_kernel<<<1, 1024, 0, s>>>(part, nblk, g_bias);
+  } else if (g_bias) {
+    sum_stage2_wide_kernel<<<1, 1024, 0, s>>>(part, nblk, g_bias);
+  }
   SEUNET_LAUNCH_CHECK();
   return 0;
 }
diff --git a/se-unet-airseg_amd/csrc/layout.hip b/se-unet-airseg_amd/csrc/layout.hip
--- a/se-unet-airseg_amd/csrc/layout.hip
+++ b/se-unet-airseg_amd/csrc/layout.hip
@@ -1,4 +1,5 @@
 #include "seunet_common.h"
+#include "wgrad.h"
 
 namespace seunet {
 
@@ -139,16 +140,19 @@
 }
 
 struct ZeroList { float* ptr[48]; int count[48]; int n; };
-__global__ void multi_zero_kernel(ZeroList z) {
+__global__ void __launch_bounds__(256) multi_zero_kernel(ZeroList z, WgReduceJob rider) {
+  if ((int)blockIdx.x >= z.n) { wgrad_reduce_body(rider, (int)blockIdx.x - z.n); return; }
   float* p = z.ptr[blockIdx.x];
   for (int i = threadIdx.x; i < z.count[blockIdx.x]; i += blockDim.x) p[i] = 0.f;
 }
-int launch_multi_zero(float* const* ptrs, const int* counts, int n, hipStream_t s) {
-  for (int base = 0; base < n; base += 48) {
+int launch_multi_zero(float* const* ptrs, const int* counts, int n, hipStream_t s, const WgReduceJob* rider) {
+  WgReduceJob job = rider ? *rider : WgReduceJob{};
+  for (int base = 0; base < n || job.blocks() > 0; base += 48) {
     ZeroList z{};
     z.n = n - base < 48 ? n - base : 48;
     for (int i = 0; i < z.n; ++i) { z.ptr[i] = ptrs[base + i]; z.count[i] = counts[base + i]; }
-    multi_zero_kernel<<<z.n, 256, 0, s>>>(z);
+    multi_zero_kernel<<<z.n + job.blocks(), 256, 0, s>>>(z, job);
+    job = WgReduceJob{};
   }
   SEUNET_LAUNCH_CHECK();
   return 0;
diff --git a/se-unet-airseg_amd/csrc/net.cpp b/se-unet-airseg_amd/csrc/net.cpp
--- a/se-unet-airseg_amd/csrc/net.cpp
+++ b/se-unet-airseg_amd/csrc/net.cpp
@@ -24,6 +24,8 @@
 }
 
 namespace {
+
+bool g_wgrad_defer = true;
 
 enum TId {
   T_NONE,
@@ -576,14 +578,26 @@
 
   float* gpar(int op, PField f) const { const int k = kG.prm[op].at[f]; return k < 0 ? nullptr : grads[k]; }
 
+  WgReduceJob pending;
+  WgReduceJob* defer() { return g_wgrad_defer ? &pending : nullptr; }
+  WgReduceJob take_pending() { const WgReduceJob j = pending; pending = WgReduceJob{}; return j; }
+  int flush_pending() {
+    if (pending.blocks() == 0) return 0;
+    mark("wgrad:flush");
+    return launch_wgrad_reduce(take_pending(), s);
+  }
+  int walk_wgrad(ConvKernel k, int taps, int dil, const SrcList& x, int cin, const void* dy, int cout, float* gw, const Dims& dm) {
+    if (int e = flush_pending()) return e;
+    return run_wgrad(k, p.d.dtype, taps, dil, x, cin, dy, cout, gw, at(p.wgrad_ws), p.wgrad_ws_bytes, dm, s, defer());
+  }
+
   int conv_backward(const Op& c) {
     const OpDesc& o = c.o;
     const OpRes& r = c.r;
     const SrcList x = srcs(c.i);
     if (float* gw = gpar(c.i, P_CONV1_W)) {
       mark("wgrad:", o.name);
-      if (int e = run_wgrad(r.wgrad, p.d.dtype, r.taps, o.dil, x, r.cin, at(p.grad[o.dst]), r.cout, gw, at(p.wgrad_ws),
-                            p.wgrad_ws_bytes, c.dm, s)) return e;
+      if (int e = walk_wgrad(r.wgrad, r.taps, o.dil, x, r.cin, at(p.grad[o.dst]), r.cout, gw, c.dm)) return e;
     }
     if (!r.need_dgrad) return 0;
     const SrcList gsrc{{at(p.grad[o.dst])}, {r.cout}, 1};
@@ -637,9 +651,10 @@
     mark("epi_bwd:", o.name);
     if (int e = launch_sse_bwd_sums(p.d.dtype, blk, g, hd, SseSums{dat(p.stats), fat(p.pgrad)}, c.dm, s)) return e;
     mark("stats");
+    const WgReduceJob rider = take_pending();
     if (int e = launch_gate_bwd_finalize(dat(p.stats), P_slots, c.r.cout, c.dm.N, c.dm.vox(), fat(p.m1), fat(p.m2), fat(p.pgrad),
                                          c.dm.N * P_slots, gpar(c.i, P_SE), gpar(c.i, P_SE2), gpar(c.i, P_CONV2_W),
-                                         gpar(c.i, P_CONV2_B), g_head, s)) return e;
+                                         gpar(c.i, P_CONV2_B), g_head, s, &rider)) return e;
     mark("in_bwd:", o.name);
     if (int e = launch_sse_bwd_apply(p.d.dtype, blk, g, hd, SseApply{fat(p.m1), fat(p.m2), at(p.grad[o.dst])}, c.dm, s)) return e;
     written[o.dst] = true;
@@ -662,12 +677,10 @@
     const CatSums sums{dat(p.stats), dat(p.stats2), recomputed && gxw ? dat(p.xwp) : nullptr};
     if (int e = launch_cat_bwd_sums(p.d.dtype, blk, g_out, pool, sums, c.dm, s)) return e;
     mark("stats");
-    if (recomputed && gxw)
-      if (int e = launch_cat_xgrad_finalize(dat(p.xwp), dat(p.stats2), P_slots, dat(r.xtot), blk.b.w2, r.cout, p.d.in_channel, c.dm.N,
-                                            p.d.eps, gxw, s)) return e;
-    if (int e = launch_stats_finalize(dat(p.stats), P_slots, r.cout, c.dm.N, c.dm.vox(), 0.f, 1, fat(p.m1), fat(p.m2), s)) return e;
-    if (two)
-      if (int e = launch_stats_finalize(dat(p.stats2), P_slots, r.cout, c.dm.N, c.dm.vox(), 0.f, 1, fat(p.m1b), fat(p.m2b), s)) return e;
+    const CatXwFinalize xwf{dat(p.xwp), dat(r.xtot), blk.b.w2, p.d.in_channel, p.d.eps, recomputed ? gxw : nullptr};
+    const WgReduceJob rider = take_pending();
+    if (int e = launch_cat_bwd_finalize(dat(p.stats), two ? dat(p.stats2) : nullptr, P_slots, r.cout, c.dm.N, c.dm.vox(), fat(p.m1),
+                                        fat(p.m2), fat(p.m1b), fat(p.m2b), xwf, s, &rider)) return e;
     mark("in_bwd:", o.name);
     CatApply ap{fat(p.m1), fat(p.m2), fat(p.m1b), fat(p.m2b), at(p.grad[o.dst]), two && !recomputed ? at(p.gx) : nullptr, nullptr, 0};
     if (recomputed && grad_x) { ap.gx_out = gxl(c.lv); ap.gx_acc = c.lv == 1 ? 1 : 0; }
@@ -679,8 +692,7 @@
       }
       if (gxw) {
         mark("wgrad:", o.xname);
-        if (int e = run_wgrad(r.x_wgrad, p.d.dtype, 1, 1, xbranch_src(o), p.d.in_channel, at(p.gx), r.cout, gxw, at(p.wgrad_ws),
-                              p.wgrad_ws_bytes, c.dm, s)) return e;
+        if (int e = walk_wgrad(r.x_wgrad, 1, 1, xbranch_src(o), p.d.in_channel, at(p.gx), r.cout, gxw, c.dm)) return e;
       }
     }
     return conv_backward(c);
@@ -723,6 +735,7 @@
     if (int e = heads_backward()) return e;
     for (int i = kNumOps - 1; i >= 0; --i) {
       if (decoder_done && i == kG.first_up) {
+        if (int e = flush_pending()) return e;
         SEUNET_HIP(hipEventRecord(decoder_done, s));
       }
       const Op c = op(i);
@@ -730,9 +743,10 @@
       if (int e = k == OP_GATED ? gated_backward(c) : k == OP_CAT ? cat_backward(c) : k == OP_POOL ? pool_backward(c) : up_backward(c))
         return e;
     }
-    if (!zero_ptrs.empty()) {
+    if (!zero_ptrs.empty() || pending.blocks() > 0) {
       mark("stats");
-      if (int e = launch_multi_zero(zero_ptrs.data(), zero_counts.data(), (int)zero_ptrs.size(), s)) return e;
+      const WgReduceJob rider = take_pending();
+      if (int e = launch_multi_zero(zero_ptrs.data(), zero_counts.data(), (int)zero_ptrs.size(), s, &rider)) return e;
     }
     if (grad_x) {
       mark("input_grad:ec1");
@@ -784,6 +798,12 @@
   *offset = t.off;
   *bytes = t.bytes;
   return 0;
+}
+
+int seunet_debug_net_wgrad_defer(int on) {
+  const int was = g_wgrad_defer ? 1 : 0;
+  g_wgrad_defer = on != 0;
+  return was;
 }
 
 int seunet_net_forward(const seunet_net_desc* desc, const float* const* params, const float* x, const float* drop1,
diff --git a/se-unet-airseg_amd/csrc/seunet_common.h b/se-unet-airseg_amd/csrc/seunet_common.h
--- a/se-unet-airseg_amd/csrc/seunet_common.h
+++ b/se-unet-airseg_amd/csrc/seunet_common.h
@@ -279,7 +279,8 @@
 int launch_upsample2_bwd(int dtype, const void* g_out, int C, void* g_in, int accumulate,
                          Dims din, hipStream_t s);
 int upsample2_form(int dtype, int C, Dims din, bool backward);
-int launch_multi_zero(float* const* ptrs, const int* counts, int n, hipStream_t s);
+struct WgReduceJob;
+int launch_multi_zero(float* const* ptrs, const int* counts, int n, hipStream_t s, const WgReduceJob* rider = nullptr);
 int class_max();
 int class_grad_records(Dims d);
 int launch_side_to_level(const float* side, const float* head_w, int wstride, const float* drop, int drop_stride, int K, float* level,
diff --git a/se-unet-airseg_amd/csrc/wgrad.h b/se-unet-airseg_amd/csrc/wgrad.h
--- a/se-unet-airseg_amd/csrc/wgrad.h
+++ b/se-unet-airseg_amd/csrc/wgrad.h
@@ -3,28 +3,30 @@
 
 namespace seunet {
 
+struct WgReduceJob;
+
 bool wgrad_stream_supported(int dtype, int taps, int dil, int x_c, int dy_c);
 size_t wgrad_stream_workspace_bytes(int x_c, int dy_c, int dil, Dims d);
 int launch_wgrad_stream(int dtype, int dil, const void* x, int x_c, int cin_w, const void* dy, int dy_c, int cout_w, float* dw,
-                        void* workspace, size_t ws_bytes, Dims d, hipStream_t s);
+                        void* workspace, size_t ws_bytes, Dims d, hipStream_t s, WgReduceJob* defer = nullptr);
 
 static constexpr int WG_TILED_SLABS = 512;
 size_t wgrad_workspace_bytes(int taps, int cin, int cout);
 int launch_wgrad(int dtype, int taps, int dil, const SrcList& x, int cin_logical, const void* dy,
-                 int cout, float* dw_torch, void* workspace, size_t ws_bytes, Dims d, hipStream_t s);
+                 int cout, float* dw_torch, void* workspace, size_t ws_bytes, Dims d, hipStream_t s, WgReduceJob* defer = nullptr);
 bool wgrad_march_supported(int dtype, int taps, int dil, const SrcList& x, int cin_logical, int cout, Dims d, long long src_dist);
 int launch_wgrad_march(int dtype, int taps, int dil, const SrcList& x, int cin_logical, const void* dy, int cout,
-                       float* dw, void* workspace, size_t ws_bytes, Dims d, hipStream_t s);
+                       float* dw, void* workspace, size_t ws_bytes, Dims d, hipStream_t s, WgReduceJob* defer = nullptr);
 size_t wgrad_march_workspace_bytes(int taps, int cin, int cout);
 bool wgrad_1x1_supported(int dtype, const SrcList& x, int cin_logical, int cout);
 int launch_wgrad_1x1(int dtype, const SrcList& x, int cin_logical, const void* dy, int cout, float* dw, void* workspace,
-                     size_t ws_bytes, Dims d, hipStream_t s);
+                     size_t ws_bytes, Dims d, hipStream_t s, WgReduceJob* defer = nullptr);
 size_t wgrad_1x1_workspace_bytes(int cin, int cout);
 int launch_wgrad_naive(int dtype, int taps, int dil, const SrcList& x, int cin_logical,
                        const void* dy, int cout, float* dw_torch, Dims d, hipStream_t s);
 ConvKernel wgrad_kernel(int dtype, int taps, int dil, const SrcList& x, int cin_logical, int cout, Dims d, long long src_dist);
 int run_wgrad(ConvKernel k, int dtype, int taps, int dil, const SrcList& x, int cin_logical, const void* dy, int cout, float* dw,
-              void* workspace, size_t ws_bytes, Dims d, hipStream_t s);
+              void* workspace, size_t ws_bytes, Dims d, hipStream_t s, WgReduceJob* defer = nullptr);
 
 static constexpr size_t WG_SLAB_PREFIX = 256;
 struct WgSlabs {
@@ -36,26 +38,82 @@
 };
 
 #ifdef __HIPCC__
+struct WgMap {
+  int taps, cin_w, cout_w, co_tiles;
+  __device__ long long operator()(int combo, int e) const {
+    const int tap = e >> 10, ci = (combo / co_tiles) * 32 + ((e >> 5) & 31), co = (combo % co_tiles) * 32 + (e & 31);
+    return ci < cin_w && co < cout_w ? (long long)(((size_t)co * cin_w + ci) * taps + tap) : -1;
+  }
+};
+struct WmMap {
+  int ncb, pw, xc, yc, nco, cin_w;
+  __device__ long long operator()(int combo, int e) const {
+    const int comp = e & 3, lane = (e >> 2) & 63, tap = (e >> 8) % 27, pair = e / (27 * 256);
+    const int wave = pair / pw, kk = pair % pw;
+    const int cib = wave % ncb, cob = (wave / ncb) * pw + kk;
+    const int co = (combo % nco) * yc + cob * 16 + 4 * (lane >> 4) + comp;
+    const int ci = (combo / nco) * xc + cib * 16 + (lane & 15);
+    return (long long)(((size_t)co * cin_w + ci) * 27 + tap);
+  }
+};
+struct WsMap {
+  int cin, cout, cin_w, cout_w;
+  __device__ long long operator()(int, int e) const {
+    const int co = e % cout, ci = (e / cout) % cin, tap = e / (cout * cin);
+    return ci < cin_w && co < cout_w ? (long long)(((size_t)co * cin_w + ci) * 27 + tap) : -1;
+  }
+};
+struct W1Map {
+  int cibw, ncob, cin;
+  __device__ long long operator()(int, int e) const {
+    const int comp = e & 3, lane = (e >> 2) & 63, pair = e >> 8;
+    const int kk = pair % ncob, c = (pair / ncob) % cibw, wave = pair / (ncob * cibw);
+    const int co = kk * 16 + 4 * (lane >> 4) + comp;
+    const int ci = (wave * cibw + c) * 16 + (lane & 15);
+    return ci < cin ? (long long)((size_t)co * cin + ci) : -1;
+  }
+};
+
+struct WgReduceJob {
+  enum Kind { None, Tiled, March, Stream, One } kind = None;
+  const float* slab = nullptr;
+  int nslab = 0, per = 0, combos = 0;
+  float* dw = nullptr;
+  union { WgMap g; WmMap m; WsMap s; W1Map o; } map = {};
+  void set(const WgMap& v) { kind = Tiled; map.g = v; }
+  void set(const WmMap& v) { kind = March; map.m = v; }
+  void set(const WsMap& v) { kind = Stream; map.s = v; }
+  void set(const W1Map& v) { kind = One; map.o = v; }
+  __host__ __device__ int blocks_per_combo() const { return (per + 63) / 64; }
+  int blocks() const { return kind == None ? 0 : combos * blocks_per_combo(); }
+};
+
+static constexpr int WG_RED_PAD = 65;
 template <typename Map>
-__global__ void __launch_bounds__(256)
-wgrad_reduce_kernel(const float* __restrict__ slab, int nslab, int per, Map map, float* __restrict__ dw) {
-  const int el = threadIdx.x & 15, part = threadIdx.x >> 4;
-  const int e = blockIdx.x * 16 + el;
-  const int combo = blockIdx.y;
-  double s0 = 0.0, s1 = 0.0;
-  if (e < per) {
-    const float* p = slab + (size_t)combo * nslab * per + e;
+__device__ __forceinline__ void wgrad_reduce_elements(const float* __restrict__ slab, int nslab, int per, const Map& map,
+                                                      float* __restrict__ dw, int bx, int combo, double (&red)[16][WG_RED_PAD]) {
+  const int quad = threadIdx.x & 15, part = threadIdx.x >> 4;
+  const int e0 = bx * 64 + quad * 4;
+  double s0[4] = {0.0, 0.0, 0.0, 0.0}, s1[4] = {0.0, 0.0, 0.0, 0.0};
+  if (e0 < per) {
+    const float* p = slab + (size_t)combo * nslab * per + e0;
     int k = part;
     for (; k + 16 < nslab; k += 32) {
-      s0 += (double)p[(size_t)k * per];
-      s1 += (double)p[(size_t)(k + 16) * per];
+      const float4 a = *reinterpret_cast<const float4*>(p + (size_t)k * per);
+      const float4 b = *reinterpret_cast<const float4*>(p + (size_t)(k + 16) * per);
+      s0[0] += (double)a.x; s0[1] += (double)a.y; s0[2] += (double)a.z; s0[3] += (double)a.w;
+      s1[0] += (double)b.x; s1[1] += (double)b.y; s1[2] += (double)b.z; s1[3] += (double)b.w;
     }
-    if (k < nslab) s0 += (double)p[(size_t)k * per];
+    if (k < nslab) {
+      const float4 a = *reinterpret_cast<const float4*>(p + (size_t)k * per);
+      s0[0] += (double)a.x; s0[1] += (double)a.y; s0[2] += (double)a.z; s0[3] += (double)a.w;
+    }
   }
-  __shared__ double red[16][17];
-  red[part][el] = s0 + s1;
+#pragma unroll
+  for (int j = 0; j < 4; ++j) red[part][quad * 4 + j] = s0[j] + s1[j];
   __syncthreads();
-  if (part == 0 && e < per) {
+  const int el = threadIdx.x, e = bx * 64 + el;
+  if (el < 64 && e < per) {
     const long long i = map(combo, e);
     if (i >= 0) {
       double t = red[0][el];
@@ -66,11 +124,30 @@
   }
 }
 
+__device__ __forceinline__ void wgrad_reduce_body(const WgReduceJob& job, int block) {
+  __shared__ double red[16][WG_RED_PAD];
+  const int bpc = job.blocks_per_combo();
+  const int combo = block / bpc, bx = block % bpc;
+  switch (job.kind) {
+    case WgReduceJob::Tiled: wgrad_reduce_elements(job.slab, job.nslab, job.per, job.map.g, job.dw, bx, combo, red); break;
+    case WgReduceJob::March: wgrad_reduce_elements(job.slab, job.nslab, job.per, job.map.m, job.dw, bx, combo, red); break;
+    case WgReduceJob::Stream: wgrad_reduce_elements(job.slab, job.nslab, job.per, job.map.s, job.dw, bx, combo, red); break;
+    case WgReduceJob::One: wgrad_reduce_elements(job.slab, job.nslab, job.per, job.map.o, job.dw, bx, combo, red); break;
+    default: break;
+  }
+}
+
+int launch_wgrad_reduce(const WgReduceJob& job, hipStream_t s);
 template <typename Map>
-static int launch_wgrad_reduce(const float* slab, int nslab, int per, int combos, Map map, float* dw, hipStream_t s) {
-  wgrad_reduce_kernel<Map><<<dim3(cdiv(per, 16), combos), 256, 0, s>>>(slab, nslab, per, map, dw);
-  SEUNET_LAUNCH_CHECK();
-  return 0;
+static int finish_wgrad(const float* slab, int nslab, int per, int combos, const Map& map, float* dw, WgReduceJob* defer,
+                        hipStream_t s) {
+  SEUNET_CHECK(per % 4 == 0 && (reinterpret_cast<uintptr_t>(slab) & 15) == 0,
+               "wgrad: the slab reduction reads 16 bytes at a time (slab of %d floats at %p)", per, (const void*)slab);
+  WgReduceJob job;
+  job.slab = slab; job.nslab = nslab; job.per = per; job.combos = combos; job.dw = dw;
+  job.set(map);
+  if (defer) { *defer = job; return 0; }
+  return launch_wgrad_reduce(job, s);
 }
 #endif
 
diff --git a/se-unet-airseg_amd/csrc/wgrad.hip b/se-unet-airseg_amd/csrc/wgrad.hip
--- a/se-unet-airseg_amd/csrc/wgrad.hip
+++ b/se-unet-airseg_amd/csrc/wgrad.hip
@@ -317,14 +317,6 @@
 #endif
 }
 
-struct WgMap {
-  int taps, cin_w, cout_w, co_tiles;
-  __device__ long long operator()(int combo, int e) const {
-    const int tap = e >> 10, ci = (combo / co_tiles) * 32 + ((e >> 5) & 31), co = (combo % co_tiles) * 32 + (e & 31);
-    return ci < cin_w && co < cout_w ? (long long)(((size_t)co * cin_w + ci) * taps + tap) : -1;
-  }
-};
-
 static inline int wgrad_groups(int combos, int total_tiles) {
   int g = WG_TILED_SLABS / combos;
   if (g < 16) g = 16;
@@ -344,15 +336,24 @@
   return tiled > other ? tiled : other;
 }
 
+__global__ void __launch_bounds__(256) wgrad_reduce_kernel(WgReduceJob job) { wgrad_reduce_body(job, blockIdx.x); }
+
+int launch_wgrad_reduce(const WgReduceJob& job, hipStream_t s) {
+  if (job.blocks() == 0) return 0;
+  wgrad_reduce_kernel<<<job.blocks(), 256, 0, s>>>(job);
+  SEUNET_LAUNCH_CHECK();
+  return 0;
+}
+
 int run_wgrad(ConvKernel k, int dtype, int taps, int dil, const SrcList& x, int cin_logical, const void* dy, int cout, float* dw,
-              void* workspace, size_t ws_bytes, Dims d, hipStream_t s) {
+              void* workspace, size_t ws_bytes, Dims d, hipStream_t s, WgReduceJob* defer) {
   switch (k) {
     case ConvKernel::Naive: return launch_wgrad_naive(dtype, taps, dil, x, cin_logical, dy, cout, dw, d, s);
-    case ConvKernel::Tiled: return launch_wgrad(dtype, taps, dil, x, cin_logical, dy, cout, dw, workspace, ws_bytes, d, s);
+    case ConvKernel::Tiled: return launch_wgrad(dtype, taps, dil, x, cin_logical, dy, cout, dw, workspace, ws_bytes, d, s, defer);
     case ConvKernel::Stream:
-      return launch_wgrad_stream(dtype, dil, x.ptr[0], x.C[0], cin_logical, dy, cout, cout, dw, workspace, ws_bytes, d, s);
-    case ConvKernel::March: return launch_wgrad_march(dtype, taps, dil, x, cin_logical, dy, cout, dw, workspace, ws_bytes, d, s);
-    case ConvKernel::Wgrad1x1: return launch_wgrad_1x1(dtype, x, cin_logical, dy, cout, dw, workspace, ws_bytes, d, s);
+      return launch_wgrad_stream(dtype, dil, x.ptr[0], x.C[0], cin_logical, dy, cout, cout, dw, workspace, ws_bytes, d, s, defer);
+    case ConvKernel::March: return launch_wgrad_march(dtype, taps, dil, x, cin_logical, dy, cout, dw, workspace, ws_bytes, d, s, defer);
+    case ConvKernel::Wgrad1x1: return launch_wgrad_1x1(dtype, x, cin_logical, dy, cout, dw, workspace, ws_bytes, d, s, defer);
   }
   return fail("wgrad: unknown kernel %d", (int)k);
 }
@@ -381,7 +382,7 @@
 }
 
 int launch_wgrad(int dtype, int taps, int dil, const SrcList& x, int cin_logical, const void* dy, int cout,
-                 float* dw, void* workspace, size_t ws_bytes, Dims d, hipStream_t s) {
+                 float* dw, void* workspace, size_t ws_bytes, Dims d, hipStream_t s, WgReduceJob* defer) {
   SEUNET_CHECK(taps == 27 || taps == 1, "wgrad: taps=%d unsupported", taps);
   SEUNET_CHECK(taps == 1 || dil == 1 || dil == 2, "wgrad: dilation %d unsupported", dil);
   SEUNET_CHECK(x.n >= 1 && x.n <= 3, "wgrad: 1..3 sources");
@@ -410,7 +411,7 @@
     else e = wgrad_launch_one<T, 27, 2, 4>(a, grid, s);
   });
   if (e) return e;
-  return launch_wgrad_reduce(a.slab, G, taps * 1024, combos, WgMap{taps, cin_logical, cout, a.co_tiles}, dw, s);
+  return finish_wgrad(a.slab, G, taps * 1024, combos, WgMap{taps, cin_logical, cout, a.co_tiles}, dw, defer, s);
 }
 
 template <typename T>
diff --git a/se-unet-airseg_amd/csrc/wgrad_1x1.hip b/se-unet-airseg_amd/csrc/wgrad_1x1.hip
--- a/se-unet-airseg_amd/csrc/wgrad_1x1.hip
+++ b/se-unet-airseg_amd/csrc/wgrad_1x1.hip
@@ -149,17 +149,6 @@
 #pragma unroll
     for (int k = 0; k < NCOB; ++k) *reinterpret_cast<f32x4*>(out + (c * NCOB + k) * 256) = acc[c][k];
 }
-
-struct W1Map {
-  int cibw, ncob, cin;
-  __device__ long long operator()(int, int e) const {
-    const int comp = e & 3, lane = (e >> 2) & 63, pair = e >> 8;
-    const int kk = pair % ncob, c = (pair / ncob) % cibw, wave = pair / (ncob * cibw);
-    const int co = kk * 16 + 4 * (lane >> 4) + comp;
-    const int ci = (wave * cibw + c) * 16 + (lane & 15);
-    return ci < cin ? (long long)((size_t)co * cin + ci) : -1;
-  }
-};
 
 struct W1Cfg { int cibw, ncob, ch, nst; };
 static bool wgrad_1x1_cfg(int dtype, const SrcList& x, int cin_logical, int cout, W1Cfg& c) {
@@ -211,7 +200,7 @@
 }
 
 int launch_wgrad_1x1(int dtype, const SrcList& x, int cin_logical, const void* dy, int cout, float* dw, void* workspace,
-                     size_t ws_bytes, Dims d, hipStream_t s) {
+                     size_t ws_bytes, Dims d, hipStream_t s, WgReduceJob* defer) {
   W1Cfg c;
   SEUNET_CHECK(wgrad_1x1_cfg(dtype, x, cin_logical, cout, c),
                "wgrad_1x1: 16-bit tensors, 1..3 sources of 32 or 64 channels (64, 128 or 192 together), 32 / 64 / 128 output channels only");
@@ -240,7 +229,7 @@
     else e = wgrad_1x1_launch<T, 3, 8, 64>(a, grid, lds, s);
   });
   if (e) return e;
-  return launch_wgrad_reduce(a.slab, grid, (int)slabs.per, 1, W1Map{c.cibw, c.ncob, cin_logical}, dw, s);
-}
-
-}
+  return finish_wgrad(a.slab, grid, (int)slabs.per, 1, W1Map{c.cibw, c.ncob, cin_logical}, dw, defer, s);
+}
+
+}
diff --git a/se-unet-airseg_amd/csrc/wgrad_march.hip b/se-unet-airseg_amd/csrc/wgrad_march.hip
--- a/se-unet-airseg_amd/csrc/wgrad_march.hip
+++ b/se-unet-airseg_amd/csrc/wgrad_march.hip
@@ -275,18 +275,6 @@
     for (int t = 0; t < 27; ++t) *reinterpret_cast<f32x4*>(out + (k * 27 + t) * 256) = acc[k][t];
 }
 
-struct WmMap {
-  int ncb, pw, xc, yc, nco, cin_w;
-  __device__ long long operator()(int combo, int e) const {
-    const int comp = e & 3, lane = (e >> 2) & 63, tap = (e >> 8) % 27, pair = e / (27 * 256);
-    const int wave = pair / pw, kk = pair % pw;
-    const int cib = wave % ncb, cob = (wave / ncb) * pw + kk;
-    const int co = (combo % nco) * yc + cob * 16 + 4 * (lane >> 4) + comp;
-    const int ci = (combo / nco) * xc + cib * 16 + (lane & 15);
-    return (long long)(((size_t)co * cin_w + ci) * 27 + tap);
-  }
-};
-
 struct WmCfg { int ncb, nob; };
 static WmCfg wm_blocks(int cin, int cout) {
   if (cin % 64 == 0) return {4, 2};
@@ -357,7 +345,7 @@
 }
 
 int launch_wgrad_march(int dtype, int taps, int dil, const SrcList& x, int cin_logical, const void* dy, int cout,
-                       float* dw, void* workspace, size_t ws_bytes, Dims d, hipStream_t s) {
+                       float* dw, void* workspace, size_t ws_bytes, Dims d, hipStream_t s, WgReduceJob* defer) {
   WmCfg c;
   SEUNET_CHECK(wgrad_march_cfg(dtype, taps, dil, x, cin_logical, cout, d, x.gap(), c),
                "wgrad_march: 16-bit 3x3x3 layers with 32k input and 32k output channels (one tensor or two equal halves) only");
@@ -381,8 +369,8 @@
     else e = wgrad_march_launch<T, 2, 2, 2>(a, grid, s);
   });
   if (e) return e;
-  return launch_wgrad_reduce(a.slab, cut.groups, (int)cut.slab_floats(), cut.combos,
-                             WmMap{c.ncb, cut.pw, cut.xc, cut.yc, cut.nco, cin_logical}, dw, s);
-}
-
-}
+  return finish_wgrad(a.slab, cut.groups, (int)cut.slab_floats(), cut.combos,
+                      WmMap{c.ncb, cut.pw, cut.xc, cut.yc, cut.nco, cin_logical}, dw, defer, s);
+}
+
+}
diff --git a/se-unet-airseg_amd/csrc/wgrad_stream.hip b/se-unet-airseg_amd/csrc/wgrad_stream.hip
--- a/se-unet-airseg_amd/csrc/wgrad_stream.hip
+++ b/se-unet-airseg_amd/csrc/wgrad_stream.hip
@@ -224,14 +224,6 @@
   }
 }
 
-struct WsMap {
-  int cin, cout, cin_w, cout_w;
-  __device__ long long operator()(int, int e) const {
-    const int co = e % cout, ci = (e / cout) % cin, tap = e / (cout * cin);
-    return ci < cin_w && co < cout_w ? (long long)(((size_t)co * cin_w + ci) * 27 + tap) : -1;
-  }
-};
-
 static bool ws_shape_ok(int cin, int cout, int dil) {
   if (cin == 32 && cout == 16) return dil == 1;
   return (cin == 8 && (cout == 8 || cout == 16)) || (cin == 16 && cout == 32) || (cin == 16 && cout == 16);
@@ -277,7 +269,7 @@
 }
 
 int launch_wgrad_stream(int dtype, int dil, const void* x, int x_c, int cin_w, const void* dy, int dy_c, int cout_w, float* dw,
-                        void* workspace, size_t ws_bytes, Dims d, hipStream_t s) {
+                        void* workspace, size_t ws_bytes, Dims d, hipStream_t s, WgReduceJob* defer) {
   SEUNET_CHECK(wgrad_stream_supported(dtype, 27, dil, x_c, dy_c), "wgrad_stream: unsupported shape (%d x %d channels, dilation %d)", x_c, dy_c, dil);
   SEUNET_CHECK(x && dy && dw && workspace && cin_w >= 1 && cin_w <= x_c && cout_w >= 1 && cout_w <= dy_c, "wgrad_stream: bad argument");
   const WsCut cut = ws_cut(d, dil);
@@ -298,7 +290,7 @@
   else if (x_c == 16 && dy_c == 32) e = dil == 1 ? ws_launch<16, 32, 1>(dtype, a, grid, s) : ws_launch<16, 32, 2>(dtype, a, grid, s);
   else if (x_c == 32 && dy_c == 16) e = ws_launch<32, 16, 1>(dtype, a, grid, s);
   if (e) return e;
-  return launch_wgrad_reduce(a.slab, cut.slabs(), (int)slabs.per, 1, WsMap{x_c, dy_c, cin_w, cout_w}, dw, s);
-}
-
-}
+  return finish_wgrad(a.slab, cut.slabs(), (int)slabs.per, 1, WsMap{x_c, dy_c, cin_w, cout_w}, dw, defer, s);
+}
+
+}
```
